# kondratevakate/mri-epilepsy-diagnosis

Measured on AMD Instinct MI355X. Metric: MRI volumes/sec (fwd+bwd) 3D U-Net @160x192x160, higher is better.
Workload: dtype f32; 1 GPU; unet.UNet(c0=8, 3 enc blocks, BN+PReLU, trilinear) fwd+softmax-Dice+bwd+AdamW, batch 2 x 1x160x192x160 fp32 per GPU (BASELINE configs[1]); global_batch=2, parallelism=dp1, launch=eager

## Files before the change

include/mri3d.h:

```cpp
#ifndef MRI3D_H
#define MRI3D_H

#include <stddef.h>
#include <stdint.h>

#ifdef __cplusplus
extern "C" {
#endif

typedef void* mri3d_stream_t;

enum { MRI3D_OK = 0, MRI3D_EINVAL = -1, MRI3D_ENOTSUP = -2, MRI3D_ELAUNCH = -3, MRI3D_EWORKSPACE = -4 };
enum { MRI3D_F32 = 0, MRI3D_BF16 = 1 };
enum { MRI3D_ACT_NONE = 0, MRI3D_ACT_RELU = 1, MRI3D_ACT_LEAKY = 2, MRI3D_ACT_PRELU = 3 };
enum { MRI3D_UP_NEAREST = 0, MRI3D_UP_TRILINEAR = 1 };
enum { MRI3D_PASS_FWD = 0, MRI3D_PASS_DGRAD = 1, MRI3D_PASS_WGRAD = 2 };

int mri3d_version(void);
const char* mri3d_last_error(void);

typedef struct Mri3dConvGeom {
    int32_t n;
    int32_t di, hi, wi, ci;
    int32_t dout, ho, wo, co;
    int32_t kd, kh, kw;
    int32_t sd, sh, sw;
    int32_t pd, ph, pw;
    int32_t dd, dh, dw;
    int32_t x_ld, y_ld;
    int32_t dtype;
} Mri3dConvGeom;

size_t mri3d_conv3d_workspace_bytes(const Mri3dConvGeom* g, int pass);

int mri3d_conv3d_fwd(const Mri3dConvGeom* g, const void* x, const void* w, const void* bias, void* y,
                     void* workspace, size_t ws_bytes, mri3d_stream_t stream);
int32_t mri3d_conv3d_fwd_stats_blocks(const Mri3dConvGeom* g);
int mri3d_conv3d_fwd_stats(const Mri3dConvGeom* g, const void* x, const void* w, const void* bias, void* y,
                           double* stat_partials, void* workspace, size_t ws_bytes, mri3d_stream_t stream);
int mri3d_conv3d_dgrad(const Mri3dConvGeom* g, const void* dy, const void* w, const void* bias, void* dx,
                       void* workspace, size_t ws_bytes, mri3d_stream_t stream);
int mri3d_conv3d_wgrad(const Mri3dConvGeom* g, const void* x, const void* dy, void* dw, void* dbias,
                       void* workspace, size_t ws_bytes, mri3d_stream_t stream);

int mri3d_conv3d_route(const Mri3dConvGeom* g, int32_t pass, int32_t stats, int32_t bias, int32_t split, int32_t second_ld,
                       int32_t align_x, int32_t align_y, char* name, size_t name_bytes);

int32_t mri3d_conv3d_cat_supported(const Mri3dConvGeom* g, int32_t split, int32_t second_ld, int32_t pass);
int32_t mri3d_conv3d_fwd_cat_stats_blocks(const Mri3dConvGeom* g, int32_t split, int32_t second_ld);
int mri3d_conv3d_fwd_cat(const Mri3dConvGeom* g, const void* x, const void* x2, int32_t split, int32_t x2_ld, const void* w,
                         const void* bias, void* y, double* stat_partials, void* workspace, size_t ws_bytes,
                         mri3d_stream_t stream);
int mri3d_conv3d_dgrad_cat(const Mri3dConvGeom* g, const void* dy, const void* w, void* dx, void* dx2, int32_t split,
                           int32_t dx2_ld, void* workspace, size_t ws_bytes, mri3d_stream_t stream);
int mri3d_conv3d_wgrad_cat(const Mri3dConvGeom* g, const void* x, const void* x2, int32_t split, int32_t x2_ld, const void* dy,
                           void* dw, void* dbias, void* workspace, size_t ws_bytes, mri3d_stream_t stream);

int32_t mri3d_conv3d_march_supported(const Mri3dConvGeom* g, int32_t pass);
int32_t mri3d_conv3d_march_stats_blocks(const Mri3dConvGeom* g);
int mri3d_conv3d_fwd_march(const Mri3dConvGeom* g, const void* x, const void* x2, int32_t split, int32_t x2_ld, const void* w,
                           const void* bias, void* y, double* stat_partials, void* workspace, size_t ws_bytes,
                           mri3d_stream_t stream);
int mri3d_conv3d_dgrad_march(const Mri3dConvGeom* g, const void* dy, const void* w, void* dx, void* dx2, int32_t split,
                             int32_t dx2_ld, void* workspace, size_t ws_bytes, mri3d_stream_t stream);

int32_t mri3d_upconv3d_supported(const Mri3dConvGeom* g, int32_t scale);
size_t mri3d_upconv3d_workspace_bytes(const Mri3dConvGeom* g, int32_t scale);
int mri3d_upconv3d_fwd(const Mri3dConvGeom* g, int32_t scale, const void* x, const float* w, const float* bias, void* y,
                       mri3d_stream_t stream);
int mri3d_upconv3d_dgrad(const Mri3dConvGeom* g, int32_t scale, const void* dy, const float* w, void* dx, mri3d_stream_t stream);
int mri3d_upconv3d_wgrad(const Mri3dConvGeom* g, int32_t scale, const void* x, const void* dy, float* dw, float* dbias,
                         void* workspace, size_t ws_bytes, mri3d_stream_t stream);

int32_t mri3d_convpair_supported(const Mri3dConvGeom* first, const Mri3dConvGeom* second);
size_t mri3d_convpair_workspace_bytes(const Mri3dConvGeom* first, const Mri3dConvGeom* second);
int mri3d_convpair_wgrad_first(const Mri3dConvGeom* first, const Mri3dConvGeom* second, const void* x, const void* dy2, const float* w2,
                               float* dw1, float* dbias1, void* workspace, size_t ws_bytes, mri3d_stream_t stream);

typedef struct Mri3dNormGeom {
    int32_t n;
    int64_t vox;
    int32_t c;
    int32_t x_ld;
    int32_t y_ld;
    int32_t instance;
    int32_t act;
    int32_t alpha_n;
    float slope;
    float eps;
    int32_t group_c;
    int32_t dtype;
} Mri3dNormGeom;

size_t mri3d_norm_workspace_bytes(const Mri3dNormGeom* g);

int mri3d_norm_stats(const Mri3dNormGeom* g, const void* x, float* mean, float* invstd,
                     float* running_mean, float* running_var, float momentum,
                     void* workspace, size_t ws_bytes, mri3d_stream_t stream);
int mri3d_norm_stats_from_partials(const Mri3dNormGeom* g, const double* partials, int32_t nblk, const float* shift,
                                   float* mean, float* invstd, float* running_mean, float* running_var, float momentum,
                                   mri3d_stream_t stream);
int mri3d_norm_act_fwd(const Mri3dNormGeom* g, const void* x, const float* mean, const float* invstd,
                       const float* gamma, const float* beta, const float* alpha, void* y,
                       mri3d_stream_t stream);
int mri3d_norm_act_bwd(const Mri3dNormGeom* g, int training, const void* x, const void* dy,
                       const float* mean, const float* invstd, const float* gamma, const float* beta,
                       const float* alpha, void* dx, float* dgamma, float* dbeta, float* dalpha,
                       void* workspace, size_t ws_bytes, mri3d_stream_t stream);

int32_t mri3d_norm_act_pw_supported(const Mri3dNormGeom* g, int32_t co);
size_t mri3d_norm_act_pw_workspace_bytes(const Mri3dNormGeom* g, int32_t co);
int mri3d_norm_act_pw_fwd(const Mri3dNormGeom* g, int32_t co, const void* x, const float* mean, const float* invstd,
                          const float* gamma, const float* beta, const float* alpha, const float* w, const float* bias,
                          void* out, mri3d_stream_t stream);
int mri3d_norm_act_pw_bwd(const Mri3dNormGeom* g, int32_t co, int training, const void* x, const void* dout,
                          const float* mean, const float* invstd, const float* gamma, const float* beta, const float* alpha,
                          const float* w, void* dx, float* dgamma, float* dbeta, float* dalpha, float* dw, float* dbias,
                          void* workspace, size_t ws_bytes, mri3d_stream_t stream);

typedef struct Mri3dPoolGeom {
    int32_t n, di, hi, wi, dout, ho, wo, c;
    int32_t kd, kh, kw, sd, sh, sw, pd, ph, pw;
    int32_t x_ld, y_ld;
    int32_t dtype;
} Mri3dPoolGeom;
int mri3d_maxpool3d_fwd(const Mri3dPoolGeom* g, const void* x, void* y, uint8_t* idx, mri3d_stream_t stream);
int mri3d_maxpool3d_bwd(const Mri3dPoolGeom* g, const void* dy, const uint8_t* idx, void* dx, mri3d_stream_t stream);
int mri3d_maxpool3d_bwd_add(const Mri3dPoolGeom* g, const void* dy, const uint8_t* idx, const void* addend,
                            int32_t addend_ld, void* dx, mri3d_stream_t stream);

typedef struct Mri3dUpGeom {
    int32_t n, di, hi, wi, dout, ho, wo, c;
    int32_t x_ld, y_ld;
    int32_t mode;
    int32_t align_corners;
    float rd, rh, rw;
    int32_t dtype;
} Mri3dUpGeom;
size_t mri3d_upsample3d_workspace_bytes(const Mri3dUpGeom* g);
int mri3d_upsample3d_fwd(const Mri3dUpGeom* g, const void* x, void* y, mri3d_stream_t stream);
int mri3d_upsample3d_bwd(const Mri3dUpGeom* g, const void* dy, void* dx, void* workspace, size_t ws_bytes,
                         mri3d_stream_t stream);

typedef struct Mri3dDiceGeom {
    int32_t n;
    int64_t vox;
    int32_t c, ct;
    int32_t x_ld, t_ld;
    float eps;
    int32_t dtype;
} Mri3dDiceGeom;
size_t mri3d_softmax_dice_workspace_bytes(const Mri3dDiceGeom* g);
int mri3d_softmax_dice_fwd(const Mri3dDiceGeom* g, const void* logits, const void* target, float* loss,
                           float* stats, void* workspace, size_t ws_bytes, mri3d_stream_t stream);
int mri3d_softmax_dice_bwd(const Mri3dDiceGeom* g, const void* logits, const void* target, const float* stats,
                           const float* dloss, void* dlogits, mri3d_stream_t stream);

int mri3d_argmax_u8(const void* logits, uint8_t* out, int64_t nvox, int32_t c, int32_t ld, int32_t dtype,
                    mri3d_stream_t stream);

size_t mri3d_mask_overlap_workspace_bytes(void);
int mri3d_mask_overlap(const uint8_t* pred, const uint8_t* gt, int64_t nvox, int64_t* counts, void* workspace,
                       size_t ws_bytes, mri3d_stream_t stream);

size_t mri3d_order_stats_workspace_bytes(void);
int mri3d_order_stats_f32(const float* x, int64_t n, const int64_t* ranks, int32_t nranks, float* out, void* workspace,
                          size_t ws_bytes, mri3d_stream_t stream);
int mri3d_piecewise_linear_f32(const float* x, float* y, int64_t n, const double* edges, const double* slope,
                               const double* intercept, int32_t nseg, mri3d_stream_t stream);
size_t mri3d_znorm_workspace_bytes(void);
int mri3d_znorm_mean_mask_f32(const float* x, float* y, int64_t n, double* stats, void* workspace, size_t ws_bytes,
                              mri3d_stream_t stream);
int mri3d_crop_or_pad_f32(const float* x, float* y, int32_t outer, int32_t di, int32_t hi, int32_t wi, int32_t dout,
                          int32_t ho, int32_t wo, float fill, mri3d_stream_t stream);

size_t mri3d_surface_distance_workspace_bytes(int32_t d, int32_t h, int32_t w);
int mri3d_surface_distance(const uint8_t* gt, const uint8_t* pred, int32_t d, int32_t h, int32_t w,
                           const double* area_table, double* sums, void* workspace, size_t ws_bytes, mri3d_stream_t stream);
int mri3d_surface_elements(const uint8_t* gt, const uint8_t* pred, int32_t d, int32_t h, int32_t w, int32_t* d2_gt,
                           uint8_t* code_gt, int32_t* d2_pred, uint8_t* code_pred, int64_t capacity, uint64_t* counts,
                           void* workspace, size_t ws_bytes, mri3d_stream_t stream);

int mri3d_extract_patches(const void* volumes, int32_t elem_bytes, int32_t nvol, int32_t d, int32_t h, int32_t w,
                          const int32_t* loc_host, int32_t npatch, int32_t pd, int32_t ph, int32_t pw, void* out,
                          mri3d_stream_t stream);
int mri3d_aggregate_patches_u8(const uint8_t* patches, const int32_t* loc_host, int32_t npatch, int32_t pd, int32_t ph,
                               int32_t pw, int32_t bd, int32_t bh, int32_t bw, uint8_t* out, int32_t nvol, int32_t d,
                               int32_t h, int32_t w, mri3d_stream_t stream);
int mri3d_aggregate_patches_argmax(const void* logits, int32_t c, int32_t ld, int32_t dtype, const int32_t* loc_host,
                                   int32_t npatch, int32_t pd, int32_t ph, int32_t pw, int32_t bd, int32_t bh, int32_t bw,
                                   uint8_t* out, int32_t nvol, int32_t d, int32_t h, int32_t w, mri3d_stream_t stream);

int mri3d_warp3d(const float* image, float* image_out, const void* label, void* label_out, int32_t label_bytes, int32_t s,
                 int32_t d, int32_t h, int32_t w, const float* affine, const float* grid, int32_t gd, int32_t gh, int32_t gw,
                 float pad_value, const float* pad_values, mri3d_stream_t stream);
int mri3d_bias_field_f32(const float* x, float* y, int32_t s, int32_t d, int32_t h, int32_t w, const float* coef_host,
                         int32_t order, mri3d_stream_t stream);

int mri3d_copy_channels(const void* src, void* dst, int64_t nvox, int32_t c, int32_t src_ld, int32_t dst_ld,
                        int32_t dtype, mri3d_stream_t stream);
int mri3d_add_channels(const void* a, const void* b, void* dst, int64_t nvox, int32_t c, int32_t a_ld,
                       int32_t b_ld, int32_t dst_ld, int32_t dtype, mri3d_stream_t stream);
int mri3d_convert_channels(const void* src, int32_t src_dtype, void* dst, int32_t dst_dtype, int64_t nvox, int32_t c,
                           int32_t src_ld, int32_t dst_ld, mri3d_stream_t stream);

int mri3d_bayes_weights_fwd(const float* mu, const float* logsigma, int64_t n, int32_t eval, float threshold, float* w_mean,
                            float* w_var, float* log_alpha, mri3d_stream_t stream);
int mri3d_bayes_weights_bwd(const float* mu, const float* logsigma, int64_t n, int32_t eval, float threshold,
                            const float* d_w_mean, const float* d_w_var, const float* d_log_alpha, float* dmu,
                            float* dlogsigma, mri3d_stream_t stream);
int mri3d_bayes_square(const void* x, void* x2, int64_t nvox, int32_t c, int32_t x_ld, int32_t x2_ld, int32_t dtype,
                       mri3d_stream_t stream);
int mri3d_bayes_sample_fwd(const void* mu_out, const void* var_out, const float* eps, void* y, int64_t nvox, int32_t c,
                           int32_t mu_ld, int32_t var_ld, int32_t eps_ld, int32_t y_ld, int32_t dtype, mri3d_stream_t stream);
int mri3d_bayes_sample_bwd(const void* dy, const void* var_out, const float* eps, void* dvar, int64_t nvox, int32_t c,
                           int32_t dy_ld, int32_t var_ld, int32_t eps_ld, int32_t dvar_ld, int32_t dtype,
                           mri3d_stream_t stream);
int mri3d_bayes_dx(const void* dx_mean, const void* dx_var, const void* x, void* dx, int64_t nvox, int32_t c,
                   int32_t dx_mean_ld, int32_t dx_var_ld, int32_t x_ld, int32_t dx_ld, int32_t dtype, mri3d_stream_t stream);

int mri3d_adam_step(float* p, const float* g, float* m, float* v, int64_t n, float lr, float beta1, float beta2,
                    float eps, float weight_decay, int32_t step, float grad_scale, int32_t decoupled,
                    mri3d_stream_t stream);

#ifdef __cplusplus
}
#endif
#endif
```

mri_epilepsy_diagnosis_amd/_lib.py:

```python
import ctypes
import os
from ctypes import POINTER, Structure, c_char_p, c_float, c_int32, c_int64, c_size_t, c_uint8, c_void_p

_HERE = os.path.dirname(os.path.abspath(__file__))
LIB_PATH = os.path.join(_HERE, "libmri3d_hip.so")

F32, BF16 = 0, 1
ACT_NONE, ACT_RELU, ACT_LEAKY, ACT_PRELU = 0, 1, 2, 3
UP_NEAREST, UP_TRILINEAR = 0, 1
PASS_FWD, PASS_DGRAD, PASS_WGRAD = 0, 1, 2


class ConvGeom(Structure):
    _fields_ = [(n, c_int32) for n in (
        "n", "di", "hi", "wi", "ci", "dout", "ho", "wo", "co", "kd", "kh", "kw", "sd", "sh", "sw",
        "pd", "ph", "pw", "dd", "dh", "dw", "x_ld", "y_ld", "dtype")]


class NormGeom(Structure):
    _fields_ = [("n", c_int32), ("vox", c_int64), ("c", c_int32), ("x_ld", c_int32), ("y_ld", c_int32),
                ("instance", c_int32), ("act", c_int32), ("alpha_n", c_int32), ("slope", c_float),
                ("eps", c_float), ("group_c", c_int32), ("dtype", c_int32)]


class PoolGeom(Structure):
    _fields_ = [(n, c_int32) for n in (
        "n", "di", "hi", "wi", "dout", "ho", "wo", "c", "kd", "kh", "kw", "sd", "sh", "sw", "pd", "ph", "pw",
        "x_ld", "y_ld", "dtype")]


class UpGeom(Structure):
    _fields_ = [(n, c_int32) for n in ("n", "di", "hi", "wi", "dout", "ho", "wo", "c", "x_ld", "y_ld", "mode",
                                       "align_corners")] + \
               [("rd", c_float), ("rh", c_float), ("rw", c_float), ("dtype", c_int32)]


class DiceGeom(Structure):
    _fields_ = [("n", c_int32), ("vox", c_int64), ("c", c_int32), ("ct", c_int32), ("x_ld", c_int32),
                ("t_ld", c_int32), ("eps", c_float), ("dtype", c_int32)]


_P = c_void_p
_FP = c_void_p

SIGNATURES = {
    "mri3d_version": (c_int32, []),
    "mri3d_last_error": (c_char_p, []),
    "mri3d_conv3d_workspace_bytes": (c_size_t, [POINTER(ConvGeom), c_int32]),
    "mri3d_conv3d_fwd": (c_int32, [POINTER(ConvGeom), _P, _P, _P, _P, _P, c_size_t, _P]),
    "mri3d_conv3d_fwd_stats_blocks": (c_int32, [POINTER(ConvGeom)]),
    "mri3d_conv3d_fwd_stats": (c_int32, [POINTER(ConvGeom), _P, _P, _P, _P, _P, _P, c_size_t, _P]),
    "mri3d_conv3d_dgrad": (c_int32, [POINTER(ConvGeom), _P, _P, _P, _P, _P, c_size_t, _P]),
    "mri3d_conv3d_wgrad": (c_int32, [POINTER(ConvGeom), _P, _P, _P, _P, _P, c_size_t, _P]),
    "mri3d_conv3d_route": (c_int32, [POINTER(ConvGeom), c_int32, c_int32, c_int32, c_int32, c_int32, c_int32, c_int32, c_char_p, c_size_t]),
    "mri3d_conv3d_cat_supported": (c_int32, [POINTER(ConvGeom), c_int32, c_int32, c_int32]),
    "mri3d_conv3d_fwd_cat_stats_blocks": (c_int32, [POINTER(ConvGeom), c_int32, c_int32]),
    "mri3d_conv3d_fwd_cat": (c_int32, [POINTER(ConvGeom), _P, _P, c_int32, c_int32, _P, _P, _P, _P, _P, c_size_t, _P]),
    "mri3d_conv3d_dgrad_cat": (c_int32, [POINTER(ConvGeom), _P, _P, _P, _P, c_int32, c_int32, _P, c_size_t, _P]),
    "mri3d_conv3d_wgrad_cat": (c_int32, [POINTER(ConvGeom), _P, _P, c_int32, c_int32, _P, _P, _P, _P, c_size_t, _P]),
    "mri3d_conv3d_march_supported": (c_int32, [POINTER(ConvGeom), c_int32]),
    "mri3d_conv3d_march_stats_blocks": (c_int32, [POINTER(ConvGeom)]),
    "mri3d_conv3d_fwd_march": (c_int32, [POINTER(ConvGeom), _P, _P, c_int32, c_int32, _P, _P, _P, _P, _P, c_size_t, _P]),
    "mri3d_conv3d_dgrad_march": (c_int32, [POINTER(ConvGeom), _P, _P, _P, _P, c_int32, c_int32, _P, c_size_t, _P]),
    "mri3d_upconv3d_supported": (c_int32, [POINTER(ConvGeom), c_int32]),
    "mri3d_upconv3d_workspace_bytes": (c_size_t, [POINTER(ConvGeom), c_int32]),
    "mri3d_upconv3d_fwd": (c_int32, [POINTER(ConvGeom), c_int32, _P, _FP, _FP, _P, _P]),
    "mri3d_upconv3d_dgrad": (c_int32, [POINTER(ConvGeom), c_int32, _P, _FP, _P, _P]),
    "mri3d_upconv3d_wgrad": (c_int32, [POINTER(ConvGeom), c_int32, _P, _P, _FP, _FP, _P, c_size_t, _P]),
    "mri3d_convpair_supported": (c_int32, [POINTER(ConvGeom), POINTER(ConvGeom)]),
    "mri3d_convpair_workspace_bytes": (c_size_t, [POINTER(ConvGeom), POINTER(ConvGeom)]),
    "mri3d_convpair_wgrad_first": (c_int32, [POINTER(ConvGeom), POINTER(ConvGeom), _P, _P, _FP, _FP, _FP, _P, c_size_t, _P]),
    "mri3d_norm_workspace_bytes": (c_size_t, [POINTER(NormGeom)]),
    "mri3d_norm_stats": (c_int32, [POINTER(NormGeom), _P, _FP, _FP, _FP, _FP, c_float, _P, c_size_t, _P]),
    "mri3d_norm_stats_from_partials": (c_int32, [POINTER(NormGeom), _P, c_int32, _FP, _FP, _FP, _FP, _FP, c_float, _P]),
    "mri3d_norm_act_fwd": (c_int32, [POINTER(NormGeom), _P, _FP, _FP, _FP, _FP, _FP, _P, _P]),
    "mri3d_norm_act_bwd": (c_int32, [POINTER(NormGeom), c_int32, _P, _P, _FP, _FP, _FP, _FP, _FP, _P, _FP, _FP, _FP,
                                     _P, c_size_t, _P]),
    "mri3d_norm_act_pw_supported": (c_int32, [POINTER(NormGeom), c_int32]),
    "mri3d_norm_act_pw_workspace_bytes": (c_size_t, [POINTER(NormGeom), c_int32]),
    "mri3d_norm_act_pw_fwd": (c_int32, [POINTER(NormGeom), c_int32, _P, _FP, _FP, _FP, _FP, _FP, _FP, _FP, _P, _P]),
    "mri3d_norm_act_pw_bwd": (c_int32, [POINTER(NormGeom), c_int32, c_int32, _P, _P, _FP, _FP, _FP, _FP, _FP, _FP, _P, _FP, _FP,
                                        _FP, _FP, _FP, _P, c_size_t, _P]),
    "mri3d_maxpool3d_fwd": (c_int32, [POINTER(PoolGeom), _P, _P, _P, _P]),
    "mri3d_maxpool3d_bwd": (c_int32, [POINTER(PoolGeom), _P, _P, _P, _P]),
    "mri3d_maxpool3d_bwd_add": (c_int32, [POINTER(PoolGeom), _P, _P, _P, c_int32, _P, _P]),
    "mri3d_upsample3d_workspace_bytes": (c_size_t, [POINTER(UpGeom)]),
    "mri3d_upsample3d_fwd": (c_int32, [POINTER(UpGeom), _P, _P, _P]),
    "mri3d_upsample3d_bwd": (c_int32, [POINTER(UpGeom), _P, _P, _P, c_size_t, _P]),
    "mri3d_softmax_dice_workspace_bytes": (c_size_t, [POINTER(DiceGeom)]),
    "mri3d_softmax_dice_fwd": (c_int32, [POINTER(DiceGeom), _P, _P, _FP, _FP, _P, c_size_t, _P]),
    "mri3d_softmax_dice_bwd": (c_int32, [POINTER(DiceGeom), _P, _P, _FP, _FP, _P, _P]),
    "mri3d_argmax_u8": (c_int32, [_P, _P, c_int64, c_int32, c_int32, c_int32, _P]),
    "mri3d_mask_overlap_workspace_bytes": (c_size_t, []),
    "mri3d_mask_overlap": (c_int32, [_P, _P, c_int64, _P, _P, c_size_t, _P]),
    "mri3d_order_stats_workspace_bytes": (c_size_t, []),
    "mri3d_order_stats_f32": (c_int32, [_P, c_int64, _P, c_int32, _P, _P, c_size_t, _P]),
    "mri3d_piecewise_linear_f32": (c_int32, [_P, _P, c_int64, _P, _P, _P, c_int32, _P]),
    "mri3d_znorm_workspace_bytes": (c_size_t, []),
    "mri3d_znorm_mean_mask_f32": (c_int32, [_P, _P, c_int64, _P, _P, c_size_t, _P]),
    "mri3d_crop_or_pad_f32": (c_int32, [_P, _P, c_int32, c_int32, c_int32, c_int32, c_int32, c_int32, c_int32, c_float, _P]),
    "mri3d_surface_distance_workspace_bytes": (c_size_t, [c_int32, c_int32, c_int32]),
    "mri3d_surface_distance": (c_int32, [_P, _P, c_int32, c_int32, c_int32, _P, _P, _P, c_size_t, _P]),
    "mri3d_surface_elements": (c_int32, [_P, _P, c_int32, c_int32, c_int32, _P, _P, _P, _P, c_int64, _P, _P, c_size_t, _P]),
    "mri3d_extract_patches": (c_int32, [_P, c_int32, c_int32, c_int32, c_int32, c_int32, _P, c_int32, c_int32, c_int32,
                                        c_int32, _P, _P]),
    "mri3d_aggregate_patches_u8": (c_int32, [_P, _P, c_int32, c_int32, c_int32, c_int32, c_int32, c_int32, c_int32, _P,
                                             c_int32, c_int32, c_int32, c_int32, _P]),
    "mri3d_aggregate_patches_argmax": (c_int32, [_P, c_int32, c_int32, c_int32, _P, c_int32, c_int32, c_int32, c_int32,
                                                 c_int32, c_int32, c_int32, _P, c_int32, c_int32, c_int32, c_int32, _P]),
    "mri3d_warp3d": (c_int32, [_FP, _FP, _P, _P, c_int32, c_int32, c_int32, c_int32, c_int32, _FP, _FP, c_int32, c_int32,
                               c_int32, c_float, _FP, _P]),
    "mri3d_bias_field_f32": (c_int32, [_FP, _FP, c_int32, c_int32, c_int32, c_int32, _P, c_int32, _P]),
    "mri3d_copy_channels": (c_int32, [_P, _P, c_int64, c_int32, c_int32, c_int32, c_int32, _P]),
    "mri3d_add_channels": (c_int32, [_P, _P, _P, c_int64, c_int32, c_int32, c_int32, c_int32, c_int32, _P]),
    "mri3d_convert_channels": (c_int32, [_P, c_int32, _P, c_int32, c_int64, c_int32, c_int32, c_int32, _P]),
    "mri3d_bayes_weights_fwd": (c_int32, [_FP, _FP, c_int64, c_int32, c_float, _FP, _FP, _FP, _P]),
    "mri3d_bayes_weights_bwd": (c_int32, [_FP, _FP, c_int64, c_int32, c_float, _FP, _FP, _FP, _FP, _FP, _P]),
    "mri3d_bayes_square": (c_int32, [_P, _P, c_int64, c_int32, c_int32, c_int32, c_int32, _P]),
    "mri3d_bayes_sample_fwd": (c_int32, [_P, _P, _FP, _P, c_int64, c_int32, c_int32, c_int32, c_int32, c_int32, c_int32, _P]),
    "mri3d_bayes_sample_bwd": (c_int32, [_P, _P, _FP, _P, c_int64, c_int32, c_int32, c_int32, c_int32, c_int32, c_int32, _P]),
    "mri3d_bayes_dx": (c_int32, [_P, _P, _P, _P, c_int64, c_int32, c_int32, c_int32, c_int32, c_int32, c_int32, _P]),
    "mri3d_adam_step": (c_int32, [_FP, _FP, _FP, _FP, c_int64, c_float, c_float, c_float, c_float, c_float, c_int32,
                                  c_float, c_int32, _P]),
}

_lib = None


class Mri3dError(RuntimeError):
    pass


def lib():
    global _lib
    if _lib is None:
        import torch
        if not os.path.exists(LIB_PATH):
            raise Mri3dError(
                "libmri3d_hip.so not found at %s — run `python -m mri_epilepsy_diagnosis_amd.build` "
                "(or __graft_entry__.build()).  There is no PyTorch fallback for device tensors." % LIB_PATH)
        h = ctypes.CDLL(LIB_PATH)
        for name, (res, args) in SIGNATURES.items():
            fn = getattr(h, name)
            fn.restype = res
            fn.argtypes = args
        _lib = h
    return _lib


def check(rc, what=""):
    if rc != 0:
        msg = lib().mri3d_last_error()
        raise Mri3dError("%s failed (rc=%d): %s" % (what, rc, msg.decode() if msg else "?"))
```

mri_epilepsy_diagnosis_amd/csrc/common.h:

```cpp
#pragma once
#include <hip/hip_runtime.h>
#include <stdint.h>
#include <stdio.h>
#include <stdarg.h>
#include <stdlib.h>
#include "../../include/mri3d.h"

namespace mri3d {

void set_error(const char* fmt, ...);

inline int check_launch(const char* what) {
    hipError_t e = hipGetLastError();
    if (e != hipSuccess) {
        set_error("%s: launch failed: %s", what, hipGetErrorString(e));
        return MRI3D_ELAUNCH;
    }
    return MRI3D_OK;
}

#define MRI3D_REQUIRE(cond, code, ...)      \
    do {                                    \
        if (!(cond)) {                      \
            ::mri3d::set_error(__VA_ARGS__); \
            return (code);                  \
        }                                   \
    } while (0)

#ifdef MRI3D_TUNING
inline int tuning_knob(const char* name, int dflt) {
    const char* v = getenv(name);
    return v ? atoi(v) : dflt;
}
#else
constexpr int tuning_knob(const char*, int dflt) { return dflt; }
#endif

inline int64_t cdiv64(int64_t a, int64_t b) { return (a + b - 1) / b; }
inline int cdiv(int a, int b) { return (a + b - 1) / b; }
inline size_t align_up(size_t x, size_t a) { return (x + a - 1) / a * a; }

constexpr int kMaxStreamBlocks = 2048;

inline int stream_grid(int64_t work_items, int per_block) {
    int64_t b = cdiv64(work_items, per_block);
    if (b > kMaxStreamBlocks) b = kMaxStreamBlocks;
    if (b < 1) b = 1;
    return (int)b;
}

typedef __bf16 bf16_t;
typedef __attribute__((ext_vector_type(4))) __bf16 bf16x4_t;
typedef __attribute__((ext_vector_type(8))) __bf16 bf16x8_t;

template <typename T> __device__ __forceinline__ float ldf(const T* p) { return (float)*p; }
template <typename T> __device__ __forceinline__ void stf(T* p, float v) { *p = (T)v; }

__device__ __forceinline__ float4 ldf4(const float* p) { return *reinterpret_cast<const float4*>(p); }
__device__ __forceinline__ float4 ldf4(const bf16_t* p) {
    const bf16x4_t v = *reinterpret_cast<const bf16x4_t*>(p);
    return make_float4((float)v[0], (float)v[1], (float)v[2], (float)v[3]);
}
__device__ __forceinline__ void stf4(float* p, float4 v) { *reinterpret_cast<float4*>(p) = v; }
__device__ __forceinline__ void stf4(bf16_t* p, float4 v) {
    bf16x4_t o;
    o[0] = (bf16_t)v.x, o[1] = (bf16_t)v.y, o[2] = (bf16_t)v.z, o[3] = (bf16_t)v.w;
    *reinterpret_cast<bf16x4_t*>(p) = o;
}

inline size_t dtype_size(int dtype) { return dtype == MRI3D_BF16 ? 2 : 4; }
inline bool aligned_vec4(int dtype, const void* a, const void* b = nullptr, const void* c = nullptr) {
    const uintptr_t m = dtype == MRI3D_BF16 ? 7 : 15;
    return ((reinterpret_cast<uintptr_t>(a) | reinterpret_cast<uintptr_t>(b) | reinterpret_cast<uintptr_t>(c)) & m) == 0;
}

inline bool aligned16(const void* a, const void* b = nullptr, const void* c = nullptr) {
    return ((reinterpret_cast<uintptr_t>(a) | reinterpret_cast<uintptr_t>(b) | reinterpret_cast<uintptr_t>(c)) & 15) == 0;
}

inline int ptr_align(const void* a, const void* b = nullptr, const void* c = nullptr, const void* d = nullptr) {
    const uintptr_t bits = reinterpret_cast<uintptr_t>(a) | reinterpret_cast<uintptr_t>(b) | reinterpret_cast<uintptr_t>(c) |
                           reinterpret_cast<uintptr_t>(d) | 16;
    return (int)(bits & (~bits + 1));
}
inline bool align_vec4(int dtype, int align) { return align >= (dtype == MRI3D_BF16 ? 8 : 16); }
inline bool align16(int align) { return align >= 16; }

#define MRI3D_DISPATCH_DTYPE(dtype, T, ...)  \
    do {                                     \
        if ((dtype) == MRI3D_BF16) {         \
            using T = ::mri3d::bf16_t;       \
            __VA_ARGS__                      \
        } else {                             \
            using T = float;                 \
            __VA_ARGS__                      \
        }                                    \
    } while (0)

__device__ __forceinline__ float wave_sum(float v) {
#pragma unroll
    for (int off = 32; off > 0; off >>= 1) v += __shfl_xor(v, off, 64);
    return v;
}

__device__ __forceinline__ double wave_sum_d(double v) {
#pragma unroll
    for (int off = 32; off > 0; off >>= 1) v += __shfl_xor(v, off, 64);
    return v;
}

__device__ __forceinline__ float apply_act(float v, int act, float slope) {
    if (act == MRI3D_ACT_RELU) return v > 0.f ? v : 0.f;
    if (act == MRI3D_ACT_LEAKY || act == MRI3D_ACT_PRELU) return v > 0.f ? v : v * slope;
    return v;
}

}
```

mri_epilepsy_diagnosis_amd/csrc/norm.hip:

```cpp
#include "common.h"
#include <algorithm>

namespace mri3d {

struct NormPlan {
    int vec;
    int CL;
    int VT;
    int cy;
    int nblk;
    int groups;
    int64_t gvox;
};

constexpr int kNormMaxBlocks = 1024;
constexpr int kFinQL = 64;

static NormPlan norm_plan(const Mri3dNormGeom& g, bool al, bool al16 = false) {
    NormPlan p;
    p.vec = (g.c % 4 == 0 && g.x_ld % 4 == 0 && g.y_ld % 4 == 0 && al) ? 4 : 1;
    if (p.vec == 4 && g.dtype == MRI3D_BF16 && g.c % 8 == 0 && g.x_ld % 8 == 0 && g.y_ld % 8 == 0 && al16) p.vec = 8;
    int lanes = g.c / p.vec;
    p.CL = lanes < 256 ? lanes : 256;
    p.cy = cdiv(lanes, p.CL);
// ... 370 lines not shown
            a += p[(size_t)q * C * 3];
            b += p[(size_t)q * C * 3 + 1];
            d += p[(size_t)q * C * 3 + 2];
            a1 += p[(size_t)(q + kFinQL) * C * 3];
            b1 += p[(size_t)(q + kFinQL) * C * 3 + 1];
            d1 += p[(size_t)(q + kFinQL) * C * 3 + 2];
        }
        if (q < nblk) {
            a += p[(size_t)q * C * 3];
            b += p[(size_t)q * C * 3 + 1];
            d += p[(size_t)q * C * 3 + 2];
        }
        a += a1;
        b += b1;
        d += d1;
    }
    r0[threadIdx.x] = a;
    r1[threadIdx.x] = b;
    r2[threadIdx.x] = d;
    __syncthreads();
    if (!ok || ql != 0) return;
    a = b = d = 0.0;
    for (int q = 0; q < kFinQL; ++q) {
        a += r0[slot * kFinQL + q];
        b += r1[slot * kFinQL + q];
        d += r2[slot * kFinQL + q];
    }
    sums[(size_t)i * 3] = (float)a;
    sums[(size_t)i * 3 + 1] = (float)b;
    sums[(size_t)i * 3 + 2] = (float)d;
}

__device__ __forceinline__ void norm_act_bwd_params_block(const float* __restrict__ sums, float* __restrict__ dgamma,
                                                          float* __restrict__ dbeta, float* __restrict__ dalpha, int alpha_n, int C,
                                                          int groups) {
    __shared__ double dal[256];
    double my_dal = 0.0;
    for (int c = threadIdx.x; c < C; c += blockDim.x) {
        double tg = 0.0, tb = 0.0, ta = 0.0;
        for (int g = 0; g < groups; ++g) {
            tb += (double)sums[((size_t)g * C + c) * 3];
            tg += (double)sums[((size_t)g * C + c) * 3 + 1];
            ta += (double)sums[((size_t)g * C + c) * 3 + 2];
        }
        if (dgamma) dgamma[c] = (float)tg;
        if (dbeta) dbeta[c] = (float)tb;
        if (dalpha && alpha_n > 1) dalpha[c] = (float)ta;
        my_dal += ta;
    }
    if (dalpha && alpha_n == 1) {
        dal[threadIdx.x] = my_dal;
        __syncthreads();
        if (threadIdx.x == 0) {
            double t = 0.0;
            for (int i = 0; i < (int)blockDim.x; ++i) t += dal[i];
            dalpha[0] = (float)t;
        }
    }
}

__global__ void norm_act_bwd_params_kernel(const float* __restrict__ sums, float* __restrict__ dgamma,
                                           float* __restrict__ dbeta, float* __restrict__ dalpha, int alpha_n, int C,
                                           int groups) {
    norm_act_bwd_params_block(sums, dgamma, dbeta, dalpha, alpha_n, C, groups);
}

template <typename T, int VEC>
__global__ void __launch_bounds__(256)
norm_act_bwd_apply_kernel(const T* __restrict__ x, const T* __restrict__ dy, T* __restrict__ dx,
                          const float* __restrict__ sums, const float* __restrict__ mean,
                          const float* __restrict__ invstd, const float* __restrict__ gamma,
                          const float* __restrict__ beta, const float* __restrict__ alpha, int alpha_n, int act,
                          float slope, int training, int C, int x_ld, int y_ld, int64_t gvox, int CL, int VT, int group_c,
                          float* __restrict__ dgamma, float* __restrict__ dbeta, float* __restrict__ dalpha) {
    if ((dgamma != nullptr || dbeta != nullptr || dalpha != nullptr) && blockIdx.x == 0 && blockIdx.y == 0 && blockIdx.z == 0)
        norm_act_bwd_params_block(sums, dgamma, dbeta, dalpha, alpha_n, C, (int)gridDim.z);
    const int tid = threadIdx.x;
    const int cl = tid % CL, vt = tid / CL;
    const int c0 = (blockIdx.y * CL + cl) * VEC;
    if (vt >= VT || c0 >= C) return;
    const int group = blockIdx.z;
    float mu[VEC], is[VEC], gm[VEC], bt[VEC], al[VEC], k0[VEC], k1[VEC], k2[VEC];
    const float invM = 1.f / ((float)gvox * (float)(group_c > 0 ? group_c : 1));
#pragma unroll
    for (int j = 0; j < VEC; ++j) {
        int c = c0 + j;
        gm[j] = gamma ? gamma[c] : 1.f;
        bt[j] = beta ? beta[c] : 0.f;
        mu[j] = mean ? mean[group * C + c] : 0.f;
        is[j] = invstd ? invstd[group * C + c] : 1.f;
        al[j] = (act == MRI3D_ACT_PRELU) ? alpha[alpha_n == 1 ? 0 : c]
                                          : (act == MRI3D_ACT_LEAKY ? slope : (act == MRI3D_ACT_RELU ? 0.f : 1.f));
        k0[j] = gm[j] * is[j];
        if (training) {
            const float kk = group_c > 0 ? is[j] : k0[j];
            k1[j] = kk * sums[((size_t)group * C + c) * 3] * invM;
            k2[j] = kk * sums[((size_t)group * C + c) * 3 + 1] * invM;
        } else {
            k1[j] = 0.f;
            k2[j] = 0.f;
        }
    }
    const T* xg = x + (int64_t)group * gvox * x_ld;
    const T* dg = dy + (int64_t)group * gvox * y_ld;
    T* og = dx + (int64_t)group * gvox * x_ld;
    auto apply = [&](const float (&xv)[VEC], const float (&gv)[VEC], float (&ov)[VEC]) {
#pragma unroll
        for (int j = 0; j < VEC; ++j) {
            float xh = (xv[j] - mu[j]) * is[j];
            float u = fmaf(gm[j], xh, bt[j]);
            float du = (u > 0.f) ? gv[j] : gv[j] * al[j];
            ov[j] = fmaf(k0[j], du, -k1[j]) - xh * k2[j];
        }
    };
    const int64_t step = (int64_t)gridDim.x * VT;
    int64_t v = (int64_t)blockIdx.x * VT + vt;
    for (; v + step < gvox; v += 2 * step) {
        float xa[VEC], ga[VEC], xb[VEC], gb[VEC], ov[VEC];
        Ld<VEC>::load(xg + v * x_ld + c0, xa);
        Ld<VEC>::load(dg + v * y_ld + c0, ga);
        Ld<VEC>::load(xg + (v + step) * x_ld + c0, xb);
        Ld<VEC>::load(dg + (v + step) * y_ld + c0, gb);
        apply(xa, ga, ov);
        Ld<VEC>::store(og + v * x_ld + c0, ov);
        apply(xb, gb, ov);
        Ld<VEC>::store(og + (v + step) * x_ld + c0, ov);
    }
    for (; v < gvox; v += step) {
        float xv[VEC], gv[VEC], ov[VEC];
        Ld<VEC>::load(xg + v * x_ld + c0, xv);
        Ld<VEC>::load(dg + v * y_ld + c0, gv);
        apply(xv, gv, ov);
        Ld<VEC>::store(og + v * x_ld + c0, ov);
    }
}


struct NapArgs {
    const float *mean, *invstd, *gamma, *beta, *alpha;
    int alpha_n, act;
    float slope;
    int C, x_ld;
    int64_t nvox;
};

constexpr int kNapMaxCo = 4;

template <typename T>
__device__ __forceinline__ float through_storage(float v) {
    if constexpr (sizeof(T) == 2) return (float)(bf16_t)v;
    else return v;
}

__device__ __forceinline__ void nap_fwd_consts(const NapArgs& p, int c0, float (&sc)[4], float (&sh)[4], float (&al)[4]) {
#pragma unroll
    for (int j = 0; j < 4; ++j) {
        int c = c0 + j;
        float gm = p.gamma ? p.gamma[c] : 1.f;
        float bt = p.beta ? p.beta[c] : 0.f;
        float mu = p.mean ? p.mean[c] : 0.f;
        float is = p.invstd ? p.invstd[c] : 1.f;
        sc[j] = gm * is;
        sh[j] = bt - mu * sc[j];
        al[j] = (p.act == MRI3D_ACT_PRELU) ? p.alpha[p.alpha_n == 1 ? 0 : c] : p.slope;
    }
}

template <typename T, int CO>
__global__ void __launch_bounds__(256)
norm_act_pw_fwd_kernel(const T* __restrict__ x, T* __restrict__ out, const float* __restrict__ w,
                       const float* __restrict__ bias, int Co, int o_ld, NapArgs p) {
    const int QC = p.C >> 2, VT = 256 / QC;
    const int q = threadIdx.x % QC, vt = threadIdx.x / QC;
    float sc[4], sh[4], al[4];
    nap_fwd_consts(p, 4 * q, sc, sh, al);
    float4 wq[CO];
    float bq[CO];
#pragma unroll
    for (int co = 0; co < CO; ++co) {
        const float* wr = w + (size_t)(co < Co ? co : 0) * p.C + 4 * q;
        wq[co] = co < Co ? make_float4(wr[0], wr[1], wr[2], wr[3]) : make_float4(0.f, 0.f, 0.f, 0.f);
        bq[co] = (bias != nullptr && co < Co) ? bias[co] : 0.f;
    }
    constexpr int U = 4;
    const int64_t stride = (int64_t)gridDim.x * VT;
    for (int64_t v0 = (int64_t)blockIdx.x * VT + vt; v0 < p.nvox; v0 += stride * U) {
        float xv[U][4];
#pragma unroll
        for (int u = 0; u < U; ++u) {
            const int64_t v = v0 + u * stride;
            Ld<4>::load(x + (v < p.nvox ? v : p.nvox - 1) * p.x_ld + 4 * q, xv[u]);
        }
#pragma unroll
        for (int u = 0; u < U; ++u) {
            const int64_t v = v0 + u * stride;
            float a[4];
#pragma unroll
            for (int j = 0; j < 4; ++j) a[j] = through_storage<T>(apply_act(fmaf(xv[u][j], sc[j], sh[j]), p.act, al[j]));
            float acc[CO];
#pragma unroll
            for (int co = 0; co < CO; ++co) {
                float t = a[0] * wq[co].x;
                t = fmaf(a[1], wq[co].y, t);
                t = fmaf(a[2], wq[co].z, t);
                t = fmaf(a[3], wq[co].w, t);
                for (int d = 1; d < QC; d <<= 1) t += __shfl_xor(t, d, 64);
                acc[co] = t + bq[co];
            }
            if (q == 0 && v < p.nvox) {
                T* op = out + v * o_ld;
#pragma unroll
                for (int co = 0; co < CO; ++co)
                    if (co < Co) stf(op + co, acc[co]);
            }
        }
    }
}

template <typename T, int CO>
struct PwHeadGrad {
    struct Args {
        const T* dout;
        const float* w;
        int Co, ld;
    };
    static constexpr int kCo = CO;
    static constexpr int kSide = 5 * CO;
    const T* dout;
    int Co, ld;
    float4 wq[CO];
    double dw[4][CO], db[CO];

    __device__ __forceinline__ void init(const Args& a, int C, int q) {
        dout = a.dout, Co = a.Co, ld = a.ld;
#pragma unroll
        for (int co = 0; co < CO; ++co) {
            const float* wr = a.w + (size_t)(co < Co ? co : 0) * C + 4 * q;
            wq[co] = co < Co ? make_float4(wr[0], wr[1], wr[2], wr[3]) : make_float4(0.f, 0.f, 0.f, 0.f);
            db[co] = 0.0;
#pragma unroll
            for (int j = 0; j < 4; ++j) dw[j][co] = 0.0;
        }
    }
    __device__ __forceinline__ void load(int64_t v, float (&gv)[CO]) const {
#pragma unroll
        for (int co = 0; co < CO; ++co) gv[co] = co < Co ? ldf(dout + v * ld + co) : 0.f;
    }
    __device__ __forceinline__ void grad(const float (&gv)[CO], float (&da)[4]) const {
        float4 acc = make_float4(0.f, 0.f, 0.f, 0.f);
#pragma unroll
        for (int co = 0; co < CO; ++co) {
            acc.x = fmaf(gv[co], wq[co].x, acc.x);
            acc.y = fmaf(gv[co], wq[co].y, acc.y);
            acc.z = fmaf(gv[co], wq[co].z, acc.z);
            acc.w = fmaf(gv[co], wq[co].w, acc.w);
        }
        da[0] = through_storage<T>(acc.x), da[1] = through_storage<T>(acc.y);
        da[2] = through_storage<T>(acc.z), da[3] = through_storage<T>(acc.w);
    }
    __device__ __forceinline__ void side(const float (&a)[4], const float (&gv)[CO], bool lead) {
#pragma unroll
        for (int co = 0; co < CO; ++co) {
#pragma unroll
            for (int j = 0; j < 4; ++j) dw[j][co] += (double)(a[j] * gv[co]);
            if (lead) db[co] += (double)gv[co];
        }
    }
    __device__ __forceinline__ void flush(double* red, double* __restrict__ spart, int C, int QC, int VT) const {
        const int tid = threadIdx.x;
#pragma unroll
        for (int co = 0; co < CO; ++co) {
#pragma unroll
            for (int j = 0; j < 4; ++j) red[tid * kSide + j * CO + co] = dw[j][co];
            red[tid * kSide + 4 * CO + co] = db[co];
        }
        __syncthreads();
        double* o = spart + (size_t)blockIdx.x * (Co * C + Co);
        for (int e = tid; e < QC * 4 * CO; e += 256) {
            const int co = e % CO, j = (e / CO) % 4, qq = e / (4 * CO);
            double s = 0.0;
            for (int l = 0; l < VT; ++l) s += red[(l * QC + qq) * kSide + j * CO + co];
            if (co < Co) o[co * C + 4 * qq + j] = s;
        }
        if (tid < Co) {
            double s = 0.0;
            for (int l = 0; l < VT; ++l) s += red[(l * QC) * kSide + 4 * CO + tid];
            o[Co * C + tid] = s;
        }
    }
};

template <typename T, class SRC, bool SUMS, bool DX>
__global__ void __launch_bounds__(256)
norm_act_src_bwd_kernel(const T* __restrict__ x, T* __restrict__ dx, typename SRC::Args sa, NapArgs p,
                        const float* __restrict__ sums, int training, double* __restrict__ part, double* __restrict__ spart,
                        float* __restrict__ dgamma, float* __restrict__ dbeta, float* __restrict__ dalpha) {
    constexpr int kRed = SUMS ? (SRC::kSide > 12 ? SRC::kSide : 12) : 1;
    __shared__ double red[256 * kRed];
    if (!SUMS && (dgamma != nullptr || dbeta != nullptr || dalpha != nullptr) && blockIdx.x == 0)
        norm_act_bwd_params_block(sums, dgamma, dbeta, dalpha, p.alpha_n, p.C, 1);
    const int QC = p.C >> 2, VT = 256 / QC;
    const int tid = threadIdx.x;
    const int q = tid % QC, vt = tid / QC;
    const int c0 = 4 * q;
    float mu[4], is[4], gm[4], bt[4], al[4], k0[4], k1[4], k2[4];
    const float invM = 1.f / (float)p.nvox;
#pragma unroll
    for (int j = 0; j < 4; ++j) {
        int c = c0 + j;
        gm[j] = p.gamma ? p.gamma[c] : 1.f;
        bt[j] = p.beta ? p.beta[c] : 0.f;
        mu[j] = p.mean ? p.mean[c] : 0.f;
        is[j] = p.invstd ? p.invstd[c] : 1.f;
        al[j] = (p.act == MRI3D_ACT_PRELU) ? p.alpha[p.alpha_n == 1 ? 0 : c]
                                            : (p.act == MRI3D_ACT_LEAKY ? p.slope : (p.act == MRI3D_ACT_RELU ? 0.f : 1.f));
        k0[j] = gm[j] * is[j];
        if (DX && !SUMS && training) {
            k1[j] = k0[j] * sums[(size_t)c * 3] * invM;
            k2[j] = k0[j] * sums[(size_t)c * 3 + 1] * invM;
        } else {
            k1[j] = 0.f;
            k2[j] = 0.f;
        }
    }
    float sc[4], sh[4], af[4];
    if constexpr (SUMS) nap_fwd_consts(p, c0, sc, sh, af);
    SRC src;
    src.init(sa, p.C, q);
    double s0[4], s1[4], s2[4];
#pragma unroll
    for (int j = 0; j < 4; ++j) { s0[j] = 0.0; s1[j] = 0.0; s2[j] = 0.0; }
    auto row = [&](const float (&xv)[4], const float (&gv)[SRC::kCo], int64_t v) {
        float da[4], ov[4];
        src.grad(gv, da);
#pragma unroll
        for (int j = 0; j < 4; ++j) {
            float xh = (xv[j] - mu[j]) * is[j];
            float u = fmaf(gm[j], xh, bt[j]);
            bool pos = u > 0.f;
            float du = pos ? da[j] : da[j] * al[j];
            if constexpr (SUMS) {
                s0[j] += (double)du;
                s1[j] = fma((double)du, (double)xh, s1[j]);
                s2[j] += pos ? 0.0 : (double)da[j] * (double)u;
            }
            if constexpr (DX) ov[j] = fmaf(k0[j], du, -k1[j]) - xh * k2[j];
        }
        if constexpr (SUMS) {
            float a[4];
#pragma unroll
            for (int j = 0; j < 4; ++j) a[j] = through_storage<T>(apply_act(fmaf(xv[j], sc[j], sh[j]), p.act, af[j]));
            src.side(a, gv, q == 0);
        }
        if constexpr (DX) Ld<4>::store(dx + v * p.x_ld + c0, ov);
    };
    const int64_t step = (int64_t)gridDim.x * VT;
    int64_t v = (int64_t)blockIdx.x * VT + vt;
    for (; v + step < p.nvox; v += 2 * step) {
        float xa[4], xb[4], ga[SRC::kCo], gb[SRC::kCo];
        Ld<4>::load(x + v * p.x_ld + c0, xa);
        src.load(v, ga);
        Ld<4>::load(x + (v + step) * p.x_ld + c0, xb);
        src.load(v + step, gb);
        row(xa, ga, v);
        row(xb, gb, v + step);
    }
    for (; v < p.nvox; v += step) {
        float xv[4], gv[SRC::kCo];
        Ld<4>::load(x + v * p.x_ld + c0, xv);
        src.load(v, gv);
        row(xv, gv, v);
    }
    if constexpr (SUMS) {
#pragma unroll
        for (int j = 0; j < 4; ++j) {
            red[(tid * 4 + j) * 3] = s0[j];
            red[(tid * 4 + j) * 3 + 1] = s1[j];
            red[(tid * 4 + j) * 3 + 2] = s2[j];
        }
        __syncthreads();
        if (vt == 0) {
#pragma unroll
            for (int j = 0; j < 4; ++j) {
                double a = 0.0, b = 0.0, d = 0.0;
                for (int l = 0; l < VT; ++l) {
                    a += red[((l * QC + q) * 4 + j) * 3];
                    b += red[((l * QC + q) * 4 + j) * 3 + 1];
                    d += red[((l * QC + q) * 4 + j) * 3 + 2];
                }
                double* o = part + ((size_t)blockIdx.x * p.C + c0 + j) * 3;
                o[0] = a;
                o[1] = b;
                o[2] = d;
            }
        }
        __syncthreads();
        src.flush(red, spart, p.C, QC, VT);
    }
}

__global__ void __launch_bounds__(256)
norm_act_pw_wsum_kernel(const double* __restrict__ spart, float* __restrict__ dw, float* __restrict__ dbias, int nb, int nw,
                        int Co) {
    __shared__ double red[256];
    const int el = threadIdx.x >> 5, ql = threadIdx.x & 31;
    const int ntot = nw + Co;
    const int i = blockIdx.x * 8 + el;
    double s = 0.0;
    if (i < ntot)
        for (int b = ql; b < nb; b += 32) s += spart[(size_t)b * ntot + i];
    red[threadIdx.x] = s;
    __syncthreads();
    if (ql == 0 && i < ntot) {
        double t = 0.0;
        for (int k = 0; k < 32; ++k) t += red[el * 32 + k];
        if (i < nw) {
            if (dw != nullptr) dw[i] = (float)t;
        } else if (dbias != nullptr) {
            dbias[i - nw] = (float)t;
        }
    }
}

struct NapPlan {
    int QC, VT, nblk;
    size_t part_off, sums_off, side_off, bytes;
};

static bool nap_supported(const Mri3dNormGeom& g, int co) {
    if (g.dtype != MRI3D_F32 && g.dtype != MRI3D_BF16) return false;
    if (g.n <= 0 || g.vox <= 0 || g.instance || g.group_c != 0) return false;
    const int qc = g.c / 4;
    if (g.c <= 0 || g.c % 4 != 0 || qc > 16 || (qc & (qc - 1)) != 0) return false;
    if (co < 1 || co > kNapMaxCo) return false;
    if (g.x_ld < g.c || g.x_ld % 4 != 0 || g.y_ld < co) return false;
    if (g.act < MRI3D_ACT_NONE || g.act > MRI3D_ACT_PRELU) return false;
    if (g.act == MRI3D_ACT_PRELU && g.alpha_n != 1 && g.alpha_n != g.c) return false;
    return true;
}

static NapPlan nap_plan(const Mri3dNormGeom& g, int co) {
    NapPlan p;
    p.QC = g.c / 4;
    p.VT = 256 / p.QC;
    const int64_t nvox = (int64_t)g.n * g.vox;
    const int64_t want = cdiv64(nvox, (int64_t)p.VT * 8);
    p.nblk = (int)(want < kNormMaxBlocks ? want : kNormMaxBlocks);
    if (p.nblk < 1) p.nblk = 1;
    p.part_off = 0;
    p.sums_off = (size_t)p.nblk * g.c * 3 * sizeof(double);
    p.side_off = p.sums_off + align_up((size_t)g.c * 3 * sizeof(float), sizeof(double));
    p.bytes = p.side_off + (size_t)p.nblk * (co * g.c + co) * sizeof(double);
    return p;
}

}

using namespace mri3d;

extern "C" size_t mri3d_norm_workspace_bytes(const Mri3dNormGeom* g) {
    if (!g) return 0;
    return norm_workspace_floats(*g) * sizeof(float);
}

static int norm_check(const Mri3dNormGeom* g, const char* who) {
    MRI3D_REQUIRE(g != nullptr, MRI3D_EINVAL, "%s: null geometry", who);
    MRI3D_REQUIRE(g->dtype == MRI3D_F32 || g->dtype == MRI3D_BF16, MRI3D_ENOTSUP, "%s: unknown dtype %d", who, g->dtype);
    MRI3D_REQUIRE(g->n > 0 && g->vox > 0 && g->c > 0 && g->x_ld >= g->c && g->y_ld >= g->c, MRI3D_EINVAL,
                  "%s: bad geometry n=%d vox=%lld c=%d x_ld=%d y_ld=%d", who, g->n, (long long)g->vox, g->c, g->x_ld,
                  g->y_ld);
    MRI3D_REQUIRE(g->act != MRI3D_ACT_PRELU || g->alpha_n == 1 || g->alpha_n == g->c, MRI3D_EINVAL,
                  "%s: PReLU alpha_n=%d must be 1 or C=%d", who, g->alpha_n, g->c);
    MRI3D_REQUIRE(g->group_c == 0 || (g->group_c > 0 && g->instance && g->c % g->group_c == 0), MRI3D_EINVAL,
                  "%s: group_c=%d needs instance mode and must divide C=%d", who, g->group_c, g->c);
    return MRI3D_OK;
}

extern "C" int mri3d_norm_stats(const Mri3dNormGeom* g, const void* x, float* mean, float* invstd, float* running_mean,
                                float* running_var, float momentum, void* workspace, size_t ws_bytes,
                                mri3d_stream_t stream) {
    int rc = norm_check(g, "norm_stats");
    if (rc) return rc;
    MRI3D_REQUIRE(x && mean && invstd, MRI3D_EINVAL, "norm_stats: null pointer");
    MRI3D_REQUIRE(workspace && ws_bytes >= mri3d_norm_workspace_bytes(g), MRI3D_EWORKSPACE,
                  "norm_stats: workspace %zu < %zu", ws_bytes, mri3d_norm_workspace_bytes(g));
    hipStream_t s = static_cast<hipStream_t>(stream);
    Mri3dNormGeom gg = *g;
    gg.y_ld = gg.x_ld;
    NormPlan p = norm_plan(gg, aligned_vec4(g->dtype, x));
    double* part = static_cast<double*>(workspace);
    dim3 grid(p.nblk, p.cy, p.groups);
    const int tot = p.groups * g->c;
    MRI3D_DISPATCH_DTYPE(g->dtype, T, {
        const T* xf = static_cast<const T*>(x);
        if (p.vec == 4)
            hipLaunchKernelGGL((norm_stats_kernel<T, 4>), grid, dim3(256), 0, s, xf, part, g->c, g->x_ld, p.gvox, p.CL, p.VT);
        else if (p.vec == 1)
            hipLaunchKernelGGL((norm_stats_kernel<T, 1>), grid, dim3(256), 0, s, xf, part, g->c, g->x_ld, p.gvox, p.CL, p.VT);
        hipLaunchKernelGGL(norm_stats_finalize_kernel<T>, dim3(cdiv(tot, 256 / kFinQL)), dim3(256), 0, s, xf, part, mean,
                           invstd, running_mean, running_var, momentum, g->eps, g->c, g->x_ld, p.gvox, p.nblk, p.groups);
        if (g->group_c > 0) {
            const int ng = p.groups * (g->c / g->group_c);
            hipLaunchKernelGGL(norm_stats_group_finalize_kernel<T>, dim3(cdiv(ng, 64)), dim3(64), 0, s, xf, part, mean,
                               invstd, g->eps, g->c, g->x_ld, p.gvox, p.nblk, p.groups, g->group_c);
        }
    });
    return check_launch("norm_stats");
}

extern "C" int mri3d_norm_stats_from_partials(const Mri3dNormGeom* g, const double* partials, int32_t nblk, const float* shift,
                                              float* mean, float* invstd, float* running_mean, float* running_var,
                                              float momentum, mri3d_stream_t stream) {
    int rc = norm_check(g, "norm_stats_from_partials");
    if (rc) return rc;
    MRI3D_REQUIRE(partials && mean && invstd && nblk > 0, MRI3D_EINVAL, "norm_stats_from_partials: null pointer / no partials");
    MRI3D_REQUIRE(!g->instance && g->group_c == 0, MRI3D_ENOTSUP,
                  "norm_stats_from_partials: batch statistics only (one group over N x voxels)");
    hipStream_t s = static_cast<hipStream_t>(stream);
    const int64_t gvox = (int64_t)g->n * g->vox;
    hipLaunchKernelGGL(norm_stats_finalize_kernel<float>, dim3(cdiv(g->c, 256 / kFinQL)), dim3(256), 0, s,
                       static_cast<const float*>(nullptr), partials, mean, invstd, running_mean, running_var, momentum, g->eps,
                       g->c, g->x_ld, gvox, nblk, 1, shift, 1);
    return check_launch("norm_stats_from_partials");
}

extern "C" int mri3d_norm_act_fwd(const Mri3dNormGeom* g, const void* x, const float* mean, const float* invstd,
                                  const float* gamma, const float* beta, const float* alpha, void* y,
                                  mri3d_stream_t stream) {
    int rc = norm_check(g, "norm_act_fwd");
    if (rc) return rc;
    MRI3D_REQUIRE(x && y, MRI3D_EINVAL, "norm_act_fwd: null pointer");
    MRI3D_REQUIRE((mean == nullptr) == (invstd == nullptr), MRI3D_EINVAL, "norm_act_fwd: mean/invstd must both be set");
    MRI3D_REQUIRE(g->act != MRI3D_ACT_PRELU || alpha, MRI3D_EINVAL, "norm_act_fwd: PReLU needs alpha");
    hipStream_t s = static_cast<hipStream_t>(stream);
    NormPlan p = norm_plan(*g, aligned_vec4(g->dtype, x, y), aligned16(x, y));
    dim3 grid(p.nblk, p.cy, p.groups);
    MRI3D_DISPATCH_DTYPE(g->dtype, T, {
        const T* xf = static_cast<const T*>(x);
        T* yf = static_cast<T*>(y);
        if constexpr (sizeof(T) == 2) {
            if (p.vec == 8) hipLaunchKernelGGL((norm_act_fwd_kernel<T, 8>), grid, dim3(256), 0, s, xf, yf, mean, invstd, gamma, beta, alpha,
                               g->alpha_n, g->act, g->slope, g->c, g->x_ld, g->y_ld, p.gvox, p.CL, p.VT);
        }
        if (p.vec == 4)
            hipLaunchKernelGGL((norm_act_fwd_kernel<T, 4>), grid, dim3(256), 0, s, xf, yf, mean, invstd, gamma, beta, alpha,
                               g->alpha_n, g->act, g->slope, g->c, g->x_ld, g->y_ld, p.gvox, p.CL, p.VT);
        else if (p.vec == 1)
            hipLaunchKernelGGL((norm_act_fwd_kernel<T, 1>), grid, dim3(256), 0, s, xf, yf, mean, invstd, gamma, beta, alpha,
                               g->alpha_n, g->act, g->slope, g->c, g->x_ld, g->y_ld, p.gvox, p.CL, p.VT);
    });
    return check_launch("norm_act_fwd");
}

extern "C" int mri3d_norm_act_bwd(const Mri3dNormGeom* g, int training, const void* x, const void* dy,
                                  const float* mean, const float* invstd, const float* gamma, const float* beta,
                                  const float* alpha, void* dx, float* dgamma, float* dbeta, float* dalpha,
                                  void* workspace, size_t ws_bytes, mri3d_stream_t stream) {
    int rc = norm_check(g, "norm_act_bwd");
    if (rc) return rc;
    MRI3D_REQUIRE(x && dy && dx, MRI3D_EINVAL, "norm_act_bwd: null pointer");
    MRI3D_REQUIRE((mean == nullptr) == (invstd == nullptr), MRI3D_EINVAL, "norm_act_bwd: mean/invstd must both be set");
    MRI3D_REQUIRE(!(training && mean == nullptr), MRI3D_EINVAL, "norm_act_bwd: training mode needs statistics");
    MRI3D_REQUIRE(g->act != MRI3D_ACT_PRELU || alpha, MRI3D_EINVAL, "norm_act_bwd: PReLU needs alpha");
    MRI3D_REQUIRE(workspace && ws_bytes >= mri3d_norm_workspace_bytes(g), MRI3D_EWORKSPACE,
                  "norm_act_bwd: workspace %zu < %zu", ws_bytes, mri3d_norm_workspace_bytes(g));
    hipStream_t s = static_cast<hipStream_t>(stream);
    NormPlan p = norm_plan(*g, aligned_vec4(g->dtype, x, dy, dx));
    dim3 grid(p.nblk, p.cy, p.groups);
    double* part = static_cast<double*>(workspace);
    float* sums = reinterpret_cast<float*>(part + (size_t)p.groups * p.nblk * g->c * 3);
    const bool need_reduce = training || dgamma || dbeta || dalpha;
    bool params_done = false;
    MRI3D_DISPATCH_DTYPE(g->dtype, T, {
        const T* xf = static_cast<const T*>(x);
// ... 4 lines not shown
                hipLaunchKernelGGL((norm_act_bwd_frozen_kernel<T, 4>), grid, dim3(256), 0, s, xf, df, of, part, mean, invstd,
                                   gamma, beta, alpha, g->alpha_n, g->act, g->slope, g->c, g->x_ld, g->y_ld, p.gvox, p.CL,
                                   p.VT);
            else if (p.vec == 1)
                hipLaunchKernelGGL((norm_act_bwd_frozen_kernel<T, 1>), grid, dim3(256), 0, s, xf, df, of, part, mean, invstd,
                                   gamma, beta, alpha, g->alpha_n, g->act, g->slope, g->c, g->x_ld, g->y_ld, p.gvox, p.CL,
                                   p.VT);
            hipLaunchKernelGGL(norm_act_bwd_sums_kernel, dim3(cdiv(p.groups * g->c, 256 / kFinQL)), dim3(256), 0, s, part,
                               sums, g->c, p.nblk, p.groups);
            hipLaunchKernelGGL(norm_act_bwd_params_kernel, dim3(1), dim3(256), 0, s, sums, dgamma, dbeta, dalpha, g->alpha_n,
                               g->c, p.groups);
            return check_launch("norm_act_bwd");
        }
        if (need_reduce) {
            if (p.vec == 4)
                hipLaunchKernelGGL((norm_act_bwd_reduce_kernel<T, 4>), grid, dim3(256), 0, s, xf, df, part, mean, invstd,
                                   gamma, beta, alpha, g->alpha_n, g->act, g->slope, g->c, g->x_ld, g->y_ld, p.gvox, p.CL,
                                   p.VT);
            else if (p.vec == 1)
                hipLaunchKernelGGL((norm_act_bwd_reduce_kernel<T, 1>), grid, dim3(256), 0, s, xf, df, part, mean, invstd,
                                   gamma, beta, alpha, g->alpha_n, g->act, g->slope, g->c, g->x_ld, g->y_ld, p.gvox, p.CL,
                                   p.VT);
            hipLaunchKernelGGL(norm_act_bwd_sums_kernel, dim3(cdiv(p.groups * g->c, 256 / kFinQL)), dim3(256), 0, s, part,
                               sums, g->c, p.nblk, p.groups);
            if ((dgamma || dbeta || dalpha) && g->group_c > 0) {
                hipLaunchKernelGGL(norm_act_bwd_params_kernel, dim3(1), dim3(256), 0, s, sums, dgamma, dbeta, dalpha,
                                   g->alpha_n, g->c, p.groups);
                params_done = true;
            }
            if (g->group_c > 0 && training) {
                const int ng = p.groups * (g->c / g->group_c);
                hipLaunchKernelGGL(norm_act_bwd_group_combine_kernel, dim3(cdiv(ng, 64)), dim3(64), 0, s, sums, gamma,
                                   g->c, p.groups, g->group_c);
            }
        }
        float* pg = params_done ? nullptr : dgamma;
        float* pb = params_done ? nullptr : dbeta;
        float* pa = params_done ? nullptr : dalpha;
        if (p.vec == 4)
            hipLaunchKernelGGL((norm_act_bwd_apply_kernel<T, 4>), grid, dim3(256), 0, s, xf, df, of, sums, mean, invstd,
                               gamma, beta, alpha, g->alpha_n, g->act, g->slope, training, g->c, g->x_ld, g->y_ld, p.gvox,
                               p.CL, p.VT, g->group_c, pg, pb, pa);
        else if (p.vec == 1)
            hipLaunchKernelGGL((norm_act_bwd_apply_kernel<T, 1>), grid, dim3(256), 0, s, xf, df, of, sums, mean, invstd,
                               gamma, beta, alpha, g->alpha_n, g->act, g->slope, training, g->c, g->x_ld, g->y_ld, p.gvox,
                               p.CL, p.VT, g->group_c, pg, pb, pa);
    });
    return check_launch("norm_act_bwd");
}

extern "C" int32_t mri3d_norm_act_pw_supported(const Mri3dNormGeom* g, int32_t co) {
    return (g != nullptr && nap_supported(*g, co)) ? 1 : 0;
}

extern "C" size_t mri3d_norm_act_pw_workspace_bytes(const Mri3dNormGeom* g, int32_t co) {
    if (g == nullptr || !nap_supported(*g, co)) return 0;
    return nap_plan(*g, co).bytes;
}

static NapArgs nap_args(const Mri3dNormGeom& g, const float* mean, const float* invstd, const float* gamma, const float* beta,
                        const float* alpha) {
    NapArgs a;
    a.mean = mean, a.invstd = invstd, a.gamma = gamma, a.beta = beta, a.alpha = alpha;
    a.alpha_n = g.alpha_n, a.act = g.act, a.slope = g.slope, a.C = g.c, a.x_ld = g.x_ld;
    a.nvox = (int64_t)g.n * g.vox;
    return a;
}

extern "C" int mri3d_norm_act_pw_fwd(const Mri3dNormGeom* g, int32_t co, const void* x, const float* mean, const float* invstd,
                                     const float* gamma, const float* beta, const float* alpha, const float* w,
                                     const float* bias, void* out, mri3d_stream_t stream) {
    MRI3D_REQUIRE(g != nullptr, MRI3D_EINVAL, "norm_act_pw_fwd: null geometry");
    MRI3D_REQUIRE(nap_supported(*g, co), MRI3D_ENOTSUP, "norm_act_pw_fwd: c=%d co=%d x_ld=%d y_ld=%d instance=%d not served",
                  g->c, co, g->x_ld, g->y_ld, g->instance);
    MRI3D_REQUIRE(x && w && out, MRI3D_EINVAL, "norm_act_pw_fwd: null pointer");
    MRI3D_REQUIRE((mean == nullptr) == (invstd == nullptr), MRI3D_EINVAL, "norm_act_pw_fwd: mean/invstd must both be set");
    MRI3D_REQUIRE(g->act != MRI3D_ACT_PRELU || alpha, MRI3D_EINVAL, "norm_act_pw_fwd: PReLU needs alpha");
    MRI3D_REQUIRE(aligned_vec4(g->dtype, x), MRI3D_EINVAL, "norm_act_pw_fwd: x must be aligned to 4 elements");
    hipStream_t s = static_cast<hipStream_t>(stream);
    const NapArgs a = nap_args(*g, mean, invstd, gamma, beta, alpha);
    const int VT = 256 / (g->c / 4);
    const unsigned grid = (unsigned)std::max<int64_t>(1, std::min<int64_t>(cdiv64(a.nvox, (int64_t)VT * 4), kMaxStreamBlocks));
    MRI3D_DISPATCH_DTYPE(g->dtype, T, {
        if (co <= 2)
            hipLaunchKernelGGL((norm_act_pw_fwd_kernel<T, 2>), dim3(grid), dim3(256), 0, s, (const T*)x, (T*)out, w, bias, co,
                               g->y_ld, a);
        else
            hipLaunchKernelGGL((norm_act_pw_fwd_kernel<T, 4>), dim3(grid), dim3(256), 0, s, (const T*)x, (T*)out, w, bias, co,
                               g->y_ld, a);
    });
    return check_launch("norm_act_pw_fwd");
}

template <typename T, int CO>
static void nap_bwd_launch(const Mri3dNormGeom& g, int co, int training, const T* x, const T* dout, const float* w, T* dx,
                           float* dgamma, float* dbeta, float* dalpha, float* dw, float* dbias, const NapArgs& a,
                           const NapPlan& p, char* ws, hipStream_t s) {
    using SRC = PwHeadGrad<T, CO>;
    const typename SRC::Args sa = {dout, w, co, g.y_ld};
    double* part = reinterpret_cast<double*>(ws + p.part_off);
    float* sums = reinterpret_cast<float*>(ws + p.sums_off);
    double* spart = reinterpret_cast<double*>(ws + p.side_off);
    const dim3 grid(p.nblk), blk(256);
    const bool params = dgamma || dbeta || dalpha;
    const bool need_sums = training || params || dw || dbias;
    if (need_sums) {
        if (training || dx == nullptr)
            hipLaunchKernelGGL((norm_act_src_bwd_kernel<T, SRC, true, false>), grid, blk, 0, s, x, dx, sa, a, sums, training,
                               part, spart, dgamma, dbeta, dalpha);
        else
            hipLaunchKernelGGL((norm_act_src_bwd_kernel<T, SRC, true, true>), grid, blk, 0, s, x, dx, sa, a, sums, training,
                               part, spart, dgamma, dbeta, dalpha);
        hipLaunchKernelGGL(norm_act_bwd_sums_kernel, dim3(cdiv(g.c, 256 / kFinQL)), dim3(256), 0, s, part, sums, g.c, p.nblk, 1);
        if (dw || dbias)
            hipLaunchKernelGGL(norm_act_pw_wsum_kernel, dim3(cdiv(co * g.c + co, 8)), dim3(256), 0, s, spart, dw, dbias, p.nblk,
                               co * g.c, co);
        if (params && !(training && dx != nullptr))
            hipLaunchKernelGGL(norm_act_bwd_params_kernel, dim3(1), dim3(256), 0, s, sums, dgamma, dbeta, dalpha, g.alpha_n, g.c,
                               1);
    }
    if (dx != nullptr && (training || !need_sums))
        hipLaunchKernelGGL((norm_act_src_bwd_kernel<T, SRC, false, true>), grid, blk, 0, s, x, dx, sa, a, sums, training, part,
                           spart, dgamma, dbeta, dalpha);
}

extern "C" int mri3d_norm_act_pw_bwd(const Mri3dNormGeom* g, int32_t co, int training, const void* x, const void* dout,
                                     const float* mean, const float* invstd, const float* gamma, const float* beta,
                                     const float* alpha, const float* w, void* dx, float* dgamma, float* dbeta, float* dalpha,
                                     float* dw, float* dbias, void* workspace, size_t ws_bytes, mri3d_stream_t stream) {
    MRI3D_REQUIRE(g != nullptr, MRI3D_EINVAL, "norm_act_pw_bwd: null geometry");
    MRI3D_REQUIRE(nap_supported(*g, co), MRI3D_ENOTSUP, "norm_act_pw_bwd: c=%d co=%d x_ld=%d y_ld=%d instance=%d not served",
                  g->c, co, g->x_ld, g->y_ld, g->instance);
    MRI3D_REQUIRE(x && dout && w, MRI3D_EINVAL, "norm_act_pw_bwd: null pointer");
    MRI3D_REQUIRE((mean == nullptr) == (invstd == nullptr), MRI3D_EINVAL, "norm_act_pw_bwd: mean/invstd must both be set");
    MRI3D_REQUIRE(!(training && mean == nullptr), MRI3D_EINVAL, "norm_act_pw_bwd: training mode needs statistics");
    MRI3D_REQUIRE(g->act != MRI3D_ACT_PRELU || alpha, MRI3D_EINVAL, "norm_act_pw_bwd: PReLU needs alpha");
    MRI3D_REQUIRE(aligned_vec4(g->dtype, x, dx), MRI3D_EINVAL, "norm_act_pw_bwd: x and dx must be aligned to 4 elements");
    const NapPlan p = nap_plan(*g, co);
    MRI3D_REQUIRE(workspace && ws_bytes >= p.bytes && (reinterpret_cast<uintptr_t>(workspace) & 7) == 0, MRI3D_EWORKSPACE,
                  "norm_act_pw_bwd: workspace %zu < %zu (or not 8-byte aligned)", ws_bytes, p.bytes);
    hipStream_t s = static_cast<hipStream_t>(stream);
    const NapArgs a = nap_args(*g, mean, invstd, gamma, beta, alpha);
    char* ws = static_cast<char*>(workspace);
    MRI3D_DISPATCH_DTYPE(g->dtype, T, {
        if (co <= 2)
            nap_bwd_launch<T, 2>(*g, co, training, (const T*)x, (const T*)dout, w, (T*)dx, dgamma, dbeta, dalpha, dw, dbias, a, p, ws,
                                 s);
        else
            nap_bwd_launch<T, 4>(*g, co, training, (const T*)x, (const T*)dout, w, (T*)dx, dgamma, dbeta, dalpha, dw, dbias, a, p, ws,
                                 s);
    });
    return check_launch("norm_act_pw_bwd");
}
```

mri_epilepsy_diagnosis_amd/csrc/resample.hip:

```cpp
#include "common.h"
#include <limits.h>
#include <algorithm>
#include <stdlib.h>

namespace mri3d {

template <int VEC>
struct V {
    float v[VEC];
    template <typename T>
    __device__ __forceinline__ void load(const T* p) {
        if constexpr (VEC == 8) {
            const bf16x8_t t = *reinterpret_cast<const bf16x8_t*>(p);
#pragma unroll
            for (int j = 0; j < 8; ++j) v[j] = (float)t[j];
        } else if constexpr (VEC == 4) {
            float4 t = ldf4(p);
            v[0] = t.x; v[1] = t.y; v[2] = t.z; v[3] = t.w;
        } else {
            v[0] = ldf(p);
        }
    }
    template <typename T>
    __device__ __forceinline__ void store(T* p) const {
// ... 53 lines not shown
                }
            }
            V<VEC> o;
#pragma unroll
            for (int j = 0; j < VEC; ++j) o.v[j] = best[j];
            const int64_t ov = obase + pix;
            o.store(y + ov * g.y_ld + cv * VEC);
            uint8_t* ip = idx + ov * g.c + cv * VEC;
            if constexpr (VEC == 8) {
                uint2 pk;
                pk.x = (uint32_t)bi[0] | ((uint32_t)bi[1] << 8) | ((uint32_t)bi[2] << 16) | ((uint32_t)bi[3] << 24);
                pk.y = (uint32_t)bi[4] | ((uint32_t)bi[5] << 8) | ((uint32_t)bi[6] << 16) | ((uint32_t)bi[7] << 24);
                *reinterpret_cast<uint2*>(ip) = pk;
            } else if constexpr (VEC == 4) {
                *reinterpret_cast<uint32_t*>(ip) = (uint32_t)bi[0] | ((uint32_t)bi[1] << 8) |
                                                   ((uint32_t)bi[VEC > 2 ? 2 : 0] << 16) | ((uint32_t)bi[VEC > 3 ? 3 : 0] << 24);
            } else {
                ip[0] = (uint8_t)bi[0];
            }
        }
    }
}

template <typename T, int VEC>
__global__ void __launch_bounds__(256)
maxpool_bwd_kernel(Mri3dPoolGeom g, const T* __restrict__ dy, const uint8_t* __restrict__ idx,
                   T* __restrict__ dx, int hch, const T* __restrict__ addend, int a_ld) {
    const unsigned CV = g.c / VEC;
    const int hchunks = (g.hi + hch - 1) / hch;
    const int slabs = g.n * g.di * hchunks;
    for (int slab = blockIdx.x; slab < slabs; slab += gridDim.x) {
        const int hc = slab % hchunks, nd = slab / hchunks;
        const int n = nd / g.di, id = nd - n * g.di;
        const int h0 = hc * hch, hn = min(hch, g.hi - h0);
        const unsigned inner = (unsigned)hn * g.wi * CV;
        int od_lo = id + g.pd - g.kd + 1; od_lo = od_lo <= 0 ? 0 : (od_lo + g.sd - 1) / g.sd;
        int od_hi = (id + g.pd) / g.sd; if (od_hi > g.dout - 1) od_hi = g.dout - 1;
        const int64_t ibase = ((int64_t)nd * g.hi + h0) * g.wi;
        for (unsigned e = threadIdx.x; e < inner; e += blockDim.x) {
            const unsigned cv = e % CV, pix = e / CV;
            const int iw = pix % g.wi, ih = h0 + pix / g.wi;
            float acc[VEC];
#pragma unroll
            for (int j = 0; j < VEC; ++j) acc[j] = 0.f;
            if (addend != nullptr) {
                V<VEC> av;
                av.load(addend + (ibase + pix) * a_ld + cv * VEC);
#pragma unroll
                for (int j = 0; j < VEC; ++j) acc[j] = av.v[j];
            }
            int oh_lo = ih + g.ph - g.kh + 1; oh_lo = oh_lo <= 0 ? 0 : (oh_lo + g.sh - 1) / g.sh;
            int oh_hi = (ih + g.ph) / g.sh; if (oh_hi > g.ho - 1) oh_hi = g.ho - 1;
            int ow_lo = iw + g.pw - g.kw + 1; ow_lo = ow_lo <= 0 ? 0 : (ow_lo + g.sw - 1) / g.sw;
            int ow_hi = (iw + g.pw) / g.sw; if (ow_hi > g.wo - 1) ow_hi = g.wo - 1;
            for (int od = od_lo; od <= od_hi; ++od) {
                const int kd = id - (od * g.sd - g.pd);
                for (int oh = oh_lo; oh <= oh_hi; ++oh) {
                    const int kh = ih - (oh * g.sh - g.ph);
                    for (int ow = ow_lo; ow <= ow_hi; ++ow) {
                        const int kw = iw - (ow * g.sw - g.pw);
                        const int tap = (kd * g.kh + kh) * g.kw + kw;
                        const int64_t ov = (((int64_t)n * g.dout + od) * g.ho + oh) * g.wo + ow;
                        V<VEC> gv;
                        gv.load(dy + ov * g.y_ld + cv * VEC);
                        const uint8_t* ip = idx + ov * g.c + cv * VEC;
                        if constexpr (VEC == 8) {
                            const uint2 pk = *reinterpret_cast<const uint2*>(ip);
#pragma unroll
                            for (int j = 0; j < 4; ++j) {
                                if ((int)((pk.x >> (8 * j)) & 0xff) == tap) acc[j] += gv.v[j];
                                if ((int)((pk.y >> (8 * j)) & 0xff) == tap) acc[4 + j] += gv.v[4 + j];
                            }
                        } else if constexpr (VEC == 4) {
                            const uint32_t pk = *reinterpret_cast<const uint32_t*>(ip);
#pragma unroll
                            for (int j = 0; j < VEC; ++j)
                                if ((int)((pk >> (8 * j)) & 0xff) == tap) acc[j] += gv.v[j];
                        } else {
                            if ((int)ip[0] == tap) acc[0] += gv.v[0];
                        }
                    }
                }
            }
            V<VEC> o;
#pragma unroll
            for (int j = 0; j < VEC; ++j) o.v[j] = acc[j];
            o.store(dx + (ibase + pix) * g.x_ld + cv * VEC);
        }
    }
}

template <typename T, int VEC>
__global__ void __launch_bounds__(256)
maxpool2_fwd_kernel(Mri3dPoolGeom g, const T* __restrict__ x, T* __restrict__ y, uint8_t* __restrict__ idx, int hch) {
    const unsigned CV = g.c / VEC;
    const int hchunks = (g.ho + hch - 1) / hch;
    const int slabs = g.n * g.dout * hchunks;
    const unsigned row = (unsigned)g.wi * g.x_ld, plane = (unsigned)g.hi * row;
    for (int slab = blockIdx.x; slab < slabs; slab += gridDim.x) {
        const int hc = slab % hchunks, nd = slab / hchunks;
        const int n = nd / g.dout, od = nd - n * g.dout;
        const int h0 = hc * hch, hn = min(hch, g.ho - h0);
        const unsigned inner = (unsigned)hn * g.wi * CV;
        const T* xs = x + ((int64_t)n * g.di + 2 * od) * g.hi * g.wi * g.x_ld;
        const int64_t obase = ((int64_t)nd * g.ho + h0) * g.wo;
        for (unsigned e0 = 0; e0 < inner; e0 += blockDim.x) {
            const unsigned e = e0 + threadIdx.x;
            const bool live = e < inner;
            const unsigned ee = live ? e : 0;
            const unsigned cv = ee % CV, col = ee / CV;
            const unsigned iw = col % g.wi, ohl = col / g.wi;
            const unsigned kw = iw & 1, ow = iw >> 1, oh = h0 + ohl;
            const T* p0 = xs + (2 * oh) * row + iw * (unsigned)g.x_ld + cv * VEC;
            V<VEC> v[4];
#pragma unroll
            for (int t = 0; t < 4; ++t) v[t].load(p0 + (t >> 1) * plane + (t & 1) * row);
            float best[VEC];
            int bi[VEC];
#pragma unroll
            for (int j = 0; j < VEC; ++j) { best[j] = v[0].v[j]; bi[j] = (int)kw; }
#pragma unroll
            for (int t = 1; t < 4; ++t)
#pragma unroll
                for (int j = 0; j < VEC; ++j)
                    if (v[t].v[j] > best[j] || v[t].v[j] != v[t].v[j]) { best[j] = v[t].v[j]; bi[j] = 2 * t + (int)kw; }
            V<VEC> o;
            int oi[VEC];
#pragma unroll
            for (int j = 0; j < VEC; ++j) {
                const float pb = __shfl_xor(best[j], (int)CV, 64);
                const int pi = __shfl_xor(bi[j], (int)CV, 64);
                const bool mine_nan = best[j] != best[j], his_nan = pb != pb;
                bool take_his;
                if (mine_nan || his_nan) take_his = his_nan && (!mine_nan || pi > bi[j]);
                else take_his = pb > best[j] || (pb == best[j] && pi < bi[j]);
                o.v[j] = take_his ? pb : best[j];
                oi[j] = take_his ? pi : bi[j];
            }
            if (live && kw == 0) {
                const int64_t ov = obase + (int64_t)ohl * g.wo + ow;
                o.store(y + ov * g.y_ld + cv * VEC);
                uint8_t* ip = idx + ov * g.c + cv * VEC;
                if constexpr (VEC == 8) {
                    uint2 pk;
                    pk.x = (uint32_t)oi[0] | ((uint32_t)oi[1] << 8) | ((uint32_t)oi[2] << 16) | ((uint32_t)oi[3] << 24);
                    pk.y = (uint32_t)oi[4] | ((uint32_t)oi[5] << 8) | ((uint32_t)oi[6] << 16) | ((uint32_t)oi[7] << 24);
                    *reinterpret_cast<uint2*>(ip) = pk;
                } else {
                    *reinterpret_cast<uint32_t*>(ip) = (uint32_t)oi[0] | ((uint32_t)oi[1] << 8) | ((uint32_t)oi[2] << 16) | ((uint32_t)oi[3] << 24);
                }
            }
        }
    }
}

static inline bool pool2_ok(const Mri3dPoolGeom& g, int vec) {
    const int cv = g.c / vec;
    return g.kd == 2 && g.kh == 2 && g.kw == 2 && g.sd == 2 && g.sh == 2 && g.sw == 2 && g.pd == 0 && g.ph == 0 && g.pw == 0 &&
           g.di == 2 * g.dout && g.hi == 2 * g.ho && g.wi == 2 * g.wo && cv >= 1 && cv <= 32 && (cv & (cv - 1)) == 0 &&
           (int64_t)g.di * g.hi * g.wi * g.x_ld < ((int64_t)1 << 31);
}

struct Lin { int i0, i1; float l0, l1; };
__device__ __forceinline__ Lin lin_src(int o, float r, int in_size, int align_corners) {
    float src = align_corners ? r * (float)o : fmaf(r, (float)o + 0.5f, -0.5f);
    if (!align_corners && src < 0.f) src = 0.f;
    Lin L;
    L.i0 = (int)src;
    if (L.i0 > in_size - 1) L.i0 = in_size - 1;
    L.i1 = L.i0 + (L.i0 < in_size - 1 ? 1 : 0);
    L.l1 = src - (float)L.i0;
    if (L.l1 < 0.f) L.l1 = 0.f;
    if (L.l1 > 1.f) L.l1 = 1.f;
    L.l0 = 1.f - L.l1;
    return L;
}
__device__ __forceinline__ int near_src(int o, float r, int in_size) {
    int i = (int)floorf((float)o * r);
    return i < in_size - 1 ? i : in_size - 1;
}

template <typename T, int VEC>
__global__ void __launch_bounds__(256)
upsample_fwd_kernel(Mri3dUpGeom g, const T* __restrict__ x, T* __restrict__ y, int hch) {
    const unsigned CV = g.c / VEC;
    const int hchunks = (g.ho + hch - 1) / hch;
    const int slabs = g.n * g.dout * hchunks;
    for (int slab = blockIdx.x; slab < slabs; slab += gridDim.x) {
        const int hc = slab % hchunks, nd = slab / hchunks;
        const int n = nd / g.dout, od = nd - n * g.dout;
        const int h0 = hc * hch, hn = min(hch, g.ho - h0);
        const unsigned inner = (unsigned)hn * g.wo * CV;
        const T* xn = x + (int64_t)n * g.di * g.hi * g.wi * g.x_ld;
        const int64_t obase = ((int64_t)nd * g.ho + h0) * g.wo;
        int idn = 0;
        Lin Ld_ = {0, 0, 1.f, 0.f};
        if (g.mode == MRI3D_UP_NEAREST) idn = near_src(od, g.rd, g.di);
        else Ld_ = lin_src(od, g.rd, g.di, g.align_corners);
        for (unsigned e = threadIdx.x; e < inner; e += blockDim.x) {
            const unsigned cv = e % CV, pix = e / CV;
            const int ow = pix % g.wo, oh = h0 + pix / g.wo;
            const T* xc = xn + cv * VEC;
            V<VEC> o;
            if (g.mode == MRI3D_UP_NEAREST) {
                const int ih = near_src(oh, g.rh, g.hi), iw = near_src(ow, g.rw, g.wi);
                o.load(xc + (((int64_t)idn * g.hi + ih) * g.wi + iw) * g.x_ld);
            } else {
                const Lin Lh = lin_src(oh, g.rh, g.hi, g.align_corners);
                const Lin Lw = lin_src(ow, g.rw, g.wi, g.align_corners);
#pragma unroll
                for (int j = 0; j < VEC; ++j) o.v[j] = 0.f;
#pragma unroll
                for (int a = 0; a < 2; ++a) {
                    const int id = a ? Ld_.i1 : Ld_.i0;
                    const float wd = a ? Ld_.l1 : Ld_.l0;
#pragma unroll
                    for (int b = 0; b < 2; ++b) {
                        const int ih = b ? Lh.i1 : Lh.i0;
                        const float wh = wd * (b ? Lh.l1 : Lh.l0);
#pragma unroll
                        for (int c = 0; c < 2; ++c) {
                            const int iw = c ? Lw.i1 : Lw.i0;
                            const float w = wh * (c ? Lw.l1 : Lw.l0);
                            V<VEC> xv;
                            xv.load(xc + (((int64_t)id * g.hi + ih) * g.wi + iw) * g.x_ld);
#pragma unroll
                            for (int j = 0; j < VEC; ++j) o.v[j] = fmaf(w, xv.v[j], o.v[j]);
                        }
                    }
                }
            }
            o.store(y + (obase + pix) * g.y_ld + cv * VEC);
        }
    }
}

__global__ void upsample_tables_kernel(Mri3dUpGeom g, int* __restrict__ tab) {
    int axis = blockIdx.x;
    int in_size = axis == 0 ? g.di : (axis == 1 ? g.hi : g.wi);
    int out_size = axis == 0 ? g.dout : (axis == 1 ? g.ho : g.wo);
    float r = axis == 0 ? g.rd : (axis == 1 ? g.rh : g.rw);
    int* lo = tab + (axis == 0 ? 0 : (axis == 1 ? 2 * g.di : 2 * g.di + 2 * g.hi));
    int* hi = lo + in_size;
    for (int i = threadIdx.x; i < in_size; i += blockDim.x) { lo[i] = INT_MAX; hi[i] = -1; }
    __syncthreads();
    for (int o = threadIdx.x; o < out_size; o += blockDim.x) {
        if (g.mode == MRI3D_UP_NEAREST) {
            int i = near_src(o, r, in_size);
            atomicMin(&lo[i], o);
            atomicMax(&hi[i], o);
        } else {
            Lin L = lin_src(o, r, in_size, g.align_corners);
            atomicMin(&lo[L.i0], o);
            atomicMax(&hi[L.i0], o);
            atomicMin(&lo[L.i1], o);
            atomicMax(&hi[L.i1], o);
        }
    }
}

__device__ __forceinline__ float up_weight(int o, int i, float r, int in_size, int mode, int align_corners) {
    if (mode == MRI3D_UP_NEAREST) return near_src(o, r, in_size) == i ? 1.f : 0.f;
    Lin L = lin_src(o, r, in_size, align_corners);
    return (L.i0 == i ? L.l0 : 0.f) + (L.i1 == i ? L.l1 : 0.f);
}

template <typename T, int VEC>
__global__ void __launch_bounds__(256)
upsample_bwd_kernel(Mri3dUpGeom g, const T* __restrict__ dy, T* __restrict__ dx, const int* __restrict__ tab, int hch) {
    const unsigned CV = g.c / VEC;
    const int* lo_d = tab; const int* hi_d = tab + g.di;
    const int* lo_h = tab + 2 * g.di; const int* hi_h = lo_h + g.hi;
    const int* lo_w = tab + 2 * g.di + 2 * g.hi; const int* hi_w = lo_w + g.wi;
    const int hchunks = (g.hi + hch - 1) / hch;
    const int slabs = g.n * g.di * hchunks;
    for (int slab = blockIdx.x; slab < slabs; slab += gridDim.x) {
        const int hc = slab % hchunks, nd = slab / hchunks;
        const int n = nd / g.di, id = nd - n * g.di;
        const int hh0 = hc * hch, hn = min(hch, g.hi - hh0);
        const unsigned inner = (unsigned)hn * g.wi * CV;
        const int d0 = lo_d[id], d1 = hi_d[id];
        const T* dn = dy + (int64_t)n * g.dout * g.ho * g.wo * g.y_ld;
        const int64_t ibase = ((int64_t)nd * g.hi + hh0) * g.wi;
        for (unsigned e = threadIdx.x; e < inner; e += blockDim.x) {
            const unsigned cv = e % CV, pix = e / CV;
            const int iw = pix % g.wi, ih = hh0 + pix / g.wi;
            float acc[VEC];
#pragma unroll
            for (int j = 0; j < VEC; ++j) acc[j] = 0.f;
            const int h0 = lo_h[ih], h1 = hi_h[ih], w0 = lo_w[iw], w1 = hi_w[iw];
            const T* dc = dn + cv * VEC;
            for (int od = d0; od <= d1; ++od) {
                const float wd = up_weight(od, id, g.rd, g.di, g.mode, g.align_corners);
                if (wd == 0.f) continue;
                for (int oh = h0; oh <= h1; ++oh) {
                    const float wh = wd * up_weight(oh, ih, g.rh, g.hi, g.mode, g.align_corners);
                    if (wh == 0.f) continue;
                    for (int ow = w0; ow <= w1; ++ow) {
                        const float w = wh * up_weight(ow, iw, g.rw, g.wi, g.mode, g.align_corners);
                        if (w == 0.f) continue;
                        V<VEC> gv;
                        gv.load(dc + (((int64_t)od * g.ho + oh) * g.wo + ow) * g.y_ld);
#pragma unroll
                        for (int j = 0; j < VEC; ++j) acc[j] = fmaf(w, gv.v[j], acc[j]);
                    }
                }
            }
            V<VEC> o;
#pragma unroll
            for (int j = 0; j < VEC; ++j) o.v[j] = acc[j];
            o.store(dx + (ibase + pix) * g.x_ld + cv * VEC);
        }
    }
// ... 219 lines not shown
                sf.y = fmaf(wh[bb], r.y, sf.y);
                sf.z = fmaf(wh[bb], r.z, sf.z);
                sf.w = fmaf(wh[bb], r.w, sf.w);
            }
            const int i = f >> 1;
            float wdi[4];
            up2_axis_weights(i, g.di, wdi);
            if (f & 1) {
                if (i >= d0) { accA.x = fmaf(wdi[2], sf.x, accA.x); accA.y = fmaf(wdi[2], sf.y, accA.y);
                               accA.z = fmaf(wdi[2], sf.z, accA.z); accA.w = fmaf(wdi[2], sf.w, accA.w); }
                float wn[4];
                up2_axis_weights(i + 1, g.di, wn);
                if (i >= d0) { accB.x = wn[0] * sf.x; accB.y = wn[0] * sf.y; accB.z = wn[0] * sf.z; accB.w = wn[0] * sf.w; }
                else { accA.x = wn[0] * sf.x; accA.y = wn[0] * sf.y; accA.z = wn[0] * sf.z; accA.w = wn[0] * sf.w; }
            } else {
                if (i > d0) {
                    float wp[4];
                    up2_axis_weights(i - 1, g.di, wp);
                    accA.x = fmaf(wp[3], sf.x, accA.x); accA.y = fmaf(wp[3], sf.y, accA.y);
                    accA.z = fmaf(wp[3], sf.z, accA.z); accA.w = fmaf(wp[3], sf.w, accA.w);
                    if (vok) stf4(dxo + (int64_t)(i - 1) * xplane, accA);
                    accA = accB;
                }
                if (i < d1) { accA.x = fmaf(wdi[1], sf.x, accA.x); accA.y = fmaf(wdi[1], sf.y, accA.y);
                              accA.z = fmaf(wdi[1], sf.z, accA.z); accA.w = fmaf(wdi[1], sf.w, accA.w); }
            }
            if (f < f1) stash((f + 1) & 1);
            __syncthreads();
        }
        if (d1 == g.di && vok) stf4(dxo + (int64_t)(d1 - 1) * xplane, accA);
    }
}

constexpr int UTH = 4, UTW = 16;
constexpr int UHH = UTH + 2, UHW = UTW + 2, UHV = UHH * UHW;
constexpr int UMD = 16;

template <typename T, int VEC, int NPV>
__global__ void __launch_bounds__(256)
upsample2x_fwd_march_kernel(Mri3dUpGeom g, const T* __restrict__ x, T* __restrict__ y, int segsD, int segl, int tilesH,
                            int tilesW, int cpasses, int nitems) {
    constexpr int PCH = VEC * NPV;
    constexpr int NST = (UHV * NPV + 255) / 256;
    __shared__ __attribute__((aligned(16))) float cbuf[2][UHV * NPV * VEC];
    const int tid = threadIdx.x;
    const int per_xcd = (nitems + 7) / 8;
    for (int b = blockIdx.x; b < per_xcd * 8; b += gridDim.x) {
        const int item = (b % 8) * per_xcd + b / 8;
        if (item >= nitems) continue;
        int t = item;
        const int c0 = (t % cpasses) * PCH;
        t /= cpasses;
        const int w0 = (t % tilesW) * UTW;
        t /= tilesW;
        const int h0 = (t % tilesH) * UTH;
        t /= tilesH;
        const int d0 = (t % segsD) * segl;
        const int n = t / segsD;
        const int d1 = min(d0 + segl, g.di);
        const T* xn = x + (int64_t)n * g.di * g.hi * g.wi * g.x_ld + c0;
        const int xplane = g.hi * g.wi * g.x_ld;
        int soff[NST];
#pragma unroll
        for (int j = 0; j < NST; ++j) {
            const int idx = min(j * 256 + tid, UHV * NPV - 1);
            const int pc = idx % NPV, hv = idx / NPV;
            const int fw = hv % UHW, fh = hv / UHW;
            const int ch = min(max(h0 - 1 + fh, 0), g.hi - 1), cw = min(max(w0 - 1 + fw, 0), g.wi - 1);
            soff[j] = (ch * g.wi + cw) * g.x_ld + (c0 + pc * VEC < g.c ? pc * VEC : 0);
        }
        V<VEC> sv[NST];
        auto fetch = [&](int c) {
            const T* pl = xn + (int64_t)min(max(c, 0), g.di - 1) * xplane;
#pragma unroll
            for (int j = 0; j < NST; ++j) sv[j].load(pl + soff[j]);
        };
        auto stash = [&](int buf) {
#pragma unroll
            for (int j = 0; j < NST; ++j) {
                const int idx = j * 256 + tid;
                if (j < NST - 1 || idx < UHV * NPV) {
#pragma unroll
                    for (int e = 0; e < VEC; e += 4)
                        *reinterpret_cast<float4*>(&cbuf[buf][idx * VEC + e]) = make_float4(sv[j].v[e], sv[j].v[e + 1], sv[j].v[e + 2], sv[j].v[e + 3]);
                }
            }
        };
        int ia[NPV], ib[NPV], ic[NPV], id[NPV], yoff[NPV];
        unsigned okm = 0;
#pragma unroll
        for (int k = 0; k < NPV; ++k) {
            const int it = k * 256 + tid;
            const int pc = it % NPV, pos = it / NPV;
            const int fwl = pos % (2 * UTW), fhl = pos / (2 * UTW);
            const int hw0 = (fwl >> 1) + 1, hw1 = hw0 + ((fwl & 1) ? 1 : -1), hh0 = (fhl >> 1) + 1, hh1 = hh0 + ((fhl & 1) ? 1 : -1);
            ia[k] = ((hh0 * UHW + hw0) * NPV + pc) * VEC;
            ib[k] = ((hh0 * UHW + hw1) * NPV + pc) * VEC;
            ic[k] = ((hh1 * UHW + hw0) * NPV + pc) * VEC;
            id[k] = ((hh1 * UHW + hw1) * NPV + pc) * VEC;
            const int oh = 2 * h0 + fhl, ow = 2 * w0 + fwl;
            const bool ok = oh < g.ho && ow < g.wo && c0 + pc * VEC < g.c;
            okm |= ok ? (1u << k) : 0u;
            yoff[k] = ok ? (oh * g.wo + ow) * g.y_ld + c0 + pc * VEC : 0;
        }
        T* yn = y + (int64_t)n * g.dout * g.ho * g.wo * g.y_ld;
        const int64_t yplane = (int64_t)g.ho * g.wo * g.y_ld;

        __syncthreads();
        fetch(d0 - 1);
        stash(0);
        __syncthreads();
        V<VEC> pp[NPV];
        for (int c = d0 - 1; c <= d1; ++c) {
            const int buf = (c - (d0 - 1)) & 1;
            if (c < d1) fetch(c + 1);
#pragma unroll
            for (int k = 0; k < NPV; ++k) {
                V<VEC> pc_;
#pragma unroll
                for (int e = 0; e < VEC; e += 4) {
                    const float4 a = *reinterpret_cast<const float4*>(&cbuf[buf][ia[k] + e]);
                    const float4 bq = *reinterpret_cast<const float4*>(&cbuf[buf][ib[k] + e]);
                    const float4 cq = *reinterpret_cast<const float4*>(&cbuf[buf][ic[k] + e]);
                    const float4 dq = *reinterpret_cast<const float4*>(&cbuf[buf][id[k] + e]);
                    pc_.v[e + 0] = 0.75f * fmaf(0.75f, a.x, 0.25f * bq.x) + 0.25f * fmaf(0.75f, cq.x, 0.25f * dq.x);
                    pc_.v[e + 1] = 0.75f * fmaf(0.75f, a.y, 0.25f * bq.y) + 0.25f * fmaf(0.75f, cq.y, 0.25f * dq.y);
                    pc_.v[e + 2] = 0.75f * fmaf(0.75f, a.z, 0.25f * bq.z) + 0.25f * fmaf(0.75f, cq.z, 0.25f * dq.z);
                    pc_.v[e + 3] = 0.75f * fmaf(0.75f, a.w, 0.25f * bq.w) + 0.25f * fmaf(0.75f, cq.w, 0.25f * dq.w);
                }
                if (c >= d0 && ((okm >> k) & 1u)) {
                    V<VEC> o;
                    if (c > d0) {
#pragma unroll
                        for (int e = 0; e < VEC; ++e) o.v[e] = fmaf(0.75f, pp[k].v[e], 0.25f * pc_.v[e]);
                        o.store(yn + (int64_t)(2 * c - 1) * yplane + yoff[k]);
                    }
                    if (c < d1) {
#pragma unroll
                        for (int e = 0; e < VEC; ++e) o.v[e] = fmaf(0.75f, pc_.v[e], 0.25f * pp[k].v[e]);
                        o.store(yn + (int64_t)(2 * c) * yplane + yoff[k]);
                    }
                }
                pp[k] = pc_;
            }
            if (c < d1) stash(buf ^ 1);
            __syncthreads();
        }
    }
}

static inline bool up2x_fast_ok(const Mri3dUpGeom& g) {
    return g.mode == MRI3D_UP_TRILINEAR && !g.align_corners && g.dout == 2 * g.di && g.ho == 2 * g.hi && g.wo == 2 * g.wi &&
           g.rd == 0.5f && g.rh == 0.5f && g.rw == 0.5f && g.c % 4 == 0 && g.x_ld % 4 == 0 && g.y_ld % 4 == 0;
}

static inline void slab_plan(int nd, int h, int w, int cv, int& hch, int& grid) {
    int64_t per_row = (int64_t)w * cv;
    hch = (int)std::max<int64_t>(1, std::min<int64_t>(h, 2048 / std::max<int64_t>(per_row, 1)));
    int64_t slabs = (int64_t)nd * ((h + hch - 1) / hch);
    grid = (int)std::min<int64_t>(slabs, 8192);
}

static inline bool vec_ok(int dtype, int c, int a_ld, int b_ld, const void* a, const void* b) {
    return c % 4 == 0 && a_ld % 4 == 0 && b_ld % 4 == 0 && aligned_vec4(dtype, a, b);
}

}

using namespace mri3d;

static int pool_check(const Mri3dPoolGeom* g, const char* who) {
    MRI3D_REQUIRE(g != nullptr, MRI3D_EINVAL, "%s: null geometry", who);
    MRI3D_REQUIRE(g->dtype == MRI3D_F32 || g->dtype == MRI3D_BF16, MRI3D_ENOTSUP, "%s: unknown dtype %d", who, g->dtype);
    MRI3D_REQUIRE(g->n > 0 && g->c > 0 && g->di > 0 && g->hi > 0 && g->wi > 0 && g->dout > 0 && g->ho > 0 && g->wo > 0,
                  MRI3D_EINVAL, "%s: empty tensor", who);
    MRI3D_REQUIRE(g->kd * g->kh * g->kw <= 256 && g->kd > 0 && g->kh > 0 && g->kw > 0, MRI3D_ENOTSUP,
                  "%s: window volume must be <= 256", who);
    MRI3D_REQUIRE(g->sd > 0 && g->sh > 0 && g->sw > 0 && g->x_ld >= g->c && g->y_ld >= g->c, MRI3D_EINVAL,
                  "%s: bad stride/pitch", who);
    MRI3D_REQUIRE((g->dout - 1) * g->sd - g->pd < g->di && (g->ho - 1) * g->sh - g->ph < g->hi &&
                      (g->wo - 1) * g->sw - g->pw < g->wi && 2 * g->pd <= g->kd && 2 * g->ph <= g->kh && 2 * g->pw <= g->kw,
                  MRI3D_EINVAL, "%s: output dims inconsistent with input", who);
    return MRI3D_OK;
}

extern "C" int mri3d_maxpool3d_fwd(const Mri3dPoolGeom* g, const void* x, void* y, uint8_t* idx,
                                   mri3d_stream_t stream) {
    int rc = pool_check(g, "maxpool3d_fwd");
    if (rc) return rc;
    MRI3D_REQUIRE(x && y && idx, MRI3D_EINVAL, "maxpool3d_fwd: null pointer");
    hipStream_t s = static_cast<hipStream_t>(stream);
    bool v4 = vec_ok(g->dtype, g->c, g->x_ld, g->y_ld, x, y) && (reinterpret_cast<uintptr_t>(idx) & 3) == 0;
    int hch, grid;
    const bool v8 = v4 && g->dtype == MRI3D_BF16 && g->c % 8 == 0 && g->x_ld % 8 == 0 && g->y_ld % 8 == 0 && aligned16(x, y) &&
                    (reinterpret_cast<uintptr_t>(idx) & 7) == 0;
    slab_plan(g->n * g->dout, g->ho, g->wo, g->c / (v8 ? 8 : (v4 ? 4 : 1)), hch, grid);
    if (v4 && pool2_ok(*g, v8 ? 8 : 4)) {
        slab_plan(g->n * g->dout, g->ho, g->wi, g->c / (v8 ? 8 : 4), hch, grid);
        MRI3D_DISPATCH_DTYPE(g->dtype, T, {
            if constexpr (sizeof(T) == 2) {
                if (v8) hipLaunchKernelGGL((maxpool2_fwd_kernel<T, 8>), dim3(grid), dim3(256), 0, s, *g, (const T*)x, (T*)y, idx, hch);
            }
            if (!v8) hipLaunchKernelGGL((maxpool2_fwd_kernel<T, 4>), dim3(grid), dim3(256), 0, s, *g, (const T*)x, (T*)y, idx, hch);
        });
        return check_launch("maxpool3d_fwd");
    }
    MRI3D_DISPATCH_DTYPE(g->dtype, T, {
        if constexpr (sizeof(T) == 2) {
            if (v8) hipLaunchKernelGGL((maxpool_fwd_kernel<T, 8>), dim3(grid), dim3(256), 0, s, *g, (const T*)x, (T*)y, idx, hch);
        }
        if (v8) {
        } else if (v4)
            hipLaunchKernelGGL((maxpool_fwd_kernel<T, 4>), dim3(grid), dim3(256), 0, s, *g, (const T*)x, (T*)y, idx, hch);
        else
            hipLaunchKernelGGL((maxpool_fwd_kernel<T, 1>), dim3(grid), dim3(256), 0, s, *g, (const T*)x, (T*)y, idx, hch);
    });
    return check_launch("maxpool3d_fwd");
}

static int maxpool_bwd_impl(const Mri3dPoolGeom* g, const void* dy, const uint8_t* idx, const void* addend, int32_t a_ld,
                            void* dx, mri3d_stream_t stream) {
    int rc = pool_check(g, "maxpool3d_bwd");
    if (rc) return rc;
    MRI3D_REQUIRE(dy && dx && idx, MRI3D_EINVAL, "maxpool3d_bwd: null pointer");
    MRI3D_REQUIRE(addend == nullptr || a_ld >= g->c, MRI3D_EINVAL, "maxpool3d_bwd: addend pitch %d < %d channels", a_ld, g->c);
    hipStream_t s = static_cast<hipStream_t>(stream);
    bool v4 = vec_ok(g->dtype, g->c, g->x_ld, g->y_ld, dx, dy) && (reinterpret_cast<uintptr_t>(idx) & 3) == 0 &&
              (addend == nullptr || (a_ld % 4 == 0 && aligned_vec4(g->dtype, addend)));
    int hch, grid;
    const bool v8 = v4 && g->dtype == MRI3D_BF16 && g->c % 8 == 0 && g->x_ld % 8 == 0 && g->y_ld % 8 == 0 && aligned16(dx, dy) &&
                    (reinterpret_cast<uintptr_t>(idx) & 7) == 0 && (addend == nullptr || (a_ld % 8 == 0 && aligned16(addend)));
    slab_plan(g->n * g->di, g->hi, g->wi, g->c / (v8 ? 8 : (v4 ? 4 : 1)), hch, grid);
    MRI3D_DISPATCH_DTYPE(g->dtype, T, {
        if constexpr (sizeof(T) == 2) {
            if (v8) hipLaunchKernelGGL((maxpool_bwd_kernel<T, 8>), dim3(grid), dim3(256), 0, s, *g, (const T*)dy, idx, (T*)dx, hch,
                                       (const T*)addend, a_ld);
        }
        if (v8) {
        } else if (v4)
            hipLaunchKernelGGL((maxpool_bwd_kernel<T, 4>), dim3(grid), dim3(256), 0, s, *g, (const T*)dy, idx, (T*)dx, hch,
                               (const T*)addend, a_ld);
        else
            hipLaunchKernelGGL((maxpool_bwd_kernel<T, 1>), dim3(grid), dim3(256), 0, s, *g, (const T*)dy, idx, (T*)dx, hch,
                               (const T*)addend, a_ld);
    });
    return check_launch("maxpool3d_bwd");
}

extern "C" int mri3d_maxpool3d_bwd(const Mri3dPoolGeom* g, const void* dy, const uint8_t* idx, void* dx,
                                   mri3d_stream_t stream) {
    return maxpool_bwd_impl(g, dy, idx, nullptr, 0, dx, stream);
}

extern "C" int mri3d_maxpool3d_bwd_add(const Mri3dPoolGeom* g, const void* dy, const uint8_t* idx, const void* addend,
                                       int32_t addend_ld, void* dx, mri3d_stream_t stream) {
    MRI3D_REQUIRE(addend != nullptr, MRI3D_EINVAL, "maxpool3d_bwd_add: null addend");
    return maxpool_bwd_impl(g, dy, idx, addend, addend_ld, dx, stream);
}

static int up_check(const Mri3dUpGeom* g, const char* who) {
    MRI3D_REQUIRE(g != nullptr, MRI3D_EINVAL, "%s: null geometry", who);
    MRI3D_REQUIRE(g->dtype == MRI3D_F32 || g->dtype == MRI3D_BF16, MRI3D_ENOTSUP, "%s: unknown dtype %d", who, g->dtype);
    MRI3D_REQUIRE(g->n > 0 && g->c > 0 && g->di > 0 && g->hi > 0 && g->wi > 0 && g->dout > 0 && g->ho > 0 && g->wo > 0,
                  MRI3D_EINVAL, "%s: empty tensor", who);
    MRI3D_REQUIRE(g->mode == MRI3D_UP_NEAREST || g->mode == MRI3D_UP_TRILINEAR, MRI3D_EINVAL, "%s: bad mode %d", who,
                  g->mode);
    MRI3D_REQUIRE(g->x_ld >= g->c && g->y_ld >= g->c, MRI3D_EINVAL, "%s: bad pitch", who);
    MRI3D_REQUIRE(g->rd >= 0.f && g->rh >= 0.f && g->rw >= 0.f, MRI3D_EINVAL, "%s: negative scale", who);
    return MRI3D_OK;
}

extern "C" size_t mri3d_upsample3d_workspace_bytes(const Mri3dUpGeom* g) {
    if (!g) return 0;
    return (size_t)2 * (g->di + g->hi + g->wi) * sizeof(int);
}

extern "C" int mri3d_upsample3d_fwd(const Mri3dUpGeom* g, const void* x, void* y, mri3d_stream_t stream) {
    int rc = up_check(g, "upsample3d_fwd");
    if (rc) return rc;
    MRI3D_REQUIRE(x && y, MRI3D_EINVAL, "upsample3d_fwd: null pointer");
    hipStream_t s = static_cast<hipStream_t>(stream);
    static const int no_fast_f = tuning_knob("MRI3D_UP_GENERIC", 0);
    if (!no_fast_f && up2x_fast_ok(*g) && aligned_vec4(g->dtype, x, y)) {
        const bool oct = g->dtype == MRI3D_BF16 && g->c % 8 == 0 && g->x_ld % 8 == 0 && g->y_ld % 8 == 0 &&
                         ((reinterpret_cast<uintptr_t>(x) | reinterpret_cast<uintptr_t>(y)) & 15) == 0;
        const int vec = oct ? 8 : 4, pieces = g->c / vec;
        const int npv = pieces >= 8 ? 8 : pieces >= 4 ? 4 : pieces >= 2 ? 2 : 1;
        const int mtilesH = cdiv(g->hi, UTH), mtilesW = cdiv(g->wi, UTW), mpasses = cdiv(pieces, npv);
        int segl = UMD;
        while (segl > 4 && (int64_t)g->n * cdiv(g->di, segl) * mpasses * mtilesH * mtilesW < 1024) segl /= 2;
        const int segsD = cdiv(g->di, segl);
        const int64_t items = (int64_t)g->n * segsD * mpasses * mtilesH * mtilesW;
        if (items <= 0x7ffffff0 && (int64_t)g->ho * g->wo * g->y_ld <= 0x7fffffff &&
            (int64_t)g->hi * g->wi * g->x_ld <= 0x7fffffff) {
            const int grid = (int)std::min<int64_t>((items + 7) / 8 * 8, 256 * 4 * 8);
#define MRI3D_UPF(Tv, VECv, NPVv)                                                                                      \
    hipLaunchKernelGGL((upsample2x_fwd_march_kernel<Tv, VECv, NPVv>), dim3(grid), dim3(256), 0, s, *g, (const Tv*)x,  \
                       (Tv*)y, segsD, segl, mtilesH, mtilesW, mpasses, (int)items)
#define MRI3D_UPF_N(Tv, VECv)                                                                                          \
    do {                                                                                                              \
        if (npv == 8) MRI3D_UPF(Tv, VECv, 8);                                                                         \
        else if (npv == 4) MRI3D_UPF(Tv, VECv, 4);                                                                    \
        else if (npv == 2) MRI3D_UPF(Tv, VECv, 2);                                                                    \
        else MRI3D_UPF(Tv, VECv, 1);                                                                                  \
    } while (0)
            if (g->dtype == MRI3D_F32) MRI3D_UPF_N(float, 4);
            else if (oct) MRI3D_UPF_N(bf16_t, 8);
            else MRI3D_UPF_N(bf16_t, 4);
#undef MRI3D_UPF_N
#undef MRI3D_UPF
            return check_launch("upsample3d_fwd(2x march)");
        }
    }
// ... 83 lines not shown
```

mri_epilepsy_diagnosis_amd/nn.py:

```python
import math

import torch
import torch.nn as tnn

from . import ops


class Conv3d(tnn.Conv3d):
    def forward(self, x):
        if self.padding_mode != "zeros" or self.groups != 1 or isinstance(self.padding, str):
            raise NotImplementedError("mri3d Conv3d supports padding_mode='zeros', groups=1, numeric padding")
        return ops.conv3d(x, self.weight, self.bias, self.stride, self.padding, self.dilation)


class ConvTranspose3d(tnn.ConvTranspose3d):
    def forward(self, x, output_size=None):
        if output_size is not None or self.groups != 1 or self.padding_mode != "zeros":
            raise NotImplementedError("mri3d ConvTranspose3d supports groups=1, zero padding, no output_size")
        return ops.conv_transpose3d(x, self.weight, self.bias, self.stride, self.padding, self.output_padding,
                                    self.dilation)


class BayesConv3d(tnn.Module):

    def __init__(self, in_channels, out_channels, kernel_size, stride=1, padding=0, dilation=1, groups=1, bias=True,
                 zero_mean=False, threshold=3):
        super().__init__()
        if in_channels % groups != 0 or out_channels % groups != 0:
            raise ValueError("in_channels and out_channels must be divisible by groups")
        self.in_channels, self.out_channels, self.groups = in_channels, out_channels, groups
        self.kernel_size, self.stride, self.dilation = ops._triple(kernel_size), ops._triple(stride), ops._triple(dilation)
        self.padding = padding if isinstance(padding, str) else ops._triple(padding)
        self.zero_mean, self.threshold = zero_mean, threshold
        self.noise = None
        self.log_alpha = None
        shape = (out_channels, in_channels // groups) + self.kernel_size
        self.mu_weight = tnn.Parameter(torch.empty(shape))
        self.logsigma_weight = tnn.Parameter(torch.empty(shape))
        if bias:
            self.mu_bias = tnn.Parameter(torch.empty(out_channels))
            self.logsigma_bias = tnn.Parameter(torch.empty(out_channels))
        else:
            self.register_parameter("mu_bias", None)
            self.register_parameter("logsigma_bias", None)
        self.reset_parameters()
        if zero_mean:
            self.mu_weight = tnn.Parameter(torch.zeros_like(self.mu_weight))

    def reset_parameters(self):
        with torch.no_grad():
            self.mu_weight.normal_(0, 0.02)
            self.logsigma_weight.fill_(-5)
            if self.mu_bias is not None:
                fan_in = self.mu_weight[0].numel()
                bound = 1 / math.sqrt(fan_in)
                self.mu_bias.uniform_(-bound, bound)
                self.logsigma_bias.uniform_(-bound, bound)

    def output_shape(self, x):
        return (x.shape[0], self.out_channels) + tuple(
            (i + 2 * p - d * (k - 1) - 1) // s + 1
            for i, p, d, k, s in zip(x.shape[2:], self.padding, self.dilation, self.kernel_size, self.stride))

    def extra_repr(self):
        return "%d, %d, kernel_size=%s, stride=%s, padding=%s%s" % (self.in_channels, self.out_channels, self.kernel_size, self.stride,
                                                                    self.padding, "" if self.mu_bias is not None else ", bias=False")

    def forward(self, x):
        if self.groups != 1 or isinstance(self.padding, str):
            raise NotImplementedError("mri3d BayesConv3d supports groups=1, numeric padding")
        eps = self.noise(self.output_shape(x), x.device) if self.noise is not None else None
        y, self.log_alpha = ops.bayes_conv3d(x, self.mu_weight, self.logsigma_weight, self.mu_bias, self.logsigma_bias, self.stride,
                                             self.padding, self.dilation, self.training, self.threshold, eps)
        return y


def _act_spec(act):
    if act is None or isinstance(act, tnn.Identity):
        return None, None, 0.0
    if isinstance(act, tnn.PReLU):
        return "prelu", act.weight, 0.0
    if isinstance(act, tnn.LeakyReLU):
        return "leaky_relu", None, float(act.negative_slope)
    if isinstance(act, tnn.ReLU):
        return "relu", None, 0.0
    raise NotImplementedError("unsupported activation module %r" % (act,))


def fused_norm_act(norm, act, x, out=None):
    kind, alpha, slope = _act_spec(act)
    if norm is None:
        if kind is None and out is None:
            return x
        return ops.norm_act(x, None, None, alpha, None, None, "none", 0.1, 0.0, kind, slope, out)
    if isinstance(norm, tnn.modules.batchnorm._BatchNorm):
        use_batch = norm.training or norm.running_mean is None
        if norm.training and norm.track_running_stats and norm.num_batches_tracked is not None:
            norm.num_batches_tracked.add_(1)
        return ops.norm_act(x, norm.weight, norm.bias, alpha,
                            norm.running_mean if norm.track_running_stats else None,
                            norm.running_var if norm.track_running_stats else None,
                            ("sync" if (norm.training and ops.sync_batchnorm_reducer() is not None) else "batch")
                            if use_batch else "running",
                            norm.momentum, norm.eps, kind, slope, out)
    if isinstance(norm, tnn.modules.instancenorm._InstanceNorm):
        if norm.track_running_stats:
            raise NotImplementedError("InstanceNorm3d(track_running_stats=True) is not supported")
        return ops.norm_act(x, norm.weight, norm.bias, alpha, None, None, "instance", 0.1, norm.eps, kind, slope, out)
    if isinstance(norm, tnn.GroupNorm):
        return ops.norm_act(x, norm.weight, norm.bias, alpha, None, None, "group", 0.1, norm.eps, kind, slope, out,
                            norm.num_channels // norm.num_groups)
    raise NotImplementedError("unsupported normalisation module %r" % (norm,))


def _plain_pointwise(head):
    return (isinstance(head, Conv3d) and tuple(head.kernel_size) == (1, 1, 1) and tuple(head.stride) == (1, 1, 1)
            and tuple(head.dilation) == (1, 1, 1) and head.groups == 1 and head.padding_mode == "zeros"
            and not isinstance(head.padding, str) and tuple(head.padding) == (0, 0, 0))


def fused_norm_act_head(norm, act, x, head):
    if not _plain_pointwise(head):
        return None
    kind, alpha, slope = _act_spec(act)
    cast = ops.autocast_dtype()
    if cast is not None and x.dtype != cast:
        return None
    if norm is None:
        mode, args = "none", (None, None, alpha, None, None, "none", 0.1, 0.0)
    elif isinstance(norm, tnn.modules.batchnorm._BatchNorm):
        use_batch = norm.training or norm.running_mean is None
        if use_batch and norm.training and ops.sync_batchnorm_reducer() is not None:
            return None
        if norm.momentum is None:
            return None
        mode = "batch" if use_batch else "running"
        args = (norm.weight, norm.bias, alpha, norm.running_mean if norm.track_running_stats else None,
                norm.running_var if norm.track_running_stats else None, mode, norm.momentum, norm.eps)
    else:
        return None
    if not ops.norm_act_pointwise_supported(x, head.weight, mode, kind, alpha):
        return None
    if mode != "none" and norm.training and norm.track_running_stats and norm.num_batches_tracked is not None:
        norm.num_batches_tracked.add_(1)
    return ops.norm_act_pointwise(x, head.weight, head.bias, *args, act=kind, slope=slope)


def conv_norm_act(conv, norm, act, x, out=None, head=None):
    wants = (isinstance(norm, tnn.modules.batchnorm._BatchNorm) and (norm.training or norm.running_mean is None)
             and ops.sync_batchnorm_reducer() is None and isinstance(conv, Conv3d) and conv.padding_mode == "zeros"
             and conv.groups == 1 and not isinstance(conv.padding, str))
    if isinstance(x, (tuple, list)):
        xa, xb = x
        plain = (isinstance(conv, Conv3d) and conv.padding_mode == "zeros" and conv.groups == 1 and not isinstance(conv.padding, str)
                 and tuple(conv.stride) == (1, 1, 1) and tuple(conv.dilation) == (1, 1, 1))
        if plain:
            y = ops.conv3d_cat(xa, xb, conv.weight, conv.bias, conv.padding, bn_stats=wants)
        else:
            y = conv(ops.cat_channels([xa, xb]))
    elif wants:
        y = ops.conv3d(x, conv.weight, conv.bias, conv.stride, conv.padding, conv.dilation, bn_stats=True)
    else:
        y = conv(x)
    if head is not None:
        logits = fused_norm_act_head(norm, act, y, head) if out is None else None
        return logits if logits is not None else head(fused_norm_act(norm, act, y, out))
    return fused_norm_act(norm, act, y, out)


class GroupNorm(tnn.GroupNorm):
    def forward(self, x):
        return fused_norm_act(self, None, x)


class BatchNorm3d(tnn.BatchNorm3d):
    def forward(self, x):
        return fused_norm_act(self, None, x)


class InstanceNorm3d(tnn.InstanceNorm3d):
    def forward(self, x):
        return fused_norm_act(self, None, x)


class PReLU(tnn.PReLU):
    def forward(self, x):
        if x.dim() != 5:
            return super().forward(x)
        return fused_norm_act(None, self, x)


class ReLU(tnn.ReLU):
    def forward(self, x):
        if x.dim() != 5:
            return super().forward(x)
        return fused_norm_act(None, self, x)


class LeakyReLU(tnn.LeakyReLU):
    def forward(self, x):
        if x.dim() != 5:
            return super().forward(x)
        return fused_norm_act(None, self, x)


class MaxPool3d(tnn.MaxPool3d):
    def forward(self, x):
        if self.ceil_mode or self.return_indices or self.dilation not in (1, (1, 1, 1)):
            raise NotImplementedError("mri3d MaxPool3d supports floor mode, dilation 1, no indices")
        return ops.max_pool3d(x, self.kernel_size, self.stride, self.padding)

    def forward_with_skip(self, x):
        if self.ceil_mode or self.return_indices or self.dilation not in (1, (1, 1, 1)):
            raise NotImplementedError("mri3d MaxPool3d supports floor mode, dilation 1, no indices")
        return ops.max_pool3d_skip(x, self.kernel_size, self.stride, self.padding)


class Upsample(tnn.Upsample):
    def forward(self, x):
        return ops.upsample3d(x, self.size, self.scale_factor, self.mode, self.align_corners)


class Dropout3d(tnn.Dropout3d):
    def forward(self, x):
        return ops.dropout3d(x, self.p, self.training)


class Flatten(tnn.Module):

    def forward(self, x):
        return x.contiguous(memory_format=torch.contiguous_format).view(x.size(0), -1)


_NORMS = (tnn.modules.batchnorm._BatchNorm, tnn.modules.instancenorm._InstanceNorm)
_ACTS = (tnn.PReLU, tnn.ReLU, tnn.LeakyReLU)


def run_fused(modules, x):
    mods = list(modules)
    i = 0
    while i < len(mods):
        m = mods[i]
        five_d = torch.is_tensor(x) and x.dim() == 5
        if (five_d and i == 0 and isinstance(m, Conv3d) and len(mods) > 2 and isinstance(mods[1], Conv3d) and isinstance(mods[2], Conv3d)
                and ops.conv3d_pair_supported(x, m, mods[1])):
            x = ops.conv3d_pair(x, m, mods[1])
            i += 2
            continue
        if five_d and isinstance(m, Conv3d) and i + 1 < len(mods) and isinstance(mods[i + 1], tnn.BatchNorm3d):
            nxt2 = mods[i + 2] if i + 2 < len(mods) else None
            if isinstance(nxt2, _ACTS):
                x = conv_norm_act(m, mods[i + 1], nxt2, x)
                i += 3
            else:
                x = conv_norm_act(m, mods[i + 1], None, x)
                i += 2
            continue
        if five_d and isinstance(m, (tnn.BatchNorm3d, tnn.InstanceNorm3d, tnn.GroupNorm)):
            nxt = mods[i + 1] if i + 1 < len(mods) else None
            if isinstance(nxt, _ACTS):
                x = fused_norm_act(m, nxt, x)
                i += 2
                continue
            x = fused_norm_act(m, None, x)
        elif five_d and isinstance(m, _ACTS):
            x = fused_norm_act(None, m, x)
        else:
            x = m(x)
        i += 1
    return x


class FusedSequential(tnn.Sequential):
    def forward(self, x):
        return run_fused(self, x)
```

mri_epilepsy_diagnosis_amd/ops.py:

```python
import ctypes
import math

import torch

from . import _lib
from ._lib import (ACT_LEAKY, ACT_NONE, ACT_PRELU, ACT_RELU, BF16, F32, PASS_DGRAD, PASS_FWD, PASS_WGRAD, UP_NEAREST,
                   UP_TRILINEAR, ConvGeom, DiceGeom, NormGeom, PoolGeom, UpGeom, check)

CL3D = torch.channels_last_3d



def _require_device(*ts):
    for t in ts:
        if t is None:
            continue
        if not t.is_cuda:
            raise RuntimeError(
                "mri_epilepsy_diagnosis_amd ops run only on a ROCm device tensor (got %s); there is no CPU fallback"
                % t.device)
        if t.dtype not in (torch.float32, torch.bfloat16):
            raise RuntimeError("mri_epilepsy_diagnosis_amd ops: only float32 / bfloat16 tensors are supported, got %s"
                               % t.dtype)

# ... 959 lines not shown
        else:
            dbeta_k, dgamma_k = dbeta, dgamma
        ws = _workspace(L.mri3d_norm_workspace_bytes(ctypes.byref(g)), x.device)
        with _timed(lambda: "norm_act_bwd c%d vox%d n%d" % (g.c, g.vox, g.n), lambda: {"flops": 0.0, "bytes": 5 * _esz(x) * x.numel()}):
            check(L.mri3d_norm_act_bwd(ctypes.byref(g), 1 if ctx.training_stats else 0, _ptr(x), _ptr(dy), _ptr(mean),
                                       _ptr(invstd), _ptr(gamma), _ptr(beta), _ptr(alpha) if prelu else None, _ptr(dx),
                                       _ptr(dgamma_k), _ptr(dbeta_k), _ptr(dalpha), _ptr(ws), ws.numel(), _stream()),
                  "norm_act_bwd")
        if sync is not None:
            tot = sync.all_reduce(torch.cat([dbeta_k.double(), dgamma_k.double()]))
            cnt = ctx.sync_count
            gam = gamma.double() if gamma is not None else torch.ones(g.c, dtype=torch.float64, device=x.device)
            a0 = (-gam * invstd.double() * tot[:g.c] / cnt).to(torch.float32).contiguous()
            b1 = (-gam * invstd.double() ** 2 * tot[g.c:] / cnt).to(torch.float32).contiguous()
            ones = torch.ones(g.c, dtype=torch.float32, device=x.device)
            corr = _new(x.shape, x)
            ga = NormGeom(g.n, g.vox, g.c, g.c, g.c, 0, ACT_NONE, 1, 0.0, 0.0, 0, g.dtype)
            check(L.mri3d_norm_act_fwd(ctypes.byref(ga), _ptr(x), _ptr(mean), _ptr(ones), _ptr(b1), _ptr(a0), None, _ptr(corr),
                                       _stream()), "norm_act_fwd")
            check(L.mri3d_add_channels(_ptr(dx), _ptr(corr), _ptr(dx), g.n * g.vox, g.c, g.c, g.c, g.c, g.dtype, _stream()),
                  "add_channels")
        return (dx, _sink_done(pg, dgamma, sg), _sink_done(pb, dbeta, sb), _sink_done(pa, dalpha, sa), None, None, None, None,
                None, None, None, None, None, None)


def norm_act(x, gamma=None, beta=None, alpha=None, running_mean=None, running_var=None, stats_mode="batch",
             momentum=0.1, eps=1e-5, act=None, slope=0.01, out=None, group_c=0):
    if momentum is None:
        raise RuntimeError("cumulative moving average (momentum=None) is not supported")
    fused = getattr(x, "_mri3d_bn_stats", None) if stats_mode == "batch" else None
    return _NormActFn.apply(x, gamma, beta, alpha, running_mean, running_var, stats_mode, momentum, eps, act, slope, out,
                            group_c, fused)


def _head_geom(x, x_ld, o_ld, act_code, alpha, slope, eps):
    n, c, d, h, w = x.shape
    alpha_n = alpha.numel() if act_code == ACT_PRELU else 1
    return NormGeom(n, d * h * w, c, x_ld, o_ld, 0, act_code, alpha_n, float(slope), float(eps), 0, _dt(x))


def norm_act_pointwise_supported(x, weight, stats_mode="batch", act=None, alpha=None):
    if stats_mode not in ("batch", "running", "none") or act not in _ACT_CODES:
        return False
    if not (x.is_cuda and x.dim() == 5 and x.dtype in (torch.float32, torch.bfloat16)):
        return False
    if weight.dim() != 5 or tuple(weight.shape[2:]) != (1, 1, 1) or weight.shape[1] != x.shape[1] or weight.dtype != torch.float32:
        return False
    x_ld = _pitch_of(x)
    if x_ld is None:
        x_ld = x.shape[1]
    elif x.data_ptr() % (4 * x.element_size()):
        return False
    g = _head_geom(x, x_ld, weight.shape[0], _ACT_CODES[act], alpha if alpha is not None else weight, 0.0, 0.0)
    return bool(_lib.lib().mri3d_norm_act_pw_supported(ctypes.byref(g), weight.shape[0]))


class _NormActPointwiseFn(torch.autograd.Function):

    @staticmethod
    def forward(ctx, x, gamma, beta, alpha, weight, bias, running_mean, running_var, stats_mode, momentum, eps, act, slope,
                fused_stats=None):
        _require_device(x)
        _require_param(gamma, beta, alpha, weight, bias)
        ctx.params = (gamma, beta, alpha, weight, bias)
        L = _lib.lib()
        x, x_ld = _nd(x)
        n, c, d, h, w = x.shape
        co = weight.shape[0]
        act_code = _ACT_CODES[act]
        wm = weight.contiguous()
        g = _head_geom(x, x_ld, co, act_code, alpha, slope, eps)
        if not L.mri3d_norm_act_pw_supported(ctypes.byref(g), co):
            raise RuntimeError("norm_act_pointwise: c=%d co=%d pitch %d is not served (ask norm_act_pointwise_supported first)"
                               % (c, co, x_ld))
        mean = invstd = None
        gn = _head_geom(x, x_ld, x_ld, act_code, alpha, slope, eps)
        if stats_mode == "batch":
            mean = torch.empty(c, dtype=torch.float32, device=x.device)
            invstd = torch.empty(c, dtype=torch.float32, device=x.device)
            upd = running_mean is not None
            if fused_stats is not None and fused_stats[0].numel() == fused_stats[1] * c * 2:
                part, blocks, shift = fused_stats
                with _timed(lambda: "norm_stats(from conv partials) c%d" % c, lambda: {"flops": 0.0, "bytes": 8.0 * part.numel()}):
                    check(L.mri3d_norm_stats_from_partials(ctypes.byref(gn), _ptr(part), blocks, _ptr(shift), _ptr(mean),
                                                           _ptr(invstd), _ptr(running_mean) if upd else None,
                                                           _ptr(running_var) if upd else None, float(momentum), _stream()),
                          "norm_stats_from_partials")
            else:
                ws = _workspace(L.mri3d_norm_workspace_bytes(ctypes.byref(gn)), x.device)
                with _timed(lambda: "norm_stats c%d vox%d n%d" % (c, g.vox, n), lambda: {"flops": 0.0, "bytes": _esz(x) * x.numel()}):
                    check(L.mri3d_norm_stats(ctypes.byref(gn), _ptr(x), _ptr(mean), _ptr(invstd),
                                             _ptr(running_mean) if upd else None, _ptr(running_var) if upd else None,
                                             float(momentum), _ptr(ws), ws.numel(), _stream()), "norm_stats")
        elif stats_mode == "running":
            mean = running_mean.detach().to(torch.float32).contiguous()
            invstd = torch.rsqrt(running_var.detach().to(torch.float32) + eps).contiguous()
        elif stats_mode != "none":
            raise RuntimeError("norm_act_pointwise: statistics mode %r is not served" % (stats_mode,))
        out = _new((n, co, d, h, w), x)
        with _timed(lambda: "norm_act_pw_fwd c%d->%d vox%d n%d" % (c, co, g.vox, n),
                    lambda: {"flops": 2.0 * co * c * n * g.vox, "bytes": _esz(x) * (x.numel() + out.numel())}):
            check(L.mri3d_norm_act_pw_fwd(ctypes.byref(g), co, _ptr(x), _ptr(mean), _ptr(invstd), _ptr(gamma), _ptr(beta),
                                          _ptr(alpha) if act_code == ACT_PRELU else None, _ptr(wm), _ptr(bias), _ptr(out),
                                          _stream()), "norm_act_pw_fwd")
        ctx.save_for_backward(x, mean, invstd, gamma, beta, alpha, wm)
        ctx.geom = g
        ctx.training_stats = stats_mode == "batch"
        return out

    @staticmethod
    def backward(ctx, dout):
        L = _lib.lib()
        x, mean, invstd, gamma, beta, alpha, wm = ctx.saved_tensors
        g0 = ctx.geom
        co = wm.shape[0]
        dout, o_ld = _nd(dout)
        if dout.dtype != x.dtype:
            raise RuntimeError("norm_act_pointwise backward: gradient dtype %s does not match activation dtype %s" % (dout.dtype, x.dtype))
        if g0.x_ld != g0.c:
            x = x.contiguous(memory_format=CL3D)
        g = NormGeom(g0.n, g0.vox, g0.c, g0.c, o_ld, 0, g0.act, g0.alpha_n, g0.slope, g0.eps, 0, g0.dtype)
        pg, pb, pa, pw, pbias = ctx.params
        prelu = g.act == ACT_PRELU
        need = ctx.needs_input_grad
        want = (gamma is not None and need[1], beta is not None and need[2], prelu and need[3], need[4],
                pbias is not None and need[5])
        srcs = (gamma, beta, alpha, wm, pbias)
        sinks = [_sink_take(p) if wt else None for p, wt in zip(ctx.params, want)]
        grads = [(sk if sk is not None else torch.empty_like(t, memory_format=torch.contiguous_format)) if wt else None
                 for sk, t, wt in zip(sinks, srcs, want)]
        dx = _new(x.shape, x) if need[0] else None
        ws = _workspace(L.mri3d_norm_act_pw_workspace_bytes(ctypes.byref(g), co), x.device)
        reads = 2 if ctx.training_stats else 1
        with _timed(lambda: "norm_act_pw_bwd c%d->%d vox%d n%d" % (g.c, co, g.vox, g.n),
                    lambda: {"flops": 4.0 * co * g.c * g.n * g.vox,
                             "bytes": _esz(x) * (reads * (x.numel() + dout.numel()) + (x.numel() if dx is not None else 0))}):
            check(L.mri3d_norm_act_pw_bwd(ctypes.byref(g), co, 1 if ctx.training_stats else 0, _ptr(x), _ptr(dout), _ptr(mean),
                                          _ptr(invstd), _ptr(gamma), _ptr(beta), _ptr(alpha) if prelu else None, _ptr(wm),
                                          _ptr(dx), _ptr(grads[0]), _ptr(grads[1]), _ptr(grads[2]), _ptr(grads[3]),
                                          _ptr(grads[4]), _ptr(ws), ws.numel(), _stream()), "norm_act_pw_bwd")
        outs = [_sink_done(p, gr, sk) for p, gr, sk in zip(ctx.params, grads, sinks)]
        return (dx, outs[0], outs[1], outs[2], outs[3], outs[4], None, None, None, None, None, None, None, None)


def norm_act_pointwise(x, weight, bias=None, gamma=None, beta=None, alpha=None, running_mean=None, running_var=None,
                       stats_mode="batch", momentum=0.1, eps=1e-5, act=None, slope=0.01):
    if momentum is None:
        raise RuntimeError("cumulative moving average (momentum=None) is not supported")
    fused = getattr(x, "_mri3d_bn_stats", None) if stats_mode == "batch" else None
    return _NormActPointwiseFn.apply(x, gamma, beta, alpha, weight, bias, running_mean, running_var, stats_mode, momentum, eps,
                                     act, slope, fused)


def activation(x, act, alpha=None, slope=0.01):
    return norm_act(x, None, None, alpha, None, None, "none", 0.1, 0.0, act, slope)


class _ScaleInstanceFn(torch.autograd.Function):

    @staticmethod
    def forward(ctx, x, scale):
        _require_device(x)
        _require_param(scale)
        L = _lib.lib()
        x = _cl(x)
        n, c, d, h, w = x.shape
        g = NormGeom(n, d * h * w, c, c, c, 1, ACT_NONE, 1, 0.0, 0.0, 0, _dt(x))
        scale = scale.reshape(n * c).contiguous()
        zeros = torch.zeros_like(scale)
        y = _new(x.shape, x)
        check(L.mri3d_norm_act_fwd(ctypes.byref(g), _ptr(x), _ptr(zeros), _ptr(scale), None, None, None, _ptr(y),
                                   _stream()), "norm_act_fwd")
        ctx.save_for_backward(scale, zeros)
        ctx.geom = g
        return y

    @staticmethod
    def backward(ctx, dy):
        L = _lib.lib()
        scale, zeros = ctx.saved_tensors
        g = ctx.geom
        dy = _cl(dy)
        dx = _new(dy.shape, dy)
        check(L.mri3d_norm_act_fwd(ctypes.byref(g), _ptr(dy), _ptr(zeros), _ptr(scale), None, None, None, _ptr(dx),
                                   _stream()), "norm_act_fwd")
        return dx, None


def dropout3d(x, p, training):
    if not training or p == 0.0:
        return x
    n, c = x.shape[0], x.shape[1]
    keep = torch.empty(n, c, device=x.device, dtype=torch.float32).bernoulli_(1.0 - p)
    return _ScaleInstanceFn.apply(x, keep / (1.0 - p))




def _pool_out(i, k, s, p, ceil_mode):
    if ceil_mode:
        o = -(-(i + 2 * p - k) // s) + 1
        if (o - 1) * s >= i + p:
            o -= 1
        return o
    return (i + 2 * p - k) // s + 1


class _MaxPool3dFn(torch.autograd.Function):
    @staticmethod
    def forward(ctx, x, kernel, stride, padding):
        _require_device(x)
        L = _lib.lib()
        x, x_ld = _nd(x)
        n, c, d, h, w = x.shape
        do, ho, wo = (_pool_out(i, k, s, p, False) for i, k, s, p in zip((d, h, w), kernel, stride, padding))
        if do <= 0 or ho <= 0 or wo <= 0:
            raise RuntimeError("max_pool3d: output size is too small (input %s, kernel %s)" % ((d, h, w), kernel))
        g = PoolGeom(n, d, h, w, do, ho, wo, c, *kernel, *stride, *padding, x_ld, c, _dt(x))
        y = _new((n, c, do, ho, wo), x)
        idx = torch.empty(n * do * ho * wo * c, dtype=torch.uint8, device=x.device)
        with _timed(lambda: "maxpool_fwd c%d" % c, lambda: {"flops": 0.0, "bytes": _esz(x) * x.numel() + (_esz(x) + 1) * y.numel()}):
            check(L.mri3d_maxpool3d_fwd(ctypes.byref(g), _ptr(x), _ptr(y), _ptr(idx), _stream()), "maxpool3d_fwd")
        ctx.save_for_backward(idx)
        ctx.geom = g
        ctx.xshape = tuple(x.shape)
        return y

    @staticmethod
    def backward(ctx, dy):
        L = _lib.lib()
        (idx,) = ctx.saved_tensors
        dy, dy_ld = _nd(dy)
        dx = _new(ctx.xshape, dy)
        g0 = ctx.geom
        g = PoolGeom(g0.n, g0.di, g0.hi, g0.wi, g0.dout, g0.ho, g0.wo, g0.c, g0.kd, g0.kh, g0.kw, g0.sd, g0.sh, g0.sw,
                     g0.pd, g0.ph, g0.pw, g0.c, dy_ld, _dt(dy))
        with _timed(lambda: "maxpool_bwd c%d" % g.c, lambda: {"flops": 0.0, "bytes": _esz(dy) * dx.numel() + (_esz(dy) + 1) * dy.numel()}):
            check(L.mri3d_maxpool3d_bwd(ctypes.byref(g), _ptr(dy), _ptr(idx), _ptr(dx), _stream()), "maxpool3d_bwd")
        return dx, None, None, None


class _MaxPoolSkipFn(torch.autograd.Function):

    @staticmethod
    def forward(ctx, x, kernel, stride, padding):
        y = _MaxPool3dFn.forward(ctx, x, kernel, stride, padding)
        return y, x.view_as(x)

    @staticmethod
    def backward(ctx, dy, dskip):
        if dskip is None:
            return _MaxPool3dFn.backward(ctx, dy)
        if dy is None:
            return dskip, None, None, None
        L = _lib.lib()
        (idx,) = ctx.saved_tensors
        dy, dy_ld = _nd(dy)
        dskip, ds_ld = _nd(dskip)
        if tuple(dskip.shape) != ctx.xshape or dskip.dtype != dy.dtype:
            raise RuntimeError("max_pool3d_skip backward: skip gradient %s %s does not match the input %s %s"
                               % (tuple(dskip.shape), dskip.dtype, ctx.xshape, dy.dtype))
        dx = _new(ctx.xshape, dy)
        g0 = ctx.geom
        g = PoolGeom(g0.n, g0.di, g0.hi, g0.wi, g0.dout, g0.ho, g0.wo, g0.c, g0.kd, g0.kh, g0.kw, g0.sd, g0.sh, g0.sw,
                     g0.pd, g0.ph, g0.pw, g0.c, dy_ld, _dt(dy))
        with _timed(lambda: "maxpool_bwd+skip c%d" % g.c, lambda: {"flops": 0.0, "bytes": _esz(dy) * 2 * dx.numel() + (_esz(dy) + 1) * dy.numel()}):
            check(L.mri3d_maxpool3d_bwd_add(ctypes.byref(g), _ptr(dy), _ptr(idx), _ptr(dskip), ds_ld, _ptr(dx), _stream()),
                  "maxpool3d_bwd_add")
        return dx, None, None, None


def max_pool3d_skip(x, kernel_size, stride=None, padding=0):
    k = _triple(kernel_size)
    s = _triple(stride) if stride is not None else k
    return _MaxPoolSkipFn.apply(x, k, s, _triple(padding))


def max_pool3d(x, kernel_size, stride=None, padding=0):
    k = _triple(kernel_size)
    s = _triple(stride) if stride is not None else k
    return _MaxPool3dFn.apply(x, k, s, _triple(padding))




class _Upsample3dFn(torch.autograd.Function):
    @staticmethod
    def forward(ctx, x, out_size, mode, align_corners, ratios, out):
        _require_device(x)
        L = _lib.lib()
        x, x_ld = _nd(x)
        n, c, d, h, w = x.shape
        do, ho, wo = out_size
        if out is None:
            y, y_ld = _new((n, c, do, ho, wo), x), c
        else:
            buf, y_off = out
            y_ld = _pitch_of(buf)
            if (y_ld != buf.shape[1] or tuple(buf.shape[2:]) != (do, ho, wo) or buf.shape[0] != n
                    or y_off + c > buf.shape[1] or buf.dtype != x.dtype):
                raise RuntimeError("upsample3d(out=): buffer %s cannot hold a %s slice at channel %d"
                                   % (tuple(buf.shape), (n, c, do, ho, wo), y_off))
            y = _slice_view(buf, y_off, c)
        g = UpGeom(n, d, h, w, do, ho, wo, c, x_ld, y_ld, mode, 1 if align_corners else 0, ratios[0], ratios[1], ratios[2],
                   _dt(x))
        with _timed(lambda: "upsample_fwd c%d" % c, lambda: {"flops": 0.0, "bytes": _esz(x) * (x.numel() + y.numel())}):
# ... 314 lines not shown
```

mri_epilepsy_diagnosis_amd/unet/unet.py:

```python
import torch
import torch.nn as tnn

from .. import nn as mnn
from .. import ops

_UPSAMPLING = {"nearest": "nearest", "linear": "trilinear", "trilinear": "trilinear"}


class ConvolutionalBlock(tnn.Module):
    def __init__(self, dimensions, in_channels, out_channels, normalization=None, kernel_size=3, activation="ReLU",
                 preactivation=False, padding=0, padding_mode="zeros", dilation=None, dropout=0):
        super().__init__()
        if dimensions != 3:
            raise NotImplementedError("only the 3-D U-Net of the reference is implemented")
        if preactivation or padding_mode != "zeros" or dropout:
            raise NotImplementedError("preactivation / non-zero padding_mode / dropout are not used by the reference")
        dilation = 1 if dilation is None else dilation
        if padding:
            total = kernel_size + 2 * (dilation - 1) - 1
            padding = total // 2
        conv = mnn.Conv3d(in_channels, out_channels, kernel_size, padding=padding, dilation=dilation)
        norm = None
        if normalization is not None:
            norm = {"batch": mnn.BatchNorm3d, "instance": mnn.InstanceNorm3d}[normalization.lower()](out_channels)
        act = None
        if activation is not None:
            act = {"PReLU": mnn.PReLU, "ReLU": mnn.ReLU, "LeakyReLU": mnn.LeakyReLU}[activation]()
        self.conv_layer = conv
        self.norm_layer = norm
        self.activation_layer = act
        self.dropout_layer = None
        self.block = tnn.Sequential(*[m for m in (conv, norm, act) if m is not None])

    def forward(self, x, out=None, head=None):
        return mnn.conv_norm_act(self.conv_layer, self.norm_layer, self.activation_layer, x, out, head)


class EncodingBlock(tnn.Module):
    def __init__(self, in_channels, out_channels_first, dimensions, normalization, pooling_type, preactivation=False,
                 is_first_block=False, residual=False, padding=0, padding_mode="zeros", activation="ReLU",
                 dilation=None, dropout=0):
        super().__init__()
        if residual:
            raise NotImplementedError("residual encoding blocks are not used by the reference")
        self.conv1 = ConvolutionalBlock(dimensions, in_channels, out_channels_first,
                                        normalization=None if is_first_block else normalization,
                                        padding=padding, activation=activation, dilation=dilation)
        out_channels_second = 2 * out_channels_first
        self.conv2 = ConvolutionalBlock(dimensions, out_channels_first, out_channels_second, normalization=normalization,
                                        padding=padding, activation=activation, dilation=dilation)
        self.downsample = None
        if pooling_type is not None:
            if pooling_type != "max":
                raise NotImplementedError("only max pooling is used by the reference")
            self.downsample = mnn.MaxPool3d(kernel_size=2)

    def forward(self, x, skip_out=None, head=None):
        if self.downsample is None:
            return self.conv2(self.conv1(x), skip_out, head)
        x = self.conv2(self.conv1(x), skip_out)
        return self.downsample.forward_with_skip(x)

    @property
    def out_channels(self):
        return self.conv2.conv_layer.out_channels


class Encoder(tnn.Module):
    def __init__(self, in_channels, out_channels_first, dimensions, pooling_type, num_encoding_blocks, normalization,
                 padding=0, activation="ReLU", initial_dilation=None):
        super().__init__()
        self.encoding_blocks = tnn.ModuleList()
        self.dilation = initial_dilation
        first = True
        for _ in range(num_encoding_blocks):
            blk = EncodingBlock(in_channels, out_channels_first, dimensions, normalization, pooling_type,
                                is_first_block=first, padding=padding, activation=activation, dilation=self.dilation)
            first = False
            self.encoding_blocks.append(blk)
            in_channels = 2 * out_channels_first
            out_channels_first = in_channels
            if self.dilation is not None:
                self.dilation *= 2

    def forward(self, x, cat_bufs=None):
        skips = []
        for i, blk in enumerate(self.encoding_blocks):
            x, skip = blk(x, None if cat_bufs is None else (cat_bufs[i], 0))
            skips.append(skip)
        return skips, x

    @property
    def out_channels(self):
        return self.encoding_blocks[-1].out_channels


class DecodingBlock(tnn.Module):
    def __init__(self, in_channels_skip_connection, dimensions, upsampling_type, normalization, padding=0,
                 activation="ReLU", dilation=None):
        super().__init__()
        if upsampling_type == "conv":
            c = 2 * in_channels_skip_connection
            self.upsample = mnn.ConvTranspose3d(c, c, kernel_size=2, stride=2)
        else:
            mode = _UPSAMPLING[upsampling_type]
            self.upsample = mnn.Upsample(scale_factor=2, mode=mode, align_corners=False if mode == "trilinear" else None)
        in_first = in_channels_skip_connection * 3
        self.conv1 = ConvolutionalBlock(dimensions, in_first, in_channels_skip_connection, normalization=normalization,
                                        padding=padding, activation=activation, dilation=dilation)
        self.conv2 = ConvolutionalBlock(dimensions, in_channels_skip_connection, in_channels_skip_connection,
                                        normalization=normalization, padding=padding, activation=activation,
                                        dilation=dilation)

    def forward(self, skip, x, cat_buf=None, head=None):
        if cat_buf is not None and isinstance(self.upsample, mnn.Upsample):
            up = ops.upsample3d(x, self.upsample.size, self.upsample.scale_factor, self.upsample.mode,
                                self.upsample.align_corners, out=(cat_buf, skip.shape[1]))
            return self.conv2(self.conv1(ops.join_channels(cat_buf, [skip, up])), head=head)
        x = self.upsample(x)
        if skip.shape[2:] != x.shape[2:]:
            raise NotImplementedError("padding=False (centre-cropped skips) is not used by the reference")
        return self.conv2(self.conv1((skip, x)), head=head)


class Decoder(tnn.Module):
    def __init__(self, in_channels_skip_connection, dimensions, upsampling_type, num_decoding_blocks, normalization,
                 padding=0, activation="ReLU", initial_dilation=None):
        super().__init__()
        self.decoding_blocks = tnn.ModuleList()
        self.dilation = initial_dilation
        for _ in range(num_decoding_blocks):
            self.decoding_blocks.append(DecodingBlock(in_channels_skip_connection, dimensions, upsampling_type,
                                                      normalization, padding=padding, activation=activation,
                                                      dilation=self.dilation))
            in_channels_skip_connection //= 2
            if self.dilation is not None:
                self.dilation //= 2

    def forward(self, skips, x, cat_bufs=None, head=None):
        last = min(len(skips), len(self.decoding_blocks)) - 1
        for j, (skip, blk) in enumerate(zip(reversed(skips), self.decoding_blocks)):
            x = blk(skip, x, None if cat_bufs is None else cat_bufs[len(skips) - 1 - j], head if j == last else None)
        return x


class UNet(tnn.Module):
    def __init__(self, in_channels=1, out_classes=2, dimensions=2, num_encoding_blocks=5, out_channels_first_layer=64,
                 normalization=None, pooling_type="max", upsampling_type="conv", preactivation=False, residual=False,
                 padding=0, padding_mode="zeros", activation="ReLU", initial_dilation=None, dropout=0,
                 monte_carlo_dropout=0):
        super().__init__()
        if dimensions != 3:
            raise NotImplementedError("only dimensions=3 (the reference's configuration) is implemented")
        if preactivation or residual or dropout or monte_carlo_dropout or padding_mode != "zeros":
            raise NotImplementedError("option not used by the reference and not implemented")
        if not padding:
            raise NotImplementedError("padding=False (valid convolutions + cropped skips) is not used by the reference")
        depth = num_encoding_blocks - 1
        self.encoder = Encoder(in_channels, out_channels_first_layer, dimensions, pooling_type, depth, normalization,
                               padding=padding, activation=activation, initial_dilation=initial_dilation)
        c = self.encoder.out_channels if depth > 0 else in_channels
        first = c if depth > 0 else out_channels_first_layer
        self.bottom_block = EncodingBlock(c, first, dimensions, normalization, pooling_type=None, padding=padding,
                                          activation=activation, dilation=self.encoder.dilation,
                                          is_first_block=depth == 0)
        skip_channels = out_channels_first_layer * 2 ** depth
        self.decoder = Decoder(skip_channels, dimensions, upsampling_type, depth, normalization, padding=padding,
                               activation=activation, initial_dilation=self.encoder.dilation)
        self.monte_carlo_layer = None
        self.shared_concat_buffers = False
        self.fused_head = True
        self.classifier = ConvolutionalBlock(dimensions, 2 * out_channels_first_layer, out_classes, kernel_size=1,
                                             activation=None)

    def forward(self, x):
        cat_bufs = None
        if self.shared_concat_buffers and x.is_cuda and len(self.encoder.encoding_blocks) and all(
                isinstance(b.upsample, mnn.Upsample) for b in self.decoder.decoding_blocks):
            cat_bufs = []
            n, sp = x.shape[0], tuple(x.shape[2:])
            for blk in self.encoder.encoding_blocks:
                if any(s % 2 for s in sp):
                    cat_bufs = None
                    break
                cat_bufs.append(ops.new_cat_buffer(n, 3 * blk.out_channels, sp, x))
                sp = tuple(s // 2 for s in sp)
        clf = self.classifier
        head = clf.conv_layer if (self.fused_head and x.is_cuda and clf.norm_layer is None and clf.activation_layer is None
                                  and clf.dropout_layer is None) else None
        skips, enc = self.encoder(x, cat_bufs)
        if not skips:
            return self.bottom_block(enc, head=head) if head is not None else self.classifier(self.bottom_block(enc))
        enc = self.bottom_block(enc)
        x = self.decoder(skips, enc, cat_bufs, head)
        return x if head is not None else self.classifier(x)
```

Before: 67.60 volumes/s.

## Fuse BatchNorm+PReLU with 2x2x2 max-pool in encoder blocks forward and backward

Adds a fused kernel that applies the normalization and activation, writes the skip tensor, and computes the 2x2x2 max-pool with argmax indices in a single pass. The backward pass combines the skip gradient with the scattered pool gradient inside the existing norm-act backward body, so no separate maxpool backward or add pass is needed. The goal is fewer full-resolution activation reads and writes and fewer launches in the encoder. In exchange it adds a templated path with lane shuffles for the pooling reduction and NaN and tie handling that must match the existing pool semantics.

After: 68.56 volumes/s, median of 6. +1.4%, better.

```diff
diff --git a/include/mri3d.h b/include/mri3d.h
--- a/include/mri3d.h
+++ b/include/mri3d.h
@@ -128,6 +128,16 @@
 int mri3d_maxpool3d_bwd(const Mri3dPoolGeom* g, const void* dy, const uint8_t* idx, void* dx, mri3d_stream_t stream);
 int mri3d_maxpool3d_bwd_add(const Mri3dPoolGeom* g, const void* dy, const uint8_t* idx, const void* addend,
                             int32_t addend_ld, void* dx, mri3d_stream_t stream);
+
+int32_t mri3d_norm_act_pool_supported(const Mri3dNormGeom* g, const Mri3dPoolGeom* pg);
+size_t mri3d_norm_act_pool_workspace_bytes(const Mri3dNormGeom* g, const Mri3dPoolGeom* pg);
+int mri3d_norm_act_pool_fwd(const Mri3dNormGeom* g, const Mri3dPoolGeom* pg, const void* x, const float* mean,
+                            const float* invstd, const float* gamma, const float* beta, const float* alpha, void* skip,
+                            void* pooled, uint8_t* idx, mri3d_stream_t stream);
+int mri3d_norm_act_pool_bwd(const Mri3dNormGeom* g, const Mri3dPoolGeom* pg, int training, const void* x, const void* dskip,
+                            const void* dpool, const uint8_t* idx, const float* mean, const float* invstd, const float* gamma,
+                            const float* beta, const float* alpha, void* dx, float* dgamma, float* dbeta, float* dalpha,
+                            void* workspace, size_t ws_bytes, mri3d_stream_t stream);
 
 typedef struct Mri3dUpGeom {
     int32_t n, di, hi, wi, dout, ho, wo, c;
diff --git a/mri_epilepsy_diagnosis_amd/_lib.py b/mri_epilepsy_diagnosis_amd/_lib.py
--- a/mri_epilepsy_diagnosis_amd/_lib.py
+++ b/mri_epilepsy_diagnosis_amd/_lib.py
@@ -84,7 +84,12 @@
     "mri3d_maxpool3d_fwd": (c_int32, [POINTER(PoolGeom), _P, _P, _P, _P]),
     "mri3d_maxpool3d_bwd": (c_int32, [POINTER(PoolGeom), _P, _P, _P, _P]),
     "mri3d_maxpool3d_bwd_add": (c_int32, [POINTER(PoolGeom), _P, _P, _P, c_int32, _P, _P]),
-    "mri3d_upsample3d_workspace_bytes": (c_size_t, [POINTER(UpGeom)]),
+    "mri3d_norm_act_pool_supported": (c_int32, [POINTER(NormGeom), POINTER(PoolGeom)]),
+    "mri3d_norm_act_pool_workspace_bytes": (c_size_t, [POINTER(NormGeom), POINTER(PoolGeom)]),
+    "mri3d_norm_act_pool_fwd": (c_int32, [POINTER(NormGeom), POINTER(PoolGeom), _P, _FP, _FP, _FP, _FP, _FP, _P, _P, _P, _P]),
+    "mri3d_norm_act_pool_bwd": (c_int32, [POINTER(NormGeom), POINTER(PoolGeom), c_int32, _P, _P, _P, _P, _FP, _FP, _FP, _FP,
+                                          _FP, _P, _FP, _FP, _FP, _P, c_size_t, _P]),
+    "mri3d_upsample3d_workspace_bytes":(c_size_t, [POINTER(UpGeom)]),
     "mri3d_upsample3d_fwd": (c_int32, [POINTER(UpGeom), _P, _P, _P]),
     "mri3d_upsample3d_bwd": (c_int32, [POINTER(UpGeom), _P, _P, _P, c_size_t, _P]),
     "mri3d_softmax_dice_workspace_bytes": (c_size_t, [POINTER(DiceGeom)]),
diff --git a/mri_epilepsy_diagnosis_amd/csrc/common.h b/mri_epilepsy_diagnosis_amd/csrc/common.h
--- a/mri_epilepsy_diagnosis_amd/csrc/common.h
+++ b/mri_epilepsy_diagnosis_amd/csrc/common.h
@@ -4,6 +4,7 @@
 #include <stdio.h>
 #include <stdarg.h>
 #include <stdlib.h>
+#include <algorithm>
 #include "../../include/mri3d.h"
 
 namespace mri3d {
@@ -97,6 +98,20 @@
         }                                    \
     } while (0)
 
+inline void slab_plan(int nd, int h, int w, int cv, int& hch, int& grid) {
+    int64_t per_row = (int64_t)w * cv;
+    hch = (int)std::max<int64_t>(1, std::min<int64_t>(h, 2048 / std::max<int64_t>(per_row, 1)));
+    int64_t slabs = (int64_t)nd * ((h + hch - 1) / hch);
+    grid = (int)std::min<int64_t>(slabs, 8192);
+}
+
+inline bool pool2_ok(const Mri3dPoolGeom& g, int vec) {
+    const int cv = g.c / vec;
+    return g.kd == 2 && g.kh == 2 && g.kw == 2 && g.sd == 2 && g.sh == 2 && g.sw == 2 && g.pd == 0 && g.ph == 0 && g.pw == 0 &&
+           g.di == 2 * g.dout && g.hi == 2 * g.ho && g.wi == 2 * g.wo && cv >= 1 && cv <= 32 && (cv & (cv - 1)) == 0 &&
+           (int64_t)g.di * g.hi * g.wi * g.x_ld < ((int64_t)1 << 31);
+}
+
 __device__ __forceinline__ float wave_sum(float v) {
 #pragma unroll
     for (int off = 32; off > 0; off >>= 1) v += __shfl_xor(v, off, 64);
diff --git a/mri_epilepsy_diagnosis_amd/csrc/norm.hip b/mri_epilepsy_diagnosis_amd/csrc/norm.hip
--- a/mri_epilepsy_diagnosis_amd/csrc/norm.hip
+++ b/mri_epilepsy_diagnosis_amd/csrc/norm.hip
@@ -546,9 +546,10 @@
     else return v;
 }
 
-__device__ __forceinline__ void nap_fwd_consts(const NapArgs& p, int c0, float (&sc)[4], float (&sh)[4], float (&al)[4]) {
-#pragma unroll
-    for (int j = 0; j < 4; ++j) {
+template <int VEC>
+__device__ __forceinline__ void nap_fwd_consts(const NapArgs& p, int c0, float (&sc)[VEC], float (&sh)[VEC], float (&al)[VEC]) {
+#pragma unroll
+    for (int j = 0; j < VEC; ++j) {
         int c = c0 + j;
         float gm = p.gamma ? p.gamma[c] : 1.f;
         float bt = p.beta ? p.beta[c] : 0.f;
@@ -618,7 +619,9 @@
         const float* w;
         int Co, ld;
     };
-    static constexpr int kCo = CO;
+    struct Val {
+        float g[CO];
+    };
     static constexpr int kSide = 5 * CO;
     const T* dout;
     int Co, ld;
@@ -636,11 +639,12 @@
             for (int j = 0; j < 4; ++j) dw[j][co] = 0.0;
         }
     }
-    __device__ __forceinline__ void load(int64_t v, float (&gv)[CO]) const {
-#pragma unroll
-        for (int co = 0; co < CO; ++co) gv[co] = co < Co ? ldf(dout + v * ld + co) : 0.f;
-    }
-    __device__ __forceinline__ void grad(const float (&gv)[CO], float (&da)[4]) const {
+    __device__ __forceinline__ void load(int64_t v, Val& val) const {
+#pragma unroll
+        for (int co = 0; co < CO; ++co) val.g[co] = co < Co ? ldf(dout + v * ld + co) : 0.f;
+    }
+    __device__ __forceinline__ void grad(const Val& val, float (&da)[4]) const {
+        const float (&gv)[CO] = val.g;
         float4 acc = make_float4(0.f, 0.f, 0.f, 0.f);
 #pragma unroll
         for (int co = 0; co < CO; ++co) {
@@ -652,7 +656,8 @@
         da[0] = through_storage<T>(acc.x), da[1] = through_storage<T>(acc.y);
         da[2] = through_storage<T>(acc.z), da[3] = through_storage<T>(acc.w);
     }
-    __device__ __forceinline__ void side(const float (&a)[4], const float (&gv)[CO], bool lead) {
+    __device__ __forceinline__ void side(const float (&a)[4], const Val& val, bool lead) {
+        const float (&gv)[CO] = val.g;
 #pragma unroll
         for (int co = 0; co < CO; ++co) {
 #pragma unroll
@@ -685,10 +690,10 @@
 };
 
 template <typename T, class SRC, bool SUMS, bool DX>
-__global__ void __launch_bounds__(256)
-norm_act_src_bwd_kernel(const T* __restrict__ x, T* __restrict__ dx, typename SRC::Args sa, NapArgs p,
-                        const float* __restrict__ sums, int training, double* __restrict__ part, double* __restrict__ spart,
-                        float* __restrict__ dgamma, float* __restrict__ dbeta, float* __restrict__ dalpha) {
+__device__ __forceinline__ void
+norm_act_src_bwd_body(const T* __restrict__ x, T* __restrict__ dx, const typename SRC::Args& sa, const NapArgs& p,
+                      const float* __restrict__ sums, int training, double* __restrict__ part, double* __restrict__ spart,
+                      float* __restrict__ dgamma, float* __restrict__ dbeta, float* __restrict__ dalpha) {
     constexpr int kRed = SUMS ? (SRC::kSide > 12 ? SRC::kSide : 12) : 1;
     __shared__ double red[256 * kRed];
     if (!SUMS && (dgamma != nullptr || dbeta != nullptr || dalpha != nullptr) && blockIdx.x == 0)
@@ -718,13 +723,13 @@
         }
     }
     float sc[4], sh[4], af[4];
-    if constexpr (SUMS) nap_fwd_consts(p, c0, sc, sh, af);
+    if constexpr (SUMS && SRC::kSide > 0) nap_fwd_consts(p, c0, sc, sh, af);
     SRC src;
     src.init(sa, p.C, q);
     double s0[4], s1[4], s2[4];
 #pragma unroll
     for (int j = 0; j < 4; ++j) { s0[j] = 0.0; s1[j] = 0.0; s2[j] = 0.0; }
-    auto row = [&](const float (&xv)[4], const float (&gv)[SRC::kCo], int64_t v) {
+    auto row = [&](const float (&xv)[4], const typename SRC::Val& gv, int64_t v) {
         float da[4], ov[4];
         src.grad(gv, da);
 #pragma unroll
@@ -740,7 +745,7 @@
             }
             if constexpr (DX) ov[j] = fmaf(k0[j], du, -k1[j]) - xh * k2[j];
         }
-        if constexpr (SUMS) {
+        if constexpr (SUMS && SRC::kSide > 0) {
             float a[4];
 #pragma unroll
             for (int j = 0; j < 4; ++j) a[j] = through_storage<T>(apply_act(fmaf(xv[j], sc[j], sh[j]), p.act, af[j]));
@@ -751,7 +756,8 @@
     const int64_t step = (int64_t)gridDim.x * VT;
     int64_t v = (int64_t)blockIdx.x * VT + vt;
     for (; v + step < p.nvox; v += 2 * step) {
-        float xa[4], xb[4], ga[SRC::kCo], gb[SRC::kCo];
+        float xa[4], xb[4];
+        typename SRC::Val ga, gb;
         Ld<4>::load(x + v * p.x_ld + c0, xa);
         src.load(v, ga);
         Ld<4>::load(x + (v + step) * p.x_ld + c0, xb);
@@ -760,7 +766,8 @@
         row(xb, gb, v + step);
     }
     for (; v < p.nvox; v += step) {
-        float xv[4], gv[SRC::kCo];
+        float xv[4];
+        typename SRC::Val gv;
         Ld<4>::load(x + v * p.x_ld + c0, xv);
         src.load(v, gv);
         row(xv, gv, v);
@@ -788,9 +795,19 @@
                 o[2] = d;
             }
         }
-        __syncthreads();
-        src.flush(red, spart, p.C, QC, VT);
-    }
+        if constexpr (SRC::kSide > 0) {
+            __syncthreads();
+            src.flush(red, spart, p.C, QC, VT);
+        }
+    }
+}
+
+template <typename T, class SRC, bool SUMS, bool DX>
+__global__ void __launch_bounds__(256)
+norm_act_src_bwd_kernel(const T* __restrict__ x, T* __restrict__ dx, typename SRC::Args sa, NapArgs p,
+                        const float* __restrict__ sums, int training, double* __restrict__ part, double* __restrict__ spart,
+                        float* __restrict__ dgamma, float* __restrict__ dbeta, float* __restrict__ dalpha) {
+    norm_act_src_bwd_body<T, SRC, SUMS, DX>(x, dx, sa, p, sums, training, part, spart, dgamma, dbeta, dalpha);
 }
 
 __global__ void __launch_bounds__(256)
@@ -814,6 +831,141 @@
             dbias[i - nw] = (float)t;
         }
     }
+}
+
+template <typename T, int VEC>
+__global__ void __launch_bounds__(256)
+norm_act_pool_fwd_kernel(Mri3dPoolGeom g, const T* __restrict__ x, T* __restrict__ skip, T* __restrict__ y,
+                         uint8_t* __restrict__ idx, int hch, NapArgs p) {
+    const unsigned CV = g.c / VEC;
+    const int hchunks = (g.ho + hch - 1) / hch;
+    const int slabs = g.n * g.dout * hchunks;
+    const unsigned xrow = (unsigned)g.wi * p.x_ld, xplane = (unsigned)g.hi * xrow;
+    const unsigned srow = (unsigned)g.wi * g.x_ld, splane = (unsigned)g.hi * srow;
+    const unsigned cv = threadIdx.x % CV;
+    float sc[VEC], sh[VEC], al[VEC];
+    nap_fwd_consts(p, (int)cv * VEC, sc, sh, al);
+    for (int slab = blockIdx.x; slab < slabs; slab += gridDim.x) {
+        const int hc = slab % hchunks, nd = slab / hchunks;
+        const int n = nd / g.dout, od = nd - n * g.dout;
+        const int h0 = hc * hch, hn = min(hch, g.ho - h0);
+        const unsigned inner = (unsigned)hn * g.wi * CV;
+        const int64_t sample = ((int64_t)n * g.di + 2 * od) * g.hi * g.wi;
+        const T* xs = x + sample * p.x_ld;
+        T* ss = skip + sample * g.x_ld;
+        const int64_t obase = ((int64_t)nd * g.ho + h0) * g.wo;
+        for (unsigned e0 = 0; e0 < inner; e0 += blockDim.x) {
+            const unsigned e = e0 + threadIdx.x;
+            const bool live = e < inner;
+            const unsigned col = (live ? e : 0) / CV;
+            const unsigned iw = col % g.wi, ohl = col / g.wi;
+            const unsigned kw = iw & 1, ow = iw >> 1, oh = h0 + ohl;
+            const T* xp = xs + (2 * oh) * xrow + iw * (unsigned)p.x_ld + cv * VEC;
+            T* sp = ss + (2 * oh) * srow + iw * (unsigned)g.x_ld + cv * VEC;
+            float v[4][VEC];
+#pragma unroll
+            for (int t = 0; t < 4; ++t) Ld<VEC>::load(xp + (t >> 1) * xplane + (t & 1) * xrow, v[t]);
+#pragma unroll
+            for (int t = 0; t < 4; ++t) {
+#pragma unroll
+                for (int j = 0; j < VEC; ++j) v[t][j] = through_storage<T>(apply_act(fmaf(v[t][j], sc[j], sh[j]), p.act, al[j]));
+                if (live) Ld<VEC>::store(sp + (t >> 1) * splane + (t & 1) * srow, v[t]);
+            }
+            float best[VEC];
+            int bi[VEC];
+#pragma unroll
+            for (int j = 0; j < VEC; ++j) { best[j] = v[0][j]; bi[j] = (int)kw; }
+#pragma unroll
+            for (int t = 1; t < 4; ++t)
+#pragma unroll
+                for (int j = 0; j < VEC; ++j)
+                    if (v[t][j] > best[j] || v[t][j] != v[t][j]) { best[j] = v[t][j]; bi[j] = 2 * t + (int)kw; }
+            float o[VEC];
+            int oi[VEC];
+#pragma unroll
+            for (int j = 0; j < VEC; ++j) {
+                const float pb = __shfl_xor(best[j], (int)CV, 64);
+                const int pi = __shfl_xor(bi[j], (int)CV, 64);
+                const bool mine_nan = best[j] != best[j], his_nan = pb != pb;
+                bool take_his;
+                if (mine_nan || his_nan) take_his = his_nan && (!mine_nan || pi > bi[j]);
+                else take_his = pb > best[j] || (pb == best[j] && pi < bi[j]);
+                o[j] = take_his ? pb : best[j];
+                oi[j] = take_his ? pi : bi[j];
+            }
+            if (live && kw == 0) {
+                const int64_t ov = obase + (int64_t)ohl * g.wo + ow;
+                Ld<VEC>::store(y + ov * g.y_ld + cv * VEC, o);
+                uint8_t* ip = idx + ov * g.c + cv * VEC;
+                if constexpr (VEC == 8) {
+                    uint2 pk;
+                    pk.x = (uint32_t)oi[0] | ((uint32_t)oi[1] << 8) | ((uint32_t)oi[2] << 16) | ((uint32_t)oi[3] << 24);
+                    pk.y = (uint32_t)oi[4] | ((uint32_t)oi[5] << 8) | ((uint32_t)oi[6] << 16) | ((uint32_t)oi[7] << 24);
+                    *reinterpret_cast<uint2*>(ip) = pk;
+                } else {
+                    *reinterpret_cast<uint32_t*>(ip) = (uint32_t)oi[0] | ((uint32_t)oi[1] << 8) | ((uint32_t)oi[2] << 16) | ((uint32_t)oi[3] << 24);
+                }
+            }
+        }
+    }
+}
+
+template <typename T>
+struct PoolSkipGrad {
+    struct Args {
+        const T *dskip, *dpool;
+        const uint8_t* idx;
+        int s_ld, p_ld;
+        unsigned wi, hi;
+    };
+    struct Val {
+        float ds[4], dp[4];
+        uint32_t ib, tap;
+    };
+    static constexpr int kSide = 0;
+    Args a;
+    int C, c0;
+
+    __device__ __forceinline__ void init(const Args& args, int C_, int q) { a = args, C = C_, c0 = 4 * q; }
+    __device__ __forceinline__ void load(int64_t v, Val& val) const {
+        if (a.dskip != nullptr) {
+            Ld<4>::load(a.dskip + v * a.s_ld + c0, val.ds);
+        } else {
+#pragma unroll
+            for (int j = 0; j < 4; ++j) val.ds[j] = 0.f;
+        }
+        val.ib = 0, val.tap = 0xff;
+        if (a.dpool != nullptr) {
+            const unsigned u = (unsigned)v;
+            const unsigned r = u / a.wi, w = u - r * a.wi;
+            const unsigned nd = r / a.hi, h = r - nd * a.hi;
+            const int64_t pv = ((int64_t)(nd >> 1) * (a.hi >> 1) + (h >> 1)) * (a.wi >> 1) + (w >> 1);
+            Ld<4>::load(a.dpool + pv * a.p_ld + c0, val.dp);
+            val.ib = *reinterpret_cast<const uint32_t*>(a.idx + pv * C + c0);
+            val.tap = ((nd & 1) * 2 + (h & 1)) * 2 + (w & 1);
+        } else {
+#pragma unroll
+            for (int j = 0; j < 4; ++j) val.dp[j] = 0.f;
+        }
+    }
+    __device__ __forceinline__ void grad(const Val& val, float (&da)[4]) const {
+#pragma unroll
+        for (int j = 0; j < 4; ++j) {
+            float acc = val.ds[j];
+            if (((val.ib >> (8 * j)) & 0xff) == val.tap) acc += val.dp[j];
+            da[j] = through_storage<T>(acc);
+        }
+    }
+    __device__ __forceinline__ void side(const float (&)[4], const Val&, bool) {}
+    __device__ __forceinline__ void flush(double*, double* __restrict__, int, int, int) const {}
+};
+
+template <typename T, bool SUMS, bool DX>
+__global__ void __launch_bounds__(256)
+norm_act_pool_bwd_kernel(const T* __restrict__ x, T* __restrict__ dx, typename PoolSkipGrad<T>::Args sa, NapArgs p,
+                         const float* __restrict__ sums, int training, double* __restrict__ part,
+                         float* __restrict__ dgamma, float* __restrict__ dbeta, float* __restrict__ dalpha) {
+    norm_act_src_bwd_body<T, PoolSkipGrad<T>, SUMS, DX>(x, dx, sa, p, sums, training, part, nullptr, dgamma, dbeta, dalpha);
 }
 
 struct NapPlan {
@@ -1124,3 +1276,111 @@
     });
     return check_launch("norm_act_pw_bwd");
 }
+
+static bool napool_supported(const Mri3dNormGeom& g, const Mri3dPoolGeom& pg) {
+    if (!nap_supported(g, 1) || g.y_ld < g.c || g.y_ld % 4 != 0) return false;
+    if (pg.dtype != g.dtype || pg.n != g.n || pg.c != g.c || pg.x_ld != g.y_ld || pg.y_ld < g.c || pg.y_ld % 4 != 0) return false;
+    if (pg.di <= 0 || pg.hi <= 0 || pg.wi <= 0 || (int64_t)pg.di * pg.hi * pg.wi != g.vox) return false;
+    if (!pool2_ok(pg, 4)) return false;
+    const int64_t ld = g.x_ld > g.y_ld ? g.x_ld : g.y_ld;
+    if (g.vox * ld >= ((int64_t)1 << 31)) return false;
+    if ((int64_t)g.n * g.vox >= ((int64_t)1 << 31)) return false;
+    return true;
+}
+
+extern "C" int32_t mri3d_norm_act_pool_supported(const Mri3dNormGeom* g, const Mri3dPoolGeom* pg) {
+    return (g != nullptr && pg != nullptr && napool_supported(*g, *pg)) ? 1 : 0;
+}
+
+extern "C" size_t mri3d_norm_act_pool_workspace_bytes(const Mri3dNormGeom* g, const Mri3dPoolGeom* pg) {
+    if (g == nullptr || pg == nullptr || !napool_supported(*g, *pg)) return 0;
+    return nap_plan(*g, 0).bytes;
+}
+
+extern "C" int mri3d_norm_act_pool_fwd(const Mri3dNormGeom* g, const Mri3dPoolGeom* pg, const void* x, const float* mean,
+                                       const float* invstd, const float* gamma, const float* beta, const float* alpha,
+                                       void* skip, void* pooled, uint8_t* idx, mri3d_stream_t stream) {
+    MRI3D_REQUIRE(g != nullptr && pg != nullptr, MRI3D_EINVAL, "norm_act_pool_fwd: null geometry");
+    MRI3D_REQUIRE(napool_supported(*g, *pg), MRI3D_ENOTSUP,
+                  "norm_act_pool_fwd: c=%d x_ld=%d y_ld=%d instance=%d pool %dx%dx%d/%d -> %dx%dx%d not served", g->c, g->x_ld,
+                  g->y_ld, g->instance, pg->di, pg->hi, pg->wi, pg->kd, pg->dout, pg->ho, pg->wo);
+    MRI3D_REQUIRE(x && skip && pooled && idx, MRI3D_EINVAL, "norm_act_pool_fwd: null pointer");
+    MRI3D_REQUIRE((mean == nullptr) == (invstd == nullptr), MRI3D_EINVAL, "norm_act_pool_fwd: mean/invstd must both be set");
+    MRI3D_REQUIRE(g->act != MRI3D_ACT_PRELU || alpha, MRI3D_EINVAL, "norm_act_pool_fwd: PReLU needs alpha");
+    MRI3D_REQUIRE(aligned_vec4(g->dtype, x, skip, pooled) && (reinterpret_cast<uintptr_t>(idx) & 3) == 0, MRI3D_EINVAL,
+                  "norm_act_pool_fwd: x, skip, pooled and idx must be aligned to 4 elements");
+    hipStream_t s = static_cast<hipStream_t>(stream);
+    const NapArgs a = nap_args(*g, mean, invstd, gamma, beta, alpha);
+    const bool v8 = g->dtype == MRI3D_BF16 && g->c % 8 == 0 && g->x_ld % 8 == 0 && g->y_ld % 8 == 0 && pg->y_ld % 8 == 0 &&
+                    aligned16(x, skip, pooled) && (reinterpret_cast<uintptr_t>(idx) & 7) == 0;
+    int hch, grid;
+    slab_plan(pg->n * pg->dout, pg->ho, pg->wi, pg->c / (v8 ? 8 : 4), hch, grid);
+    MRI3D_DISPATCH_DTYPE(g->dtype, T, {
+        if constexpr (sizeof(T) == 2) {
+            if (v8)
+                hipLaunchKernelGGL((norm_act_pool_fwd_kernel<T, 8>), dim3(grid), dim3(256), 0, s, *pg, (const T*)x, (T*)skip,
+                                   (T*)pooled, idx, hch, a);
+        }
+        if (!v8)
+            hipLaunchKernelGGL((norm_act_pool_fwd_kernel<T, 4>), dim3(grid), dim3(256), 0, s, *pg, (const T*)x, (T*)skip, (T*)pooled,
+                               idx, hch, a);
+    });
+    return check_launch("norm_act_pool_fwd");
+}
+
+template <typename T>
+static void napool_bwd_launch(const Mri3dNormGeom& g, const Mri3dPoolGeom& pg, int training, const T* x, const T* dskip,
+                              const T* dpool, const uint8_t* idx, T* dx, float* dgamma, float* dbeta, float* dalpha,
+                              const NapArgs& a, const NapPlan& p, char* ws, hipStream_t s) {
+    const typename PoolSkipGrad<T>::Args sa = {dskip, dpool, idx, g.y_ld, pg.y_ld, (unsigned)pg.wi, (unsigned)pg.hi};
+    double* part = reinterpret_cast<double*>(ws + p.part_off);
+    float* sums = reinterpret_cast<float*>(ws + p.sums_off);
+    const dim3 grid(p.nblk), blk(256);
+    const bool params = dgamma || dbeta || dalpha;
+    const bool need_sums = training || params;
+    if (need_sums) {
+        if (training || dx == nullptr)
+            hipLaunchKernelGGL((norm_act_pool_bwd_kernel<T, true, false>), grid, blk, 0, s, x, dx, sa, a, sums, training, part,
+                               dgamma, dbeta, dalpha);
+        else
+            hipLaunchKernelGGL((norm_act_pool_bwd_kernel<T, true, true>), grid, blk, 0, s, x, dx, sa, a, sums, training, part,
+                               dgamma, dbeta, dalpha);
+        hipLaunchKernelGGL(norm_act_bwd_sums_kernel, dim3(cdiv(g.c, 256 / kFinQL)), dim3(256), 0, s, part, sums, g.c, p.nblk, 1);
+        if (params && !(training && dx != nullptr))
+            hipLaunchKernelGGL(norm_act_bwd_params_kernel, dim3(1), dim3(256), 0, s, sums, dgamma, dbeta, dalpha, g.alpha_n, g.c,
+                               1);
+    }
+    if (dx != nullptr && (training || !need_sums))
+        hipLaunchKernelGGL((norm_act_pool_bwd_kernel<T, false, true>), grid, blk, 0, s, x, dx, sa, a, sums, training, part, dgamma,
+                           dbeta, dalpha);
+}
+
+extern "C" int mri3d_norm_act_pool_bwd(const Mri3dNormGeom* g, const Mri3dPoolGeom* pg, int training, const void* x,
+                                       const void* dskip, const void* dpool, const uint8_t* idx, const float* mean,
+                                       const float* invstd, const float* gamma, const float* beta, const float* alpha, void* dx,
+                                       float* dgamma, float* dbeta, float* dalpha, void* workspace, size_t ws_bytes,
+                                       mri3d_stream_t stream) {
+    MRI3D_REQUIRE(g != nullptr && pg != nullptr, MRI3D_EINVAL, "norm_act_pool_bwd: null geometry");
+    MRI3D_REQUIRE(napool_supported(*g, *pg), MRI3D_ENOTSUP,
+                  "norm_act_pool_bwd: c=%d x_ld=%d y_ld=%d instance=%d pool %dx%dx%d/%d -> %dx%dx%d not served", g->c, g->x_ld,
+                  g->y_ld, g->instance, pg->di, pg->hi, pg->wi, pg->kd, pg->dout, pg->ho, pg->wo);
+    MRI3D_REQUIRE(x != nullptr, MRI3D_EINVAL, "norm_act_pool_bwd: null pointer");
+    MRI3D_REQUIRE(dpool == nullptr || idx != nullptr, MRI3D_EINVAL, "norm_act_pool_bwd: dpool needs the index bytes");
+    MRI3D_REQUIRE((mean == nullptr) == (invstd == nullptr), MRI3D_EINVAL, "norm_act_pool_bwd: mean/invstd must both be set");
+    MRI3D_REQUIRE(!(training && mean == nullptr), MRI3D_EINVAL, "norm_act_pool_bwd: training mode needs statistics");
+    MRI3D_REQUIRE(g->act != MRI3D_ACT_PRELU || alpha, MRI3D_EINVAL, "norm_act_pool_bwd: PReLU needs alpha");
+    MRI3D_REQUIRE(aligned_vec4(g->dtype, x, dx) && aligned_vec4(g->dtype, dskip, dpool) &&
+                      (reinterpret_cast<uintptr_t>(idx) & 3) == 0,
+                  MRI3D_EINVAL, "norm_act_pool_bwd: x, dx, dskip, dpool and idx must be aligned to 4 elements");
+    const NapPlan p = nap_plan(*g, 0);
+    MRI3D_REQUIRE(workspace && ws_bytes >= p.bytes && (reinterpret_cast<uintptr_t>(workspace) & 7) == 0, MRI3D_EWORKSPACE,
+                  "norm_act_pool_bwd: workspace %zu < %zu (or not 8-byte aligned)", ws_bytes, p.bytes);
+    hipStream_t s = static_cast<hipStream_t>(stream);
+    const NapArgs a = nap_args(*g, mean, invstd, gamma, beta, alpha);
+    char* ws = static_cast<char*>(workspace);
+    MRI3D_DISPATCH_DTYPE(g->dtype, T, {
+        napool_bwd_launch<T>(*g, *pg, training, (const T*)x, (const T*)dskip, (const T*)dpool, idx, (T*)dx, dgamma, dbeta, dalpha, a,
+                             p, ws, s);
+    });
+    return check_launch("norm_act_pool_bwd");
+}
diff --git a/mri_epilepsy_diagnosis_amd/csrc/resample.hip b/mri_epilepsy_diagnosis_amd/csrc/resample.hip
--- a/mri_epilepsy_diagnosis_amd/csrc/resample.hip
+++ b/mri_epilepsy_diagnosis_amd/csrc/resample.hip
@@ -229,13 +229,6 @@
             }
         }
     }
-}
-
-static inline bool pool2_ok(const Mri3dPoolGeom& g, int vec) {
-    const int cv = g.c / vec;
-    return g.kd == 2 && g.kh == 2 && g.kw == 2 && g.sd == 2 && g.sh == 2 && g.sw == 2 && g.pd == 0 && g.ph == 0 && g.pw == 0 &&
-           g.di == 2 * g.dout && g.hi == 2 * g.ho && g.wi == 2 * g.wo && cv >= 1 && cv <= 32 && (cv & (cv - 1)) == 0 &&
-           (int64_t)g.di * g.hi * g.wi * g.x_ld < ((int64_t)1 << 31);
 }
 
 struct Lin { int i0, i1; float l0, l1; };
@@ -761,13 +754,6 @@
 static inline bool up2x_fast_ok(const Mri3dUpGeom& g) {
     return g.mode == MRI3D_UP_TRILINEAR && !g.align_corners && g.dout == 2 * g.di && g.ho == 2 * g.hi && g.wo == 2 * g.wi &&
            g.rd == 0.5f && g.rh == 0.5f && g.rw == 0.5f && g.c % 4 == 0 && g.x_ld % 4 == 0 && g.y_ld % 4 == 0;
-}
-
-static inline void slab_plan(int nd, int h, int w, int cv, int& hch, int& grid) {
-    int64_t per_row = (int64_t)w * cv;
-    hch = (int)std::max<int64_t>(1, std::min<int64_t>(h, 2048 / std::max<int64_t>(per_row, 1)));
-    int64_t slabs = (int64_t)nd * ((h + hch - 1) / hch);
-    grid = (int)std::min<int64_t>(slabs, 8192);
 }
 
 static inline bool vec_ok(int dtype, int c, int a_ld, int b_ld, const void* a, const void* b) {
diff --git a/mri_epilepsy_diagnosis_amd/nn.py b/mri_epilepsy_diagnosis_amd/nn.py
--- a/mri_epilepsy_diagnosis_amd/nn.py
+++ b/mri_epilepsy_diagnosis_amd/nn.py
@@ -119,26 +119,31 @@
             and not isinstance(head.padding, str) and tuple(head.padding) == (0, 0, 0))
 
 
+def _local_stats_spec(norm, act):
+    kind, alpha, slope = _act_spec(act)
+    if norm is None:
+        return "none", (None, None, alpha, None, None, "none", 0.1, 0.0), kind, alpha, slope
+    if not isinstance(norm, tnn.modules.batchnorm._BatchNorm) or norm.momentum is None:
+        return None
+    use_batch = norm.training or norm.running_mean is None
+    if use_batch and norm.training and ops.sync_batchnorm_reducer() is not None:
+        return None
+    mode = "batch" if use_batch else "running"
+    args = (norm.weight, norm.bias, alpha, norm.running_mean if norm.track_running_stats else None,
+            norm.running_var if norm.track_running_stats else None, mode, norm.momentum, norm.eps)
+    return mode, args, kind, alpha, slope
+
+
 def fused_norm_act_head(norm, act, x, head):
     if not _plain_pointwise(head):
         return None
-    kind, alpha, slope = _act_spec(act)
     cast = ops.autocast_dtype()
     if cast is not None and x.dtype != cast:
         return None
-    if norm is None:
-        mode, args = "none", (None, None, alpha, None, None, "none", 0.1, 0.0)
-    elif isinstance(norm, tnn.modules.batchnorm._BatchNorm):
-        use_batch = norm.training or norm.running_mean is None
-        if use_batch and norm.training and ops.sync_batchnorm_reducer() is not None:
-            return None
-        if norm.momentum is None:
-            return None
-        mode = "batch" if use_batch else "running"
-        args = (norm.weight, norm.bias, alpha, norm.running_mean if norm.track_running_stats else None,
-                norm.running_var if norm.track_running_stats else None, mode, norm.momentum, norm.eps)
-    else:
-        return None
+    spec = _local_stats_spec(norm, act)
+    if spec is None:
+        return None
+    mode, args, kind, alpha, slope = spec
     if not ops.norm_act_pointwise_supported(x, head.weight, mode, kind, alpha):
         return None
     if mode != "none" and norm.training and norm.track_running_stats and norm.num_batches_tracked is not None:
@@ -146,7 +151,24 @@
     return ops.norm_act_pointwise(x, head.weight, head.bias, *args, act=kind, slope=slope)
 
 
-def conv_norm_act(conv, norm, act, x, out=None, head=None):
+def fused_norm_act_pool(norm, act, x, pool):
+    if (not isinstance(pool, tnn.MaxPool3d) or pool.ceil_mode or pool.return_indices or pool.dilation not in (1, (1, 1, 1))
+            or not x.is_cuda):
+        return None
+    if x.dtype != torch.float32:
+        return None
+    spec = _local_stats_spec(norm, act)
+    if spec is None:
+        return None
+    mode, args, kind, alpha, slope = spec
+    if not ops.norm_act_pool_supported(x, pool.kernel_size, pool.stride, pool.padding, mode, kind, alpha):
+        return None
+    if mode != "none" and norm.training and norm.track_running_stats and norm.num_batches_tracked is not None:
+        norm.num_batches_tracked.add_(1)
+    return ops.norm_act_pool(x, *args, act=kind, slope=slope)
+
+
+def conv_norm_act(conv, norm, act, x, out=None, head=None, pool=None):
     wants = (isinstance(norm, tnn.modules.batchnorm._BatchNorm) and (norm.training or norm.running_mean is None)
              and ops.sync_batchnorm_reducer() is None and isinstance(conv, Conv3d) and conv.padding_mode == "zeros"
              and conv.groups == 1 and not isinstance(conv.padding, str))
@@ -165,6 +187,9 @@
     if head is not None:
         logits = fused_norm_act_head(norm, act, y, head) if out is None else None
         return logits if logits is not None else head(fused_norm_act(norm, act, y, out))
+    if pool is not None:
+        both = fused_norm_act_pool(norm, act, y, pool) if out is None else None
+        return both if both is not None else pool.forward_with_skip(fused_norm_act(norm, act, y, out))
     return fused_norm_act(norm, act, y, out)
 
 
diff --git a/mri_epilepsy_diagnosis_amd/ops.py b/mri_epilepsy_diagnosis_amd/ops.py
--- a/mri_epilepsy_diagnosis_amd/ops.py
+++ b/mri_epilepsy_diagnosis_amd/ops.py
@@ -1135,6 +1135,146 @@
                                      act, slope, fused)
 
 
+def _pool_tail_geoms(x, x_ld, s_ld, p_ld, kernel, stride, padding, act_code, alpha, slope, eps):
+    n, c, d, h, w = x.shape
+    do, ho, wo = (_pool_out(i, k, s, p, False) for i, k, s, p in zip((d, h, w), kernel, stride, padding))
+    alpha_n = alpha.numel() if (act_code == ACT_PRELU and alpha is not None) else 1
+    g = NormGeom(n, d * h * w, c, x_ld, s_ld, 0, act_code, alpha_n, float(slope), float(eps), 0, _dt(x))
+    pg = PoolGeom(n, d, h, w, do, ho, wo, c, *kernel, *stride, *padding, s_ld, c if p_ld is None else p_ld, _dt(x))
+    return g, pg, (do, ho, wo)
+
+
+def norm_act_pool_supported(x, kernel_size=2, stride=None, padding=0, stats_mode="batch", act=None, alpha=None):
+    if stats_mode not in ("batch", "running", "none") or act not in _ACT_CODES:
+        return False
+    if not (x.dim() == 5 and x.dtype in (torch.float32, torch.bfloat16)):
+        return False
+    k = _triple(kernel_size)
+    s = _triple(stride) if stride is not None else k
+    x_ld = _pitch_of(x)
+    if x_ld is None:
+        x_ld = x.shape[1]
+    elif x.data_ptr() % (4 * x.element_size()):
+        return False
+    g, pg, out = _pool_tail_geoms(x, x_ld, x.shape[1], None, k, s, _triple(padding), _ACT_CODES[act], alpha, 0.0, 0.0)
+    if min(out) <= 0:
+        return False
+    return bool(_lib.lib().mri3d_norm_act_pool_supported(ctypes.byref(g), ctypes.byref(pg)))
+
+
+class _NormActPoolFn(torch.autograd.Function):
+
+    @staticmethod
+    def forward(ctx, x, gamma, beta, alpha, running_mean, running_var, stats_mode, momentum, eps, act, slope, fused_stats=None):
+        _require_device(x)
+        _require_param(gamma, beta, alpha)
+        ctx.params = (gamma, beta, alpha)
+        L = _lib.lib()
+        x, x_ld = _nd(x)
+        n, c, d, h, w = x.shape
+        act_code = _ACT_CODES[act]
+        two = (2, 2, 2)
+        g, pg, (do, ho, wo) = _pool_tail_geoms(x, x_ld, c, c, two, two, (0, 0, 0), act_code, alpha, slope, eps)
+        if not L.mri3d_norm_act_pool_supported(ctypes.byref(g), ctypes.byref(pg)):
+            raise RuntimeError("norm_act_pool: c=%d pitch %d extents %s is not served (ask norm_act_pool_supported first)"
+                               % (c, x_ld, (d, h, w)))
+        mean = invstd = None
+        gn = _head_geom(x, x_ld, x_ld, act_code, alpha, slope, eps)
+        if stats_mode == "batch":
+            mean = torch.empty(c, dtype=torch.float32, device=x.device)
+            invstd = torch.empty(c, dtype=torch.float32, device=x.device)
+            upd = running_mean is not None
+            if fused_stats is not None and fused_stats[0].numel() == fused_stats[1] * c * 2:
+                part, blocks, shift = fused_stats
+                with _timed(lambda: "norm_stats(from conv partials) c%d" % c, lambda: {"flops": 0.0, "bytes": 8.0 * part.numel()}):
+                    check(L.mri3d_norm_stats_from_partials(ctypes.byref(gn), _ptr(part), blocks, _ptr(shift), _ptr(mean),
+                                                           _ptr(invstd), _ptr(running_mean) if upd else None,
+                                                           _ptr(running_var) if upd else None, float(momentum), _stream()),
+                          "norm_stats_from_partials")
+            else:
+                ws = _workspace(L.mri3d_norm_workspace_bytes(ctypes.byref(gn)), x.device)
+                with _timed(lambda: "norm_stats c%d vox%d n%d" % (c, g.vox, n), lambda: {"flops": 0.0, "bytes": _esz(x) * x.numel()}):
+                    check(L.mri3d_norm_stats(ctypes.byref(gn), _ptr(x), _ptr(mean), _ptr(invstd),
+                                             _ptr(running_mean) if upd else None, _ptr(running_var) if upd else None,
+                                             float(momentum), _ptr(ws), ws.numel(), _stream()), "norm_stats")
+        elif stats_mode == "running":
+            mean = running_mean.detach().to(torch.float32).contiguous()
+            invstd = torch.rsqrt(running_var.detach().to(torch.float32) + eps).contiguous()
+        elif stats_mode != "none":
+            raise RuntimeError("norm_act_pool: statistics mode %r is not served" % (stats_mode,))
+        skip = _new(x.shape, x)
+        pooled = _new((n, c, do, ho, wo), x)
+        idx = torch.empty(pooled.numel(), dtype=torch.uint8, device=x.device)
+        with _timed(lambda: "norm_act_pool_fwd c%d" % c,
+                    lambda: {"flops": 0.0, "bytes": _esz(x) * 2 * x.numel() + (_esz(x) + 1) * pooled.numel()}):
+            check(L.mri3d_norm_act_pool_fwd(ctypes.byref(g), ctypes.byref(pg), _ptr(x), _ptr(mean), _ptr(invstd), _ptr(gamma),
+                                            _ptr(beta), _ptr(alpha) if act_code == ACT_PRELU else None, _ptr(skip), _ptr(pooled),
+                                            _ptr(idx), _stream()), "norm_act_pool_fwd")
+        ctx.save_for_backward(x, idx, mean, invstd, gamma, beta, alpha)
+        ctx.geom = g
+        ctx.pooled_shape = tuple(pooled.shape)
+        ctx.training_stats = stats_mode == "batch"
+        ctx.set_materialize_grads(False)
+        return pooled, skip
+
+    @staticmethod
+    def backward(ctx, dpool, dskip):
+        L = _lib.lib()
+        if dpool is None and dskip is None:
+            return (None,) * 12
+        x, idx, mean, invstd, gamma, beta, alpha = ctx.saved_tensors
+        g0 = ctx.geom
+        n, c, d, h, w = x.shape
+        s_ld = p_ld = c
+        for name, t, shape in (("pooled", dpool, ctx.pooled_shape), ("skip", dskip, tuple(x.shape))):
+            if t is not None and (tuple(t.shape) != shape or t.dtype != x.dtype):
+                raise RuntimeError("norm_act_pool backward: %s gradient %s %s does not match %s %s"
+                                   % (name, tuple(t.shape), t.dtype, shape, x.dtype))
+        if dskip is not None:
+            dskip, s_ld = _nd(dskip)
+            if s_ld % 4 or dskip.data_ptr() % (4 * dskip.element_size()):
+                dskip, s_ld = dskip.contiguous(memory_format=CL3D), c
+        if dpool is not None:
+            dpool, p_ld = _nd(dpool)
+            if p_ld % 4 or dpool.data_ptr() % (4 * dpool.element_size()):
+                dpool, p_ld = dpool.contiguous(memory_format=CL3D), c
+        if g0.x_ld != g0.c:
+            x = x.contiguous(memory_format=CL3D)
+        two = (2, 2, 2)
+        g, pg, _ = _pool_tail_geoms(x, c, s_ld, p_ld, two, two, (0, 0, 0), g0.act, alpha, g0.slope, g0.eps)
+        pg_, pb_, pa_ = ctx.params
+        prelu = g.act == ACT_PRELU
+        need = ctx.needs_input_grad
+        want = (gamma is not None and need[1], beta is not None and need[2], prelu and need[3])
+        srcs = (gamma, beta, alpha)
+        sinks = [_sink_take(p) if wt else None for p, wt in zip(ctx.params, want)]
+        grads = [(sk if sk is not None else torch.empty_like(t, memory_format=torch.contiguous_format)) if wt else None
+                 for sk, t, wt in zip(sinks, srcs, want)]
+        dx = _new(x.shape, x) if need[0] else None
+        ws = _workspace(L.mri3d_norm_act_pool_workspace_bytes(ctypes.byref(g), ctypes.byref(pg)), x.device)
+        passes = 2 if ctx.training_stats else 1
+        npool = idx.numel()
+        with _timed(lambda: "norm_act_pool_bwd c%d" % c,
+                    lambda: {"flops": 0.0,
+                             "bytes": passes * (_esz(x) * (x.numel() + (x.numel() if dskip is not None else 0))
+                                                + ((_esz(x) + 1) * npool if dpool is not None else 0))
+                                      + (_esz(x) * x.numel() if dx is not None else 0)}):
+            check(L.mri3d_norm_act_pool_bwd(ctypes.byref(g), ctypes.byref(pg), 1 if ctx.training_stats else 0, _ptr(x),
+                                            _ptr(dskip), _ptr(dpool), _ptr(idx), _ptr(mean), _ptr(invstd), _ptr(gamma),
+                                            _ptr(beta), _ptr(alpha) if prelu else None, _ptr(dx), _ptr(grads[0]), _ptr(grads[1]),
+                                            _ptr(grads[2]), _ptr(ws), ws.numel(), _stream()), "norm_act_pool_bwd")
+        outs = [_sink_done(p, gr, sk) for p, gr, sk in zip(ctx.params, grads, sinks)]
+        return (dx, outs[0], outs[1], outs[2], None, None, None, None, None, None, None, None)
+
+
+def norm_act_pool(x, gamma=None, beta=None, alpha=None, running_mean=None, running_var=None, stats_mode="batch",
+                  momentum=0.1, eps=1e-5, act=None, slope=0.01):
+    if momentum is None:
+        raise RuntimeError("cumulative moving average (momentum=None) is not supported")
+    fused = getattr(x, "_mri3d_bn_stats", None) if stats_mode == "batch" else None
+    return _NormActPoolFn.apply(x, gamma, beta, alpha, running_mean, running_var, stats_mode, momentum, eps, act, slope, fused)
+
+
 def activation(x, act, alpha=None, slope=0.01):
     return norm_act(x, None, None, alpha, None, None, "none", 0.1, 0.0, act, slope)
 
diff --git a/mri_epilepsy_diagnosis_amd/unet/unet.py b/mri_epilepsy_diagnosis_amd/unet/unet.py
--- a/mri_epilepsy_diagnosis_amd/unet/unet.py
+++ b/mri_epilepsy_diagnosis_amd/unet/unet.py
@@ -32,8 +32,8 @@
         self.dropout_layer = None
         self.block = tnn.Sequential(*[m for m in (conv, norm, act) if m is not None])
 
-    def forward(self, x, out=None, head=None):
-        return mnn.conv_norm_act(self.conv_layer, self.norm_layer, self.activation_layer, x, out, head)
+    def forward(self, x, out=None, head=None, pool=None):
+        return mnn.conv_norm_act(self.conv_layer, self.norm_layer, self.activation_layer, x, out, head, pool)
 
 
 class EncodingBlock(tnn.Module):
@@ -55,9 +55,11 @@
                 raise NotImplementedError("only max pooling is used by the reference")
             self.downsample = mnn.MaxPool3d(kernel_size=2)
 
-    def forward(self, x, skip_out=None, head=None):
+    def forward(self, x, skip_out=None, head=None, fused_pool=True):
         if self.downsample is None:
             return self.conv2(self.conv1(x), skip_out, head)
+        if fused_pool and skip_out is None and isinstance(self.downsample, mnn.MaxPool3d):
+            return self.conv2(self.conv1(x), pool=self.downsample)
         x = self.conv2(self.conv1(x), skip_out)
         return self.downsample.forward_with_skip(x)
 
@@ -83,10 +85,10 @@
             if self.dilation is not None:
                 self.dilation *= 2
 
-    def forward(self, x, cat_bufs=None):
+    def forward(self, x, cat_bufs=None, fused_pool=True):
         skips = []
         for i, blk in enumerate(self.encoding_blocks):
-            x, skip = blk(x, None if cat_bufs is None else (cat_bufs[i], 0))
+            x, skip = blk(x, None if cat_bufs is None else (cat_bufs[i], 0), fused_pool=fused_pool)
             skips.append(skip)
         return skips, x
 
@@ -170,6 +172,7 @@
         self.monte_carlo_layer = None
         self.shared_concat_buffers = False
         self.fused_head = True
+        self.fused_pool = True
         self.classifier = ConvolutionalBlock(dimensions, 2 * out_channels_first_layer, out_classes, kernel_size=1,
                                              activation=None)
 
@@ -188,7 +191,7 @@
         clf = self.classifier
         head = clf.conv_layer if (self.fused_head and x.is_cuda and clf.norm_layer is None and clf.activation_layer is None
                                   and clf.dropout_layer is None) else None
-        skips, enc = self.encoder(x, cat_bufs)
+        skips, enc = self.encoder(x, cat_bufs, self.fused_pool)
         if not skips:
             return self.bottom_block(enc, head=head) if head is not None else self.classifier(self.bottom_block(enc))
         enc = self.bottom_block(enc)
```
